# bderembl/msom

Hardware: AMD Instinct MI355X
Metric: grid-point-updates/s (timesteps/s x N^2 x nl), multi-layer QG RK2 step at 4096x4096x6 per GPU (higher is better)
Workload: dtype f64; 1 GPU; C4: msqg double gyre (Verron 1992 params), 4096x4096x6 fp64, tiles 1x1 of 4096x4096, TOLERANCE 1e-3, RK2 step = 2 inversions + 2 tendencies + 2 advances; mg_nrelax=4

## Files before the change

### msom_amd/csrc/kernels.h

```cpp
#ifndef MSOM_KERNELS_H
#define MSOM_KERNELS_H

#include <stdio.h>
#include <stdlib.h>

#include <type_traits>
#include <utility>

#include "msom_internal.h"
#include "modes_inl.h"

template <int LO, int HI, class F>
static inline bool with_int(int v, F &&f) {
  if constexpr (LO > HI) return false;
  else {
    if (v == LO) { f(std::integral_constant<int, LO>{}); return true; }
    return with_int<LO + 1, HI>(v, std::forward<F>(f));
  }
}
template <class F>
static inline void with_bool(bool b, F &&f) {
  if (b) f(std::true_type{});
  else f(std::false_type{});
}
[[noreturn]] static inline void no_kernel(const char *launcher, int nl) {
  fprintf(stderr, "msom: %s: no kernel for nl = %d\n", launcher, nl);
  abort();
}

struct LayerCoef {
  double idh0[MSOM_MAXNL], idh1[MSOM_MAXNL];
};

struct RelaxCoef {
  double D, sqD;
  double idh0[MSOM_MAXNL], idh1[MSOM_MAXNL];
  double t2[MSOM_MAXNL];
  double w[MSOM_MAXNL];
  double it1[MSOM_MAXNL];
  double S[MSOM_MAXNL];
};

struct KernelOpts {
  int march_rows = 0;
  int march_xcd = 1;
  int march_flip = 1;
  int march_dbg = 0;
  int march_lean = 2;
  int march_dma = 2;
  int march_visit_rows = 0;
  int march_visit_pairs = 2;
  int march_visit_ring = 2;
  int march_visit_split = 0;
  int resmax_rows = 0;
  int block_variant = 0;
  int rhs_dbg = 0;
  int lpw_dbg = 0;
};
int device_cu_count();

void launch_fill_ghost(hipStream_t st, double *f, const NatGeom &g, int nl, int bc, int walls, int depth = 1);
void launch_fill_periodic(hipStream_t st, double *f, const NatGeom &g, int nl, int depth);
void launch_fill_lin_dirichlet(hipStream_t st, double *f, const NatGeom &g, int nl, const double *upg, const double *vpg, double D, double Lx,
                               double Ly, int ox = 0, int oy = 0, int sides = WALL_ALL);
void launch_slip_bc(hipStream_t st, const double *po, double *zeta, const NatGeom &g, int nl, double c, int walls);
void launch_pack(hipStream_t st, const double *src, double *dst, const NatGeom &g, int nl);
void launch_unpack(hipStream_t st, const double *src, double *dst, const NatGeom &g, int nl);
void launch_del2(hipStream_t st, const double *po, double *zeta, const NatGeom &g, int nl, double add, double fac, double D);
void launch_stretch(hipStream_t st, const double *po, double *out, const double *S, const NatGeom &g, int nl, double add, double fac,
                    const LayerCoef &lc);
void launch_advection(hipStream_t st, const double *zeta, const double *psi, const double *psipg, const double *zetapg, const double *S,
                      const double *qot, double *dq, const NatGeom &g, int nl, int have_pg, int have_zpg, int stochastic, double D,
                      double beta, double itr_stoch, const LayerCoef &lc);
void launch_umax(hipStream_t st, const double *f, double *partial, double *out, const NatGeom &g, int nl, double D);
void launch_axpy(hipStream_t st, double *dq, const double *x, const NatGeom &g, int nl, double c);
void launch_forcing(hipStream_t st, const double *zeta, const double *psi, const double *qforc, const double *topo, const double *Ro,
                    const double *wind, double *dq, const NatGeom &g, int nl, int have_qforc, int flag_topo, double cs, double cb,
                    double D, double dhb);
void launch_advance(hipStream_t st, double *qo, const double *qi, const double *dq, const double *noise, const NatGeom &g, int nl, double dt,
                    double dts);
void launch_bfn_ab3(hipStream_t st, double *q, double *f1, const double *f2, const double *f3, const double *obs, const double *gain,
                    const NatGeom &g, int nl, double dt12, double k);
int bfn_misfit_blocks(const NatGeom &g);
void launch_bfn_misfit(hipStream_t st, const double *q, const double *obs, const double *gain, double *partial, double *out2, const NatGeom &g,
                       int nl);
struct StatsAcc {
  double *s[MSOM_ST_NACC];
};
void launch_stats_acc(hipStream_t st, unsigned mask, const double *psi, const double *q, const StatsAcc &a, const NatGeom &g, int nl,
                      const double *w_dev, double w, double D2, double *W);
void launch_stats_mean(hipStream_t st, double *out, const double *s, const double *W, const NatGeom &g, int nl);
void launch_stats_derive(hipStream_t st, double *out, const double *pm, const double *sa, const double *sq, const double *W, const NatGeom &g,
                         int nl, int which, double D2);
void launch_time_filter(hipStream_t st, double *me, const double *q, const NatGeom &g, int nl, double a);
int partial_count(const NatGeom &g);
void launch_sum_final(hipStream_t st, const double *partial, double *out, int n);
void launch_ke(hipStream_t st, const double *po, double *partial, double *out, const NatGeom &g, double D);
void launch_sum_layers(hipStream_t st, const double *f, double *partial, double *out, const NatGeom &g, int nl);
void launch_sub_layer_const(hipStream_t st, double *f, const double *sums, const NatGeom &g, int nl, double inv_count);
void launch_make_S(hipStream_t st, const double *Fr, const double *Ro, double *S, const NatGeom &g, int nlm);

void launch_noise(hipStream_t st, double *n, const double *sigma, const NatGeom &g, int nl, double amp, unsigned seed, unsigned draw, int gx0,
                  int gy0, int gnx);

void launch_ptr_rhs(hipStream_t st, const double *psi, const double *c, const double *rel, double *dp, const NatGeom &g, int nl, int np,
                    const double *iPe, const double *ptr_ir, double D);

void launch_advection_de(hipStream_t st, const double *zeta, const double *psi, const double *psipg, const double *zetapg, const double *S, double *j1,
                         double *j2, double *j3, const NatGeom &g, int nl, double D, double beta, double dt, double ediag, const LayerCoef &lc);
void launch_dissip_de(hipStream_t st, const double *p4, const double *str, const double *po, double *dq, const NatGeom &g, int nl, double iRe,
                      double iRe4, double dt, double ediag, double D, int stage);
void launch_ekman_de(hipStream_t st, const double *zeta, const double *po, double *dq, const NatGeom &g, int nl, double cs, double cb, double dt,
                     double ediag);
void launch_running_mean(hipStream_t st, double *pm, const double *po, const NatGeom &g, int nl, int n);
void launch_filter_de(hipStream_t st, double *ft, const double *tmp2, double *pm, const NatGeom &g, int nl, double dtflt, double ediag);

struct RhsResid {
  double *res, *res_c;
  double *res_max;
  double *bsum_partial;
  SplitGeom sg, cg;
};
int rhs_fused_blocks(const NatGeom &g);
void launch_rhs_fused(hipStream_t st, const KernelOpts &o, const double *psi, const double *S, const double *qforc, const double *wind, double *dq,
                      double *umax_partial, double *umax_out, const NatGeom &g, int nl, int walls, int uniformS, const double *Su,
                      int have_qforc, double D, double beta, double iRe, double iRe4, double cs, double cb, double slip_c,
                      const LayerCoef &lc, int variant, const double *q_in = nullptr, double *q_out = nullptr, double dt = 0.,
                      const RhsResid *rr = nullptr, int region = 0, const double *dt_ptr = nullptr);
int rhs_pipe_blocks(const NatGeom &g);
void launch_rhs_lpw(hipStream_t st, const KernelOpts &o, const double *psi, const double *S, const double *qforc, const double *wind, double *dq,
                    const NatGeom &g, int nl, int walls, int uniformS, const double *Su, int have_qforc, double D, double beta, double iRe, double iRe4,
                    double cs, double cb, double slip_c, const LayerCoef &lc, const double *q_in, double *q_out, double dt, int stoch = 0,
                    const double *q_stage = nullptr, const double *noise = nullptr, double crelax = 0., double dts = 0., int region = 0,
                    const double *dt_ptr = nullptr, const RhsResid *rr = nullptr);
int rhs_lpw_blocks(const KernelOpts &o, const NatGeom &g, int nl);

#define MGC_MAXLEV 8
#define MGC_MAXDIM 32
#define MGC_NT 512
struct CoarseLev { double *da, *res; const double *S; SplitGeom g; RelaxCoef rc; };
struct CoarseArgs { CoarseLev lev[MGC_MAXLEV]; int n, walls, prolong_fused, lds; };
void launch_mg_coarse(hipStream_t st, const CoarseArgs *d_args, int nrelax, int nl, int uniformS, int lean = 0);
size_t mg_coarse_lean_doubles(const CoarseArgs &h, int nl);
#define MGC_POOL 19200
size_t mg_coarse_static_lds();
void launch_nat_to_split(hipStream_t st, const double *nat, const NatGeom &g, double *sp, const SplitGeom &sg, int nl);
void launch_split_to_nat(hipStream_t st, const double *sp, const SplitGeom &sg, double *nat, const NatGeom &g, int nl);
void launch_split_pack(hipStream_t st, const double *src, double *sp, const SplitGeom &sg, int nl, int bc, int walls);
void launch_split_unpack(hipStream_t st, const double *sp, const SplitGeom &sg, double *dst, int nl);
void launch_residual(hipStream_t st, const double *a, const double *b, const double *S, const NatGeom &g, double *res, const SplitGeom &sg,
                     int nl, const RelaxCoef &rc, int uniformS, double *maxres, double *sum_partial, int want_sum);
int residual2_blocks(const NatGeom &g);
void launch_residual2(hipStream_t st, const KernelOpts &o, int mode, const double *a, const double *da, double *a_out, const double *b, const double *S,
                      const NatGeom &g, double *res, const SplitGeom &sg, double *res_c, const SplitGeom &cg, int nl, const RelaxCoef &rc,
                      int uniformS, int walls, double *maxres, double *sum_partial, int want_sum, double *umax_partial, double *umax_out,
                      int umax_clean = 0,
                      double *res_c2 = nullptr, const SplitGeom *cg2 = nullptr);
void launch_restrict(hipStream_t st, const double *fine, const SplitGeom &fg, double *coarse, const SplitGeom &cg, int nl);
void launch_restrict_pyramid(hipStream_t st, const double *fine, double *const *out, const SplitGeom *g, int n, int nl);
void launch_prolong(hipStream_t st, const double *coarse, const SplitGeom &cg, double *fine, const SplitGeom &fg, int nl, int walls);
void launch_relax_color(hipStream_t st, double *da, const double *res, const double *S, const SplitGeom &sg, int nl, const RelaxCoef &rc,
                        int uniformS, int color, int walls, int fine, int region = 0);
void launch_relax_ring(hipStream_t st, double *da, const double *res, const double *S, const SplitGeom &sg, int nl, const RelaxCoef &rc,
                       int uniformS, int color, int walls);
int launch_relax_block8(hipStream_t st, const KernelOpts &o, const double *da_in, const double *coarse, const SplitGeom &cg, const double *res, double *da_out,
                        const SplitGeom &sg, int nl, const RelaxCoef &rc, int walls, int nh, int c0, const double *S = nullptr);
void launch_relax_block2(hipStream_t st, const KernelOpts &o, const double *da_in, const double *coarse, const SplitGeom &cg, const double *res, double *da_out,
                         const SplitGeom &sg, int nl, const RelaxCoef &rc, int walls, int fine);
void launch_relax_red_prolong(hipStream_t st, const KernelOpts &o, double *da, const double *coarse, const SplitGeom &cg, const double *res, const double *S,
                              const SplitGeom &sg, int nl, const RelaxCoef &rc, int uniformS, int walls);
void launch_correct(hipStream_t st, double *a, const NatGeom &g, const double *da, const SplitGeom &sg, int nl, int walls);

struct VisitRingBands { int s0[4], ns[4], c0[4], nc[4], n; };
struct MarchCorrect { const double *psi; double *psi_out; NatGeom g; };
struct MarchHalo { const double *in_s, *in_n, *res_s, *res_n; size_t ls; int rows; };
int launch_relax_march(hipStream_t st, const KernelOpts &o, const double *in, double *out, const double *res, const SplitGeom &sg, int nl, const RelaxCoef &rc, int c1,
                       int K, int walls, int chunk_rows = 0, const MarchHalo *h = nullptr, const double *coarse = nullptr, const SplitGeom *cg = nullptr,
                       const MarchCorrect *mc = nullptr, int more_follow = 0, const MarchHalo *coarse_halo = nullptr, int region = 0,
                       const int *skip = nullptr, int skip_compact = 0);
int launch_relax_visit(hipStream_t st, const KernelOpts &o, double *da, double *da_alt, const double *res, const SplitGeom &sg, int nl, const RelaxCoef &rc,
                       int walls, const double *coarse, const SplitGeom &cg, const MarchCorrect &mc);
bool relax_visit_fits(int nl, const SplitGeom &sg, int rows, int pairs);
extern "C" int msom_visit_ring(int hk, int ny, int march_rows, int visit_rows, int pairs, int corr, int *geom, int *bands);
bool march_lean_fits(int nl, const SplitGeom &sg, const NatGeom *ng);

struct ModeCoef {
  double m2l[MSOM_MAXNL * MSOM_MAXNL], ibu[MSOM_MAXNL];
};
int launch_modes_eig(hipStream_t st, const double *S, const NatGeom &g, int nl, int ncx, int ncy, double *out, size_t ols, int per_column,
                     const ModesLayers &l, int *flag);
int launch_modes_get(hipStream_t st, double *out, const double *md, const ModeCoef *mc, const NatGeom &g, int nl, const ModesLayers &l, int which,
                     int first, int cnt);
int launch_modes_rd(hipStream_t st, double *rd, const double *md, const ModeCoef *mc, const NatGeom &g, int nl, int mode);
int launch_modes_project(hipStream_t st, const double *in, double *out, const double *md, const ModeCoef *mc, const NatGeom &g, int nl,
                         const ModesLayers &l, int to_modes);
int modes_energy_blocks(const NatGeom &g);
int modes_energy_stride(const NatGeom &g);
int launch_modes_energy(hipStream_t st, const double *psi, const double *md, const ModeCoef *mc, const NatGeom &g, int nl, const ModesLayers &l,
                        double *partial, double *out, double D);

struct HelmCoef {
  double ibu[MSOM_MAXNL];
  double rd[MSOM_MAXNL];
};
struct HelmCount {
  int n[MSOM_MAXNL];
};
MSOM_HD double helm_diag(double ibu, double sqD) {
#ifdef MSOM_STRICT
  return (-(ibu * sqD) + 2.) + 2.;
#else
  return fma(-ibu, sqD, 4.);
#endif
}
HelmCoef helm_coef(const double *ibu, int nl, double sqD);
int launch_helm_relax(hipStream_t st, double *da, const double *res, const double *ibu_sp, const HelmCoef *hc, const SplitGeom &sg, int nl,
                      double sqD, int color, int sweep, const HelmCount &cnt, int walls);
int helm_residual_blocks(const NatGeom &g);
int launch_helm_residual(hipStream_t st, const double *a, const double *b, const double *ibu_sp, const HelmCoef *hc, const NatGeom &g, double *res,
                         const SplitGeom &sg, int nl, double D, double *maxres, double *sum_partial, int stride, int want_sum);

enum { SPEC_IN_AB = 0, SPEC_IN_UV = 1, SPEC_IN_G = 2 };
enum { SPEC_CROSS = 0, SPEC_SUM = 1 };
struct SpecIn {
  const double *a, *b;
  size_t off, ls;
  int pitch, l0, mode;
  double D2, rD2;
  double dhc[MSOM_MAXNL];
};
int spec_prepare_device();
void launch_spec_rows(hipStream_t st, const SpecIn &in, int nx, int ny, int layers, double2 *Z, const double2 *tw, int nt);
void launch_spec_transpose(hipStream_t st, const double2 *Z, double2 *ZT, int nx, int ny, int layers);
void launch_spec_cols(hipStream_t st, const double2 *ZT, int nx, int ny, int layers, int kind, double scale, double *V, double *out2d, const double2 *tw,
                      int nt);
void launch_spec_shells(hipStream_t st, const double *V, int nx, int ny, int layers, int smax, double *TE);
void launch_spec_final(hipStream_t st, const double *TE, int smax, int nbins, int layers, double dk2, double *res);

int nq_rhs_rows(const NatGeom &g, int rows);
void launch_nq_rhs(hipStream_t st, const double *psi, const double *qforc, double *zeta, double *dq, const NatGeom &g, int walls, double D,
                   double beta, double nu, double cek, double bc_fac, const double *q_in, double *q_out, double dt, int rows);
void launch_nq_ghost(hipStream_t st, const double *psi, double *f, const NatGeom &g, double bc_fac);
void launch_nq_adv(hipStream_t st, const double *psi, const double *zeta, double *dq, const NatGeom &g, double D, double beta);

void launch_wv_restrict(hipStream_t st, const double *f, const NatGeom &fg, double *c, const NatGeom &cg, int nl);
void launch_wv_recon(hipStream_t st, const double *s, const double *sc, const double *rc, const double *sig, double *out, const NatGeom &fg,
                     const NatGeom &cg, int nl);
void launch_wv_root(hipStream_t st, const double *s, const double *sig, double *r, const NatGeom &g, int nl);
void launch_wv_recon_m(hipStream_t st, const double *s, const double *sc, const double *rc, const double *sig, const double *mc, double *out,
                       const NatGeom &fg, const NatGeom &cg, int nl);
void launch_wv_root_m(hipStream_t st, const double *s, const double *sig, const double *mc, double *r, const NatGeom &g, int nl);
void launch_wv_vert2cell(hipStream_t st, const double *v, const NatGeom &vg, double *c, const NatGeom &cg, int nl);
void launch_wv_vertex_update(hipStream_t st, double *psi, double *psif, const double *c, const double *mask, const NatGeom &vg, const NatGeom &cg, int nl,
                             double dtflt, int nbar, int update_mean);
void launch_wv_qof(hipStream_t st, double *qof, double *q, const double *tmp, const NatGeom &g, int nl, double dtflt, int nbar, int restore);

void launch_n_bnd_from(hipStream_t st, double *f, const double *g, const NatGeom &ge, int nl, double c, int use_g_bnd, double gbc, int walls = WALL_ALL);
void launch_n_bnd_const(hipStream_t st, double *f, const NatGeom &ge, int nl, double v, int sp = 0, int walls = WALL_ALL);
void launch_n_mul_mask(hipStream_t st, double *a, double *b, const double *mk, const NatGeom &g, int nl);
void launch_n_del2(hipStream_t st, const double *in, double *out, const NatGeom &g, int nl, double add, double fac, double D);
void launch_n_stretch(hipStream_t st, const double *in, double *out, const double *S2, const NatGeom &g, int nl, double add, double fac,
                      const LayerCoef &lc);
void launch_n_stretch_sqg(hipStream_t st, const double *in, const double *bs, const double *S2S, double *out, const double *S2, const NatGeom &g, int nl,
                          double add, double fac, const LayerCoef &lc);
void launch_n_lap_bs(hipStream_t st, const double *bs, double *out, const NatGeom &g, double D);
void launch_n_sqg_rhs(hipStream_t st, const double *q, const double *S2S, const double *bs, double *qeff, const NatGeom &g, int nl, double idh00);
void launch_n_rhs_main(hipStream_t st, const double *psi, const double *zeta, const double *pg, const double *S2, const double *topo, double *dq,
                       const NatGeom &g, int nl, int have_pg, int have_topo, double D, double beta, double drag, double f0, double dhb, const LayerCoef &lc);
void launch_n_axpy(hipStream_t st, double *dq, const double *x, const NatGeom &g, int nl, double c);
void launch_n_rhs_pre(hipStream_t st, double *q, const double *psi, double *psi_out, double *zeta, const double *mk, const NatGeom &g, int nl, double D,
                      double bc, double gbc);
void launch_n_del2_bnd(hipStream_t st, const double *in, double *out, const NatGeom &g, int nl, double D, double bc, int use_bnd, double gbc);
void launch_n_rhs_all(hipStream_t st, const double *psi, const double *zeta, const double *tmp, const double *pg, const double *S2, const double *topo,
                      const double *qf, const double *qf3d, const double *mk, const double *d2bs, const double *S2S, double *dq, const NatGeom &g, int nl,
// ... 67 lines not shown
```

### msom_amd/csrc/kernels_lpw.hip

```cpp
#include "rhs_inl.h"

#pragma clang fp contract(off)

#define LPW_W 58
#define LPW_R 4
#define LPW_R_RES 2
#ifdef MSOM_STRICT
#define LPW_NV 3
#define LPW_MAXW 8
#else
#define LPW_NV 2
#define LPW_MAXW 12
#endif

struct LpwArgs {
  const double *psi, *S, *qforc, *wind, *q_in;
  const double *q_stage, *noise;
  double crelax, dts;
  double *dq, *q_out;
  double dt;
  const double *dt_ptr;
  NatGeom g;
  int nl, walls, uniformS, have_qforc, H, NS;
  int noedge_off;
  int region;
  int dbg;
  RhsResid rr;
  double D, beta, iRe, iRe4, cs, cb, slip_c;
  LayerCoef lc;
  double Su[MSOM_MAXNL];
};

template <int R, bool UNI, bool QF, bool ADV, bool STOCH, bool EDGE, bool RES, int NV>
__device__ __forceinline__ void lpw_body(const LpwArgs &a, double (&ring)[2][LPW_MAXW][R][NV][64], double &res_m, double &res_bs) {
  const int lane = threadIdx.x & 63;
  const int wv = __builtin_amdgcn_readfirstlane((int)(threadIdx.x >> 6));
  const int nl = a.nl, nx = a.g.nx, ny = a.g.ny;
  const int l = wv % nl;
  const ptrdiff_t pitch = a.g.pitch;
  const int strip = blockIdx.x * a.NS + wv / nl, nstrips = (nx + LPW_W - 1) / LPW_W;
  const int x0 = min(strip, nstrips - 1) * LPW_W, y0 = blockIdx.y * a.H, y1 = min(ny, y0 + a.H);
  const int gi = x0 - 3 + lane, gic = min(gi, nx + 2);
  const double dtv = a.dt_ptr ? *a.dt_ptr : a.dt;
  const double D = a.D, D2 = D * D, rD2 = 1. / D2, D12 = 12. * D * D, rD12 = 1. / D12, D2x = 2 * D, rD2x = 1. / D2x;
  const double rD = 1. / D;
  const bool oddx = !(lane & 1);
  const bool lower = l + 1 < nl, upper = l > 0;
  const int lW = ((a.walls & WALL_W) && x0 == 0) ? 2 : -1;
  const int eL = nx - x0 + 3;
  const int lE = ((a.walls & WALL_E) && eL <= 63) ? eL : -1;
  const bool bcx = EDGE && (lW >= 0 || lE >= 0);
  const bool south = (a.walls & WALL_S) != 0, north = (a.walls & WALL_N) != 0;
  const bool slip = a.slip_c > 0.;
  const bool out_ok = lane >= 3 && lane <= 60 && gi < nx && strip < nstrips;
  const double *pP = a.psi + nat_idx(a.g, l, 0, gic);
  const double *pQ = lower ? pP + a.g.ls : pP;
  const double idh0 = a.lc.idh0[l], idh1 = a.lc.idh1[l];
  const double su0 = (nl > 1 && upper) ? a.Su[l - 1] : 0., su1 = (nl > 1 && lower) ? a.Su[l] : 0.;
  const double windv = l == 0 ? a.wind[min(y0 + lane, ny - 1)] : 0.;
  auto wind_row = [&](int j) -> double {
    const long long b = __double_as_longlong(windv);
    const int lo = __builtin_amdgcn_readlane((int)b, j - y0), hi = __builtin_amdgcn_readlane((int)(b >> 32), j - y0);
    return __longlong_as_double(((long long)hi << 32) | (unsigned int)lo);
  };

  double P[5], PL[4], PR[4], Z[4], ZL[4], ZR[4], T[3], TL[2], TR[2], Q[3], QL[3], QR[3];
#pragma unroll
  for (int k = 0; k < 5; k++) P[k] = 0.;
#pragma unroll
  for (int k = 0; k < 4; k++) PL[k] = PR[k] = Z[k] = ZL[k] = ZR[k] = 0.;
#pragma unroll
  for (int k = 0; k < 3; k++) T[k] = Q[k] = QL[k] = QR[k] = 0.;
  TL[0] = TL[1] = TR[0] = TR[1] = 0.;

#ifdef MSOM_STRICT
  double abA[R], jdA[R], lapTA[R], zcA[R], tcA[R];
#else
  double tlA[R];
#endif
  double pnext[R], qnext[R], qreg[R], fqreg[R], qsreg[STOCH ? R : 1], nzreg[STOCH ? R : 1];
  double xdA[R], ydA[R];
#pragma unroll
  for (int r = 0; r < R; r++) xdA[r] = ydA[r] = 0.;
#pragma unroll
  for (int r = 0; r < R; r++) {
#ifdef MSOM_STRICT
    abA[r] = jdA[r] = lapTA[r] = zcA[r] = tcA[r] = 0.;
#else
    tlA[r] = 0.;
#endif
    pnext[r] = qnext[r] = qreg[r] = fqreg[r] = 0.;
  }

  auto ld = [&](const double *base, int j) -> double { return base[(ptrdiff_t)((a.dbg & 2) ? y0 : (EDGE ? min(j, ny + 2) : j)) * pitch]; };
#ifdef MSOM_STRICT
  auto lap5 = [&](double c, double w, double e, double n, double s) -> double { return DIVC(e + w + n + s - 4 * c, D2, rD2); };
#else
  auto lap5 = [&](double c, double w, double e, double n, double s) -> double { return fma(-4., c, e + w + n + s) * rD2; };
#endif
  auto xfix = [&](double raw, double so, double sw, double se) -> double {
    if (bcx) {
      if (slip) {
        if (lane == lW) raw = a.slip_c * (se - so);
        if (lane == lE) raw = a.slip_c * (sw - so);
      } else {
        const double re = lane_above(raw), rw = lane_below(raw);
        if (lane == lW) raw = -re;
        if (lane == lE) raw = -rw;
      }
    }
    return raw;
  };
  auto yghost = [&](double dm, double dmw, double dme, double sm, double sg) -> double {
    double v = slip ? a.slip_c * (sm - sg) : -dm;
    if (lane == lW) v = dme;
    if (lane == lE) v = dmw;
    return v;
  };

  auto row = [&](int j, double pnew, double qnew, bool centre, bool yedge, int b, int r) {
#pragma unroll
    for (int k = 0; k < 4; k++) P[k] = P[k + 1];
    P[4] = pnew;
#pragma unroll
    for (int k = 0; k < 3; k++) { PL[k] = PL[k + 1]; PR[k] = PR[k + 1]; Z[k] = Z[k + 1]; ZL[k] = ZL[k + 1]; ZR[k] = ZR[k + 1]; }
    T[0] = T[1]; T[1] = T[2]; TL[0] = TL[1]; TR[0] = TR[1];
#pragma unroll
    for (int k = 0; k < 2; k++) { Q[k] = Q[k + 1]; QL[k] = QL[k + 1]; QR[k] = QR[k + 1]; }
    Q[2] = qnew; QL[2] = lane_below(qnew); QR[2] = lane_above(qnew);
    PL[3] = lane_below(P[3]); PR[3] = lane_above(P[3]);
    double z = xfix(lap5(P[3], PL[3], PR[3], P[4], P[2]), P[3], PL[3], PR[3]);
    if (yedge && north && j + 2 == ny) z = yghost(Z[2], ZL[2], ZR[2], P[2], P[3]);
    Z[3] = z; ZL[3] = lane_below(z); ZR[3] = lane_above(z);
    if (yedge && south && j + 2 == 0) {
      Z[2] = yghost(Z[3], ZL[3], ZR[3], P[3], P[2]);
      ZL[2] = lane_below(Z[2]); ZR[2] = lane_above(Z[2]);
    }
    double t = xfix(lap5(Z[2], ZL[2], ZR[2], Z[3], Z[1]), Z[2], ZL[2], ZR[2]);
    if (yedge && north && j + 1 == ny) t = yghost(T[1], TL[0], TR[0], Z[1], Z[2]);
    T[2] = t; TL[1] = lane_below(t); TR[1] = lane_above(t);
    if (yedge && south && j + 1 == 0) T[1] = yghost(T[2], TL[1], TR[1], Z[2], Z[1]);
    if (!centre) return;

    double p[3][3], zz[3][3], p1[3][3];
#pragma unroll
    for (int k = 0; k < 3; k++) {
      p[k][0] = PL[k]; p[k][1] = P[k]; p[k][2] = PR[k];
      zz[k][0] = ZL[k]; zz[k][1] = Z[k]; zz[k][2] = ZR[k];
      p1[k][0] = QL[k]; p1[k][1] = Q[k]; p1[k][2] = QR[k];
    }
    const double adv = (STOCH && l == 0) ? 0. : mjac9(p, zz, D12, rD12);
    const double be = DIVC(a.beta * (p[1][0] - p[1][2]), D2x, rD2x);
    const double jd = (lower && !STOCH) ? mjac9(p, p1, D12, rD12) : 0.;
    const double zc = Z[1], tc = T[1];
    const double lapT = lap5(tc, TL[0], TR[0], T[2], T[0]);
    if (RES) {
      const double dW = P[1] - PL[1], dE = PR[1] - P[1], dS = P[1] - P[0], dN = P[2] - P[1];
#ifdef MSOM_STRICT
      xdA[r] = (dW / D - dE / D) / D;
      ydA[r] = (dS / D - dN / D) / D;
#else
      const double fa = oddx ? dW : dE, fb = oddx ? dE : dW;
      const double x = fma(rD, fb, -(rD * fa));
      xdA[r] = oddx ? -x : x;
      ydA[r] = fma(rD, dS, -(rD * dN));
#endif
      ring[b][wv][r][NV - 1][lane] = Q[1] - P[1];
    }
#ifdef MSOM_STRICT
    abA[r] = adv + be; jdA[r] = jd; lapTA[r] = lapT; zcA[r] = zc; tcA[r] = tc;
    ring[b][wv][r][0][lane] = zc;
    ring[b][wv][r][1][lane] = tc;
    ring[b][wv][r][2][lane] = jd;
#else
    double tl = fma(tc, a.iRe, fma(a.iRe4, lapT, adv + be));
    if (l == 0) tl -= fma(a.cs, zc, wind_row(j));
    if (l == nl - 1) tl = fma(-a.cb, zc, tl);
    tlA[r] = tl;
    ring[b][wv][r][0][lane] = fma(a.iRe, zc, a.iRe4 * tc);
    ring[b][wv][r][1][lane] = jd;
#endif
  };

  auto finish = [&](int j, int b, int r, double s0, double s1, double fq) -> double {
#ifdef MSOM_STRICT
    const double zc = zcA[r], tc = tcA[r];
    double zm = 0., tm = 0., zp = 0., tp = 0., ju = 0.;
    if (upper) { zm = ring[b][wv - 1][r][0][lane]; tm = ring[b][wv - 1][r][1][lane]; ju = -ring[b][wv - 1][r][2][lane]; }
    if (lower) { zp = ring[b][wv + 1][r][0][lane]; tp = ring[b][wv + 1][r][1][lane]; }
    double t = abA[r];
    if (nl > 1) {
      if (upper) t = t + s0 * ju * idh0;
      if (lower) t = t + s1 * jdA[r] * idh1;
    }
    t = 0. + t;
    double dq = t;
    auto stretch = [&](double fac, double pm, double pc, double pp) -> double {
      if (l == 0) return fac * s1 * (pp - pc) * idh1;
      if (l < nl - 1) return fac * (s0 * (pm - pc) * idh0 + s1 * (pp - pc) * idh1);
      return fac * s0 * (pm - pc) * idh0;
    };
    if (a.iRe != 0.) {
      if (nl > 1) dq = 1. * dq + stretch(a.iRe, zm, zc, zp);
      dq += tc * a.iRe;
    }
    if (a.iRe4 != 0.) {
      if (nl > 1) dq = 1. * dq + stretch(a.iRe4, tm, tc, tp);
      dq = 1. * dq + a.iRe4 * lapTA[r];
    }
    if (l == 0) dq -= a.cs * zc;
    if (l == nl - 1) dq -= a.cb * zc;
    if (l == 0) dq -= wind_row(j);
#else
    double dq = tlA[r];
    const double xc = ring[b][wv][r][0][lane];
    if (nl > 1) {
      if (upper) dq = fma(s0 * idh0, (ring[b][wv - 1][r][0][lane] - xc) - ring[b][wv - 1][r][1][lane], dq);
      if (lower) dq = fma(s1 * idh1, (ring[b][wv + 1][r][0][lane] - xc) + ring[b][wv][r][1][lane], dq);
    }
#endif
    if (QF) dq += fq;
#ifdef MSOM_STRICT
    if (STOCH) return (qreg[r] + qsreg[r] * a.crelax + nzreg[r] * a.dts) + dq * a.dt;
    return ADV ? qreg[r] + dq * dtv : dq;
#else
    if (STOCH) return fma(dq, a.dt, fma(nzreg[r], a.dts, fma(qsreg[r], a.crelax, qreg[r])));
    return ADV ? fma(dq, dtv, qreg[r]) : dq;
#endif
  };

  auto resid = [&](int b, int r, double s0, double s1, double q) -> double {
    double re = q;
#ifdef MSOM_STRICT
    if (upper) re = re + s0 * ring[b][wv - 1][r][NV - 1][lane] * idh0;
    if (lower) re = re - s1 * ring[b][wv][r][NV - 1][lane] * idh1;
    re += xdA[r];
    re += ydA[r];
#else
    if (upper) re = fma(idh0, s0 * ring[b][wv - 1][r][NV - 1][lane], re);
    if (lower) re = fma(-(ring[b][wv][r][NV - 1][lane] * s1), idh1, re);
    re = fma(rD, xdA[r], re);
    re = fma(rD, ydA[r], re);
#endif
    return re;
  };

#pragma unroll
  for (int r = 0; r < R; r++) {
    pnext[r] = ld(pP, y0 + r + 3);
    qnext[r] = ld(pQ, y0 + r + 1);
  }
  {
    double wp[6], wq[2];
#pragma unroll
    for (int k = 0; k < 6; k++) wp[k] = ld(pP, y0 - 3 + k);
    wq[0] = ld(pQ, y0 - 1); wq[1] = ld(pQ, y0);
#pragma unroll
    for (int k = 0; k < 6; k++) row(y0 - 6 + k, wp[k], k >= 4 ? wq[k - 4] : 0., false, EDGE, 0, 0);
  }

  double *const outp = ADV ? a.q_out : a.dq;
  const int nblk = (y1 - y0 + R - 1) / R;
  __builtin_amdgcn_s_waitcnt(0x0F70);
  for (int k = 0; k <= nblk; k++) {
    const int b = k & 1;
    if (k > 0) {
      const int jb = y0 + (k - 1) * R;
      double s0[R], s1[R], val[R];
#pragma unroll
      for (int r = 0; r < R; r++) {
        s0[r] = su0; s1[r] = su1;
        if (!UNI && nl > 1) {
          const size_t c = nat_idx(a.g, l, min(jb + r, ny - 1), gic);
          if (upper) s0[r] = a.S[c - a.g.ls];
          if (lower) s1[r] = a.S[c];
        }
      }
#pragma unroll
      for (int r = 0; r < R; r++) {
        val[r] = finish(jb + r, b ^ 1, r, s0[r], s1[r], fqreg[r]);
        asm volatile("" : "+v"(val[r]));
      }
#pragma unroll
      for (int r = 0; r < R; r++)
        if (out_ok && jb + r < y1 && !(a.dbg & 1)) outp[nat_idx(a.g, l, jb + r, gic)] = val[r];
      if (RES) {
        double re[R];
#pragma unroll
        for (int r = 0; r < R; r++) {
          re[r] = resid(b ^ 1, r, s0[r], s1[r], val[r]);
          if (out_ok && jb + r < y1) {
            res_m = fmax(res_m, fabs(re[r]));
            res_bs += val[r];
            if (!(a.dbg & 1)) a.rr.res[split_idx(a.rr.sg, l, jb + r, gi)] = re[r];
          }
        }
#pragma unroll
        for (int r = 0; r + 1 < R; r += 2) {
          const double o0 = lane_above(re[r]), o1 = lane_above(re[r + 1]);
          if (out_ok && !oddx && jb + r + 1 < y1 && !(a.dbg & 1)) {
            double sum = 0.;
            sum += re[r];
            sum += re[r + 1];
            sum += o0;
            sum += o1;
            a.rr.res_c[split_idx(a.rr.cg, l, (jb + r) >> 1, gi >> 1)] = sum / 4;
          }
        }
      }
    }
    if (k < nblk) {
      const int j0 = y0 + k * R;
      const bool yedge = EDGE && j0 + R + 2 > ny;
#pragma unroll
      for (int r = 0; r < R; r++) {
        const size_t c = nat_idx(a.g, l, (a.dbg & 2) ? y0 : (EDGE ? min(j0 + r, ny - 1) : j0 + r), gic);
        if (ADV) qreg[r] = a.q_in[c];
        if (QF) fqreg[r] = a.qforc[c];
        if (STOCH) { qsreg[r] = a.q_stage[c]; nzreg[r] = a.noise[c]; }
      }
#pragma unroll
      for (int r = 0; r < R; r++) {
        const int j = j0 + r;
        double pn, qn;
        asm volatile("v_mov_b64 %0, %1" : "=v"(pn) : "v"(pnext[r]));
        asm volatile("v_mov_b64 %0, %1" : "=v"(qn) : "v"(qnext[r]));
        pnext[r] = ld(pP, j + R + 3);
        qnext[r] = ld(pQ, j + R + 1);
        row(j, pn, qn, true, yedge, b, r);
      }
    }
    __syncthreads();
  }
}

template <int R, bool UNI, bool QF, bool ADV, bool STOCH = false, bool RES = false>
__global__ void __launch_bounds__(64 * LPW_MAXW) k_rhs_lpw(LpwArgs a) {
  static_assert(!RES || (ADV && !STOCH && R % 2 == 0), "the residual by-product rides in the plain tendency + advance pass");
  constexpr int NV = LPW_NV + (RES ? 1 : 0);
  __shared__ double ring[2][LPW_MAXW][R][NV][64];
  double res_m = 0., res_bs = 0.;
  const int wv = __builtin_amdgcn_readfirstlane((int)(threadIdx.x >> 6));
  const int nx = a.g.nx, ny = a.g.ny;
  const int strip = blockIdx.x * a.NS + wv / a.nl, nstrips = (nx + LPW_W - 1) / LPW_W;
  const int x0 = min(strip, nstrips - 1) * LPW_W, y0 = blockIdx.y * a.H, y1 = min(ny, y0 + a.H);
  const bool xwall = ((a.walls & WALL_W) && x0 == 0) || ((a.walls & WALL_E) && nx - x0 + 3 <= 63);
  const int nblk = (y1 - y0 + R - 1) / R;
  const bool ywall = y0 == 0 || y0 + nblk * R + R > ny;
  if (a.region) {
    const bool inner = strip < nstrips && x0 - 3 >= 0 && x0 + 60 < nx && y0 - 3 >= 0 && y0 + nblk * R + R + 2 < ny;
    if ((a.region == 1) != inner) return;
  }
  if (xwall || ywall || a.noedge_off) lpw_body<R, UNI, QF, ADV, STOCH, true, RES, NV>(a, ring, res_m, res_bs);
  else lpw_body<R, UNI, QF, ADV, STOCH, false, RES, NV>(a, ring, res_m, res_bs);
  if (RES) {
    const int lane = threadIdx.x & 63, nw = blockDim.x >> 6;
    for (int o = 32; o > 0; o >>= 1) {
      res_m = fmax(res_m, __shfl_xor(res_m, o, 64));
      res_bs += __shfl_xor(res_bs, o, 64);
    }
    double *red = &ring[0][0][0][0][0];
    if (lane == 0) { red[wv] = res_m; red[LPW_MAXW + wv] = res_bs; }
    __syncthreads();
    if (threadIdx.x == 0) {
      double mm = red[0], ss = red[LPW_MAXW];
      for (int k = 1; k < nw; k++) { mm = fmax(mm, red[k]); ss += red[LPW_MAXW + k]; }
      atomicMax((unsigned long long *)a.rr.res_max, (unsigned long long)__double_as_longlong(mm));
      a.rr.bsum_partial[blockIdx.y * gridDim.x + blockIdx.x] = ss;
    }
  }
}

static void lpw_shape(const KernelOpts &o, const NatGeom &g, int nl, bool res, int &NS, int &H) {
  const int strips = (g.nx + LPW_W - 1) / LPW_W;
  H = o.rhs_dbg >> 8;
  NS = LPW_MAXW / nl < 1 ? 1 : LPW_MAXW / nl;
  if (NS > strips) NS = strips;
  if (H <= 0) {
    const int ncu = device_cu_count();
    const int wgx = (strips + NS - 1) / NS;
    double best = -1.;
    for (int h = 64; h >= 8; h -= 8) {
      const double r = (double)wgx * ((g.ny + h - 1) / h) / ncu, cost = (r <= 3. ? ceil(r) : r + 0.5) * (h + 6);
      if (best < 0. || cost < best) { best = cost; H = h; }
    }
  }
  if (H < 8) H = 8;
  if (res) H = (H + 1) & ~1;
}
int rhs_lpw_blocks(const KernelOpts &o, const NatGeom &g, int nl) {
  int NS, H;
  lpw_shape(o, g, nl, true, NS, H);
  const int strips = (g.nx + LPW_W - 1) / LPW_W;
  return ((strips + NS - 1) / NS) * ((g.ny + H - 1) / H);
}

void launch_rhs_lpw(hipStream_t st, const KernelOpts &o, const double *psi, const double *S, const double *qforc, const double *wind, double *dq,
                    const NatGeom &g, int nl, int walls, int uniformS, const double *Su, int have_qforc, double D, double beta, double iRe, double iRe4,
                    double cs, double cb, double slip_c, const LayerCoef &lc, const double *q_in, double *q_out, double dt, int stoch,
                    const double *q_stage, const double *noise, double crelax, double dts, int region, const double *dt_ptr, const RhsResid *rr) {
  LpwArgs a;
  const bool res = rr != nullptr;
  if (res && (stoch || !q_out || region || (g.nx & 1) || (g.ny & 1) || !rr->res_c)) {
    fprintf(stderr, "msom: launch_rhs_lpw: the residual by-product needs the plain tendency + advance pass on one tile with even sides\n");
    abort();
  }
  if (res) {
    a.rr = *rr;
    (void)hipMemsetAsync(rr->res_max, 0, sizeof(double), st);
  } else {
    a.rr.res = a.rr.res_c = a.rr.res_max = a.rr.bsum_partial = nullptr;
    a.rr.sg = SplitGeom(); a.rr.cg = SplitGeom();
  }
  a.region = region;
  a.dt_ptr = dt_ptr;
  a.q_stage = q_stage; a.noise = noise; a.crelax = crelax; a.dts = dts;
  a.psi = psi; a.S = S; a.qforc = qforc; a.wind = wind; a.q_in = q_in; a.dq = dq; a.q_out = q_out; a.dt = dt;
  a.dbg = o.lpw_dbg & 3;
  a.noedge_off = (o.lpw_dbg & 4) != 0;
  a.g = g; a.nl = nl; a.walls = walls; a.uniformS = uniformS; a.have_qforc = have_qforc;
  a.D = D; a.beta = beta; a.iRe = iRe; a.iRe4 = iRe4; a.cs = cs; a.cb = cb; a.slip_c = slip_c; a.lc = lc;
  for (int l = 0; l < MSOM_MAXNL; l++) a.Su[l] = Su ? Su[l] : 0.;
  const int strips = (g.nx + LPW_W - 1) / LPW_W;
  int H;
  lpw_shape(o, g, nl, res, a.NS, H);
  a.H = H;
  const dim3 gr((strips + a.NS - 1) / a.NS, (g.ny + H - 1) / H), bl(64 * nl * a.NS);
  if (stoch && !q_out) {
    fprintf(stderr, "msom: launch_rhs_lpw: stochastic variant needs q_out\n");
    abort();
  }
  with_bool(uniformS, [&](auto U) {
    with_bool(have_qforc, [&](auto Q) {
      constexpr bool UNI = decltype(U)::value, QF = decltype(Q)::value;
      if (stoch) hipLaunchKernelGGL((k_rhs_lpw<LPW_R, UNI, QF, true, true>), gr, bl, 0, st, a);
      else if (res) hipLaunchKernelGGL((k_rhs_lpw<LPW_R_RES, UNI, QF, true, false, true>), gr, bl, 0, st, a);
      else if (q_out) hipLaunchKernelGGL((k_rhs_lpw<LPW_R, UNI, QF, true>), gr, bl, 0, st, a);
      else hipLaunchKernelGGL((k_rhs_lpw<LPW_R, UNI, QF, false>), gr, bl, 0, st, a);
    });
  });
}
```

### msom_amd/csrc/kernels_mg.hip

```cpp
#include "kernels.h"
#include "mg_inl.h"
#include "rhs_inl.h"


#define BX 64
#define BY 4

static inline dim3 grid2d(int nx, int ny) { return dim3((nx + BX - 1) / BX, (ny + BY - 1) / BY); }
static inline dim3 block2d() { return dim3(BX, BY); }

__device__ __forceinline__ double wave_max(double v) {
  for (int o = 32; o > 0; o >>= 1) v = fmax(v, __shfl_down(v, o, 64));
  return v;
}
__device__ __forceinline__ double wave_sum(double v) {
  for (int o = 32; o > 0; o >>= 1) v += __shfl_down(v, o, 64);
  return v;
}


__global__ void k_nat_to_split(const double *__restrict__ nat, NatGeom g, double *sp, SplitGeom sg, int nl) {
  const int i = blockIdx.x * BX + threadIdx.x, j = blockIdx.y * BY + threadIdx.y;
  if (i >= g.nx || j >= g.ny) return;
  for (int l = 0; l < nl; l++) sp[split_idx(sg, l, j, i)] = nat[nat_idx(g, l, j, i)];
// ... 228 lines not shown
  if (p.want_sum) bs = wave_sum(bs);
  if (VEL) {
#pragma unroll
    for (int l = 0; l < MSOM_MAXNL; l++)
      if (l < nl) {
        const double v = wave_max(um[l]);
        if (threadIdx.x == 0) smu[l][threadIdx.y] = v;
      }
  }
  if (threadIdx.x == 0) { smm[threadIdx.y] = m; sms[threadIdx.y] = bs; }
  __syncthreads();
  if (threadIdx.x == 0 && threadIdx.y == 0) {
    double mm = smm[0], ss = sms[0];
    for (int k = 1; k < BY; k++) { mm = fmax(mm, smm[k]); ss += sms[k]; }
    atomicMax((unsigned long long *)p.maxres, (unsigned long long)__double_as_longlong(mm));
    if (p.want_sum) p.sum_partial[blockIdx.y * gridDim.x + blockIdx.x] = ss;
  }
  if (VEL && threadIdx.y == 0 && threadIdx.x < nl) {
    double v = smu[threadIdx.x][0];
    for (int k = 1; k < BY; k++) v = fmax(v, smu[threadIdx.x][k]);
    p.umax_partial[(size_t)(blockIdx.y * gridDim.x + blockIdx.x) * nl + threadIdx.x] = v;
  }
}

#define CR_TR 16
#define CR_TW 128
#define CR_LP 132
template <bool UNIFORM, bool CORR = true>
__global__ void __launch_bounds__(BX *BY, UNIFORM ? 4 : 3) k_correct_residual(Res2Args p) {
  __shared__ __align__(16) double T[2][CR_TR + 2][CR_LP];
  __shared__ double smm[BY];
  __shared__ double smu[MSOM_MAXNL][BY];
  constexpr int NR = CR_TR / BY;
  const int tx = threadIdx.x, ty = threadIdx.y, tid = ty * BX + tx;
  const int x0 = blockIdx.x * CR_TW, y0 = blockIdx.y * CR_TR;
  const int nl = p.nl, nx = p.g.nx, ny = p.g.ny;
  const int i = x0 + 2 * tx;
  const double D = p.rc.D, rD = 1. / D;
  const bool inx = i < nx;
  const size_t c0 = nat_idx(p.g, 0, y0 + ty, inx ? i : 0), se0 = split_idx(p.sg, 0, y0 + ty, inx ? i : 0);
  const size_t cstep = (size_t)BY * p.g.pitch, sstep = (size_t)BY * p.sg.rp;
  constexpr int NH = 2 * (CR_TW + 2) + 2 * CR_TR;
  double a0e[NR], a0o[NR], a1e[NR], a1o[NR], a2e[NR], a2o[NR];
  auto stage = [&](int l, int b, double *xe, double *xo) {
    const double *al = p.a + (size_t)l * p.g.ls, *dl = p.da + (size_t)l * p.sg.ls;
#pragma unroll
    for (int k = 0; k < NR; k++) {
      double e = 0., o = 0.;
      if (inx && y0 + ty + BY * k < ny) {
        const double2 v = *reinterpret_cast<const double2 *>(al + c0 + k * cstep);
        e = v.x; o = v.y;
        if (CORR) { e = e + dl[se0 + k * sstep]; o = o + dl[se0 + k * sstep + p.sg.hp]; }
      }
      xe[k] = e; xo[k] = o;
      *reinterpret_cast<double2 *>(&T[b][ty + BY * k + 1][2 * tx + 2]) = make_double2(e, o);
    }
    for (int h = tid; h < NH; h += BX * BY) {
      int r, cc;
      if (h < CR_TW + 2) { r = -1; cc = h - 1; }
      else if (h < 2 * (CR_TW + 2)) { r = CR_TR; cc = h - (CR_TW + 2) - 1; }
      else if (h < 2 * (CR_TW + 2) + CR_TR) { r = h - 2 * (CR_TW + 2); cc = -1; }
      else { r = h - 2 * (CR_TW + 2) - CR_TR; cc = CR_TW; }
      const int gx = x0 + cc, gy = y0 + r;
      double v = 0.;
      if (gx <= nx && gy <= ny) {
        v = al[nat_idx(p.g, 0, gy, gx)];
        if (CORR) v = v + dl[split_idx(p.sg, 0, gy, gx)];
      }
      T[b][r + 1][cc + 2] = v;
    }
  };
  double m = 0.;
  double s1e[NR], s1o[NR], s0e[NR], s0o[NR];
#pragma unroll
  for (int k = 0; k < NR; k++) { a0e[k] = a0o[k] = a2e[k] = a2o[k] = 0.; s0e[k] = s0o[k] = s1e[k] = s1o[k] = 0.; }
  stage(0, 0, a1e, a1o);
  __syncthreads();
  for (int l = 0; l < nl; l++) {
    const int b = l & 1;
    if (l < nl - 1) stage(l + 1, b ^ 1, a2e, a2o);
    const double su0 = l > 0 ? p.rc.S[l - 1] : 0., su1 = l < nl - 1 ? p.rc.S[l] : 0.;
    const double i0 = p.rc.idh0[l], i1 = p.rc.idh1[l];
    double uu = 0.;
#pragma unroll
    for (int k = 0; k < NR; k++) {
      const int j = y0 + ty + BY * k;
      if (inx && j < ny) {
        const int r = ty + BY * k + 1, cx = 2 * tx + 2;
        const size_t cl = c0 + k * cstep + (size_t)l * p.g.ls;
        const double2 bv = *reinterpret_cast<const double2 *>(p.b + cl);
        const double be = bv.x, bo = bv.y;
        double z0e, z0o, z1e, z1o;
        if (UNIFORM) { z0e = z0o = su0; z1e = z1o = su1; }
        else {
          if (l < nl - 1) { const double2 sv = *reinterpret_cast<const double2 *>(p.S + cl); s1e[k] = sv.x; s1o[k] = sv.y; }
          z0e = s0e[k]; z0o = s0o[k]; z1e = s1e[k]; z1o = s1o[k];
        }
        const double e1 = a1e[k], o1 = a1o[k];
        const double a1w = T[b][r][cx - 1], a1ee = T[b][r][cx + 2];
        const double2 sv2 = *reinterpret_cast<const double2 *>(&T[b][r - 1][cx]), nv2 = *reinterpret_cast<const double2 *>(&T[b][r + 1][cx]);
        const double a1se = sv2.x, a1so = sv2.y, a1ne = nv2.x, a1no = nv2.y;
        double re = be, ro = bo;
        if (nl > 1) {
          if (l == 0) {
            re = be + z1e * (e1 - a2e[k]) * i1;
            ro = bo + z1o * (o1 - a2o[k]) * i1;
          } else if (l < nl - 1) {
            re = be + z0e * (e1 - a0e[k]) * i0 - z1e * (a2e[k] - e1) * i1;
            ro = bo + z0o * (o1 - a0o[k]) * i0 - z1o * (a2o[k] - o1) * i1;
          } else {
            re = be + z0e * (e1 - a0e[k]) * i0;
            ro = bo + z0o * (o1 - a0o[k]) * i0;
          }
        }
        re += DIVC(DIVC(e1 - a1w, D, rD) - DIVC(o1 - e1, D, rD), D, rD);
        re += DIVC(DIVC(e1 - a1se, D, rD) - DIVC(a1ne - e1, D, rD), D, rD);
        ro += DIVC(DIVC(o1 - e1, D, rD) - DIVC(a1ee - o1, D, rD), D, rD);
        ro += DIVC(DIVC(o1 - a1so, D, rD) - DIVC(a1no - o1, D, rD), D, rD);
        if (CORR) {
          *reinterpret_cast<double2 *>(p.a_out + cl) = make_double2(e1, o1);
          nat_write_ghosts(p.a_out, p.g, l, j, i, e1, p.walls);
          nat_write_ghosts(p.a_out, p.g, l, j, i + 1, o1, p.walls);
        }
        m = fmax(m, fmax(fabs(re), fabs(ro)));
        const double nw = T[b][r + 1][cx - 1], sw = T[b][r - 1][cx - 1], se2 = T[b][r - 1][cx + 2];
        const double ue = fabs(DIVC(0.25 * (a1ne - a1se + nw - sw), D, rD)), ve = fabs(DIVC(0.25 * (o1 - a1w + a1so - sw), D, rD));
        const double uo = fabs(DIVC(0.25 * (a1no - a1so + a1ne - a1se), D, rD)), vo = fabs(DIVC(0.25 * (a1ee - e1 + se2 - a1se), D, rD));
        uu = fmax(uu, fmax(fmax(ue, ve), fmax(uo, vo)));
        a0e[k] = e1; a0o[k] = o1;
        if (!UNIFORM) { s0e[k] = s1e[k]; s0o[k] = s1o[k]; }
        a1e[k] = a2e[k]; a1o[k] = a2o[k];
      }
    }
    uu = wave_max(uu);
    if (tx == 0) smu[l][ty] = uu;
    __syncthreads();
  }
  m = wave_max(m);
  if (tx == 0) smm[ty] = m;
  __syncthreads();
  if (tid == 0) {
    double mm = smm[0];
    for (int k = 1; k < BY; k++) mm = fmax(mm, smm[k]);
    atomicMax((unsigned long long *)p.maxres, (unsigned long long)__double_as_longlong(mm));
  }
  if (ty == 0 && tx < nl) {
    double v = smu[tx][0];
    for (int k = 1; k < BY; k++) v = fmax(v, smu[tx][k]);
    p.umax_partial[(size_t)(blockIdx.y * gridDim.x + blockIdx.x) * nl + tx] = v;
  }
}

#define RM_OW 62
template <int NL>
__global__ void __launch_bounds__(256) k_resmax_march(Res2Args p, int H) {
  __shared__ double smm[4];
  __shared__ double smu[MSOM_MAXNL][4];
  const int lane = threadIdx.x & 63, wv = threadIdx.x >> 6;
  const int strip = blockIdx.x * 4 + wv;
  const int nx = p.g.nx, ny = p.g.ny, pitch = p.g.pitch;
  const int nstrips = (nx + RM_OW - 1) / RM_OW;
  const double D = p.rc.D, rD = 1. / D;
  double m = 0., uu[NL];
#pragma unroll
  for (int l = 0; l < NL; l++) uu[l] = 0.;
  const int y0 = blockIdx.y * H, y1 = min(y0 + H, ny);
  if (strip < nstrips && y0 < ny) {
    const int x0 = strip * RM_OW, gi = min(x0 - 1 + lane, nx);
    const bool own = lane >= 1 && lane <= RM_OW && x0 - 1 + lane < nx;
    const size_t ls = p.g.ls;
    const double *pa = p.a + nat_idx(p.g, 0, 0, gi), *pb = p.b + nat_idx(p.g, 0, 0, min(gi, nx - 1) < 0 ? 0 : min(gi, nx - 1));
    double Wm[NL], Wc[NL], Wp[NL], Wn[NL], Em[NL], Mm[NL], qc[NL], qn[NL];
#pragma unroll
    for (int l = 0; l < NL; l++) {
      Wm[l] = pa[l * ls + (ptrdiff_t)(y0 - 1) * pitch];
      Wc[l] = pa[l * ls + (ptrdiff_t)y0 * pitch];
      Wp[l] = pa[l * ls + (ptrdiff_t)min(y0 + 1, ny) * pitch];
      qc[l] = pb[l * ls + (ptrdiff_t)y0 * pitch];
    }
#pragma unroll
    for (int l = 0; l < NL; l++) { Em[l] = lane_above(Wm[l]); Mm[l] = lane_below(Wm[l]); }
    for (int j = y0; j < y1; j++) {
      const ptrdiff_t rn = (ptrdiff_t)min(j + 2, ny) * pitch, rq = (ptrdiff_t)min(j + 1, ny - 1) * pitch;
#pragma unroll
      for (int l = 0; l < NL; l++) { Wn[l] = pa[l * ls + rn]; qn[l] = pb[l * ls + rq]; }
#pragma unroll
      for (int l = 0; l < NL; l++) {
        const double c = Wc[l], E = lane_above(c), W = lane_below(c), N = Wp[l], S = Wm[l], NW = lane_below(N), SE = Em[l], SW = Mm[l];
        const double be = qc[l];
        double re = be;
        if (NL > 1) {
          const double i0 = p.rc.idh0[l], i1 = p.rc.idh1[l];
          const double z0 = l > 0 ? p.rc.S[l - 1] : 0., z1 = l < NL - 1 ? p.rc.S[l] : 0.;
          if (l == 0) re = be + z1 * (c - Wc[l + 1 < NL ? l + 1 : l]) * i1;
          else if (l < NL - 1) re = be + z0 * (c - Wc[l - 1]) * i0 - z1 * (Wc[l + 1 < NL ? l + 1 : l] - c) * i1;
          else re = be + z0 * (c - Wc[l - 1]) * i0;
        }
        re += DIVC(DIVC(c - W, D, rD) - DIVC(E - c, D, rD), D, rD);
        re += DIVC(DIVC(c - S, D, rD) - DIVC(N - c, D, rD), D, rD);
        const double u = fabs(DIVC(0.25 * (N - S + NW - SW), D, rD)), v = fabs(DIVC(0.25 * (E - W + SE - SW), D, rD));
        if (own) { m = fmax(m, fabs(re)); uu[l] = fmax(uu[l], fmax(u, v)); }
        Em[l] = E; Mm[l] = W;
      }
#pragma unroll
      for (int l = 0; l < NL; l++) { Wm[l] = Wc[l]; Wc[l] = Wp[l]; Wp[l] = Wn[l]; qc[l] = qn[l]; }
    }
  }
  m = wave_max(m);
  if (lane == 0) smm[wv] = m;
#pragma unroll
  for (int l = 0; l < NL; l++) {
    const double w = wave_max(uu[l]);
    if (lane == 0) smu[l][wv] = w;
  }
  __syncthreads();
  if (threadIdx.x == 0) {
    const double mm = fmax(fmax(smm[0], smm[1]), fmax(smm[2], smm[3]));
    atomicMax((unsigned long long *)p.maxres, (unsigned long long)__double_as_longlong(mm));
  }
  if (threadIdx.x < NL)
    p.umax_partial[(size_t)(blockIdx.y * gridDim.x + blockIdx.x) * NL + threadIdx.x] =
        fmax(fmax(smu[threadIdx.x][0], smu[threadIdx.x][1]), fmax(smu[threadIdx.x][2], smu[threadIdx.x][3]));
}
template <int NL>
static dim3 resmax_march_launch(hipStream_t st, const Res2Args &p, int H) {
  const int nstrips = (p.g.nx + RM_OW - 1) / RM_OW;
  dim3 gr((nstrips + 3) / 4, (p.g.ny + H - 1) / H);
  hipLaunchKernelGGL(k_resmax_march<NL>, gr, dim3(256), 0, st, p, H);
  return gr;
}
static dim3 launch_resmax_march(hipStream_t st, const Res2Args &p, int H) {
  dim3 gr;
  if (!with_int<1, MSOM_FASTNL>(p.nl, [&](auto N) { gr = resmax_march_launch<N()>(st, p, H); })) no_kernel("launch_resmax_march", p.nl);
  return gr;
}

__global__ void k_max_final_mg(const double *partial, double *out, int nb, int nl) {
  __shared__ double sm[MSOM_MAXNL][4];
  const int per = (nb + gridDim.x - 1) / gridDim.x, b0 = blockIdx.x * per, b1 = min(nb, b0 + per);
  double v[MSOM_MAXNL];
#pragma unroll
  for (int l = 0; l < MSOM_MAXNL; l++) v[l] = 0.;
  for (int b = b0 + threadIdx.x; b < b1; b += 256) {
    const double *row = partial + (size_t)b * nl;
#pragma unroll
    for (int l = 0; l < MSOM_MAXNL; l++)
      if (l < nl) v[l] = fmax(v[l], row[l]);
  }
#pragma unroll
  for (int l = 0; l < MSOM_MAXNL; l++) {
    double w = v[l];
    for (int o = 32; o > 0; o >>= 1) w = fmax(w, __shfl_down(w, o, 64));
    if ((threadIdx.x & 63) == 0) sm[l][threadIdx.x >> 6] = w;
  }
  __syncthreads();
  if (threadIdx.x < nl) {
    const double w = fmax(fmax(sm[threadIdx.x][0], sm[threadIdx.x][1]), fmax(sm[threadIdx.x][2], sm[threadIdx.x][3]));
    atomicMax((unsigned long long *)(out + threadIdx.x), (unsigned long long)__double_as_longlong(w));
  }
}

int residual2_blocks(const NatGeom &g) {
  dim3 gr = grid2d(g.nx / 2, g.ny);
  return gr.x * gr.y;
}
void launch_residual2(hipStream_t st, const KernelOpts &o, int mode, const double *a, const double *da, double *a_out, const double *b, const double *S,
                      const NatGeom &g, double *res, const SplitGeom &sg, double *res_c, const SplitGeom &cg, int nl, const RelaxCoef &rc,
                      int uniformS, int walls, double *maxres, double *sum_partial, int want_sum, double *umax_partial, double *umax_out, int umax_clean,
                      double *res_c2, const SplitGeom *cg2) {
  Res2Args p;
  p.res_c2 = res_c2;
  if (cg2) p.cg2 = *cg2; else p.cg2 = cg;
  p.dbg = o.rhs_dbg;
  p.umax_partial = umax_partial;
  p.a = a; p.b = b; p.S = S; p.da = da; p.a_out = a_out; p.res = res; p.res_c = res_c; p.maxres = maxres; p.sum_partial = sum_partial;
  p.g = g; p.sg = sg; p.cg = cg; p.nl = nl; p.uniformS = uniformS; p.want_sum = want_sum; p.walls = walls; p.rc = rc;
  dim3 gr = grid2d(g.nx / 2, g.ny);
  switch (mode) {
    case 1:
      if (g.nx % 2 == 0 && g.nx >= CR_TW && g.ny >= CR_TR && !(p.dbg & 128)) {
        gr = dim3((g.nx + CR_TW - 1) / CR_TW, (g.ny + CR_TR - 1) / CR_TR);
        if (uniformS) hipLaunchKernelGGL((k_correct_residual<true, true>), gr, block2d(), 0, st, p);
        else hipLaunchKernelGGL((k_correct_residual<false, true>), gr, block2d(), 0, st, p);
      } else
        hipLaunchKernelGGL((k_residual2<true, false, false>), gr, block2d(), 0, st, p);
      if (!umax_clean) (void)hipMemsetAsync(umax_out, 0, nl * sizeof(double), st);
      hipLaunchKernelGGL(k_max_final_mg, dim3(64), dim3(256), 0, st, umax_partial, umax_out, (int)(gr.x * gr.y), nl);
      break;
    case 2: hipLaunchKernelGGL((k_residual2<false, true, false>), gr, block2d(), 0, st, p); break;
    case 6: hipLaunchKernelGGL((k_residual2<false, true, true>), gr, block2d(), (size_t)nl * (BY * BX * 2 + 2 * BX) * sizeof(double), st, p); break;
    case 0: hipLaunchKernelGGL((k_residual2<false, false, false>), gr, block2d(), 0, st, p); break;
    case 8:
      if (uniformS && g.nx >= 64 && g.ny >= 16 && o.resmax_rows >= 0 && nl <= MSOM_FASTNL) {
        gr = launch_resmax_march(st, p, o.resmax_rows ? o.resmax_rows : 32);
      } else if (g.nx % 2 == 0 && g.nx >= CR_TW && g.ny >= CR_TR && !(p.dbg & 128)) {
        gr = dim3((g.nx + CR_TW - 1) / CR_TW, (g.ny + CR_TR - 1) / CR_TR);
        if (uniformS) hipLaunchKernelGGL((k_correct_residual<true, false>), gr, block2d(), 0, st, p);
        else hipLaunchKernelGGL((k_correct_residual<false, false>), gr, block2d(), 0, st, p);
      } else
        hipLaunchKernelGGL((k_residual2<false, false, false, true>), gr, block2d(), 0, st, p);
      if (!umax_clean) (void)hipMemsetAsync(umax_out, 0, nl * sizeof(double), st);
      hipLaunchKernelGGL(k_max_final_mg, dim3(64), dim3(256), 0, st, umax_partial, umax_out, (int)(gr.x * gr.y), nl);
      break;
    default: break;
  }
}


__device__ __forceinline__ void restrict_pt(const double *__restrict__ fine, const SplitGeom &fg, double *coarse, const SplitGeom &cg, int nl, int I, int J) {
  for (int l = 0; l < nl; l++) {
    double sum = 0.;
    sum += fine[split_idx(fg, l, 2 * J, 2 * I)];
    sum += fine[split_idx(fg, l, 2 * J + 1, 2 * I)];
    sum += fine[split_idx(fg, l, 2 * J, 2 * I + 1)];
    sum += fine[split_idx(fg, l, 2 * J + 1, 2 * I + 1)];
    coarse[split_idx(cg, l, J, I)] = sum / 4;
  }
}
__global__ void k_restrict(const double *__restrict__ fine, SplitGeom fg, double *coarse, SplitGeom cg, int nl) {
  const int I = blockIdx.x * BX + threadIdx.x, J = blockIdx.y * BY + threadIdx.y;
  if (I >= cg.nx || J >= cg.ny) return;
  restrict_pt(fine, fg, coarse, cg, nl, I, J);
}
void launch_restrict(hipStream_t st, const double *fine, const SplitGeom &fg, double *coarse, const SplitGeom &cg, int nl) {
  hipLaunchKernelGGL(k_restrict, grid2d(cg.nx, cg.ny), block2d(), 0, st, fine, fg, coarse, cg, nl);
}

#define RPYR_MAX 5
struct RestrictPyramidArgs {
  const double *fine;
  double *out[RPYR_MAX];
  SplitGeom g[RPYR_MAX + 1];
  int n, nl;
};
__global__ void __launch_bounds__(256) k_restrict_pyramid(RestrictPyramidArgs a) {
  extern __shared__ double rp[];
  const int tid = threadIdx.x, n = a.n, nl = a.nl, T = 1 << n;
  const int X0 = blockIdx.x * T, Y0 = blockIdx.y * T;
  double *cur = rp, *nxt = rp + nl * (T / 2) * (T / 2);
  {
    const int s = T >> 1;
    for (int t = tid; t < s * s * nl; t += 256) {
      const int I = t % s, J = (t / s) % s, l = t / (s * s);
      const int fi = X0 + 2 * I, fj = Y0 + 2 * J;
      double sum = 0.;
      sum += a.fine[split_idx(a.g[0], l, fj, fi)];
      sum += a.fine[split_idx(a.g[0], l, fj + 1, fi)];
      sum += a.fine[split_idx(a.g[0], l, fj, fi + 1)];
      sum += a.fine[split_idx(a.g[0], l, fj + 1, fi + 1)];
      const double v = sum / 4;
      cur[(l * s + J) * s + I] = v;
      a.out[0][split_idx(a.g[1], l, (Y0 >> 1) + J, (X0 >> 1) + I)] = v;
    }
  }
  for (int k = 2; k <= n; k++) {
    __syncthreads();
    const int s = T >> k, sf = s << 1;
    for (int t = tid; t < s * s * nl; t += 256) {
      const int I = t % s, J = (t / s) % s, l = t / (s * s);
      const double *f = cur + l * sf * sf;
      double sum = 0.;
      sum += f[(2 * J) * sf + 2 * I];
      sum += f[(2 * J + 1) * sf + 2 * I];
      sum += f[(2 * J) * sf + 2 * I + 1];
      sum += f[(2 * J + 1) * sf + 2 * I + 1];
      const double v = sum / 4;
      nxt[(l * s + J) * s + I] = v;
      a.out[k - 1][split_idx(a.g[k], l, (Y0 >> k) + J, (X0 >> k) + I)] = v;
    }
    double *tmp = cur; cur = nxt; nxt = tmp;
  }
}
void launch_restrict_pyramid(hipStream_t st, const double *fine, double *const *out, const SplitGeom *g, int n, int nl) {
  RestrictPyramidArgs a;
  a.fine = fine; a.n = n; a.nl = nl;
  for (int k = 0; k <= n; k++) a.g[k] = g[k];
  for (int k = 0; k < n; k++) a.out[k] = out[k];
  const int T = 1 << n;
  const size_t lds = (size_t)nl * ((T / 2) * (T / 2) + (T / 4 > 0 ? (T / 4) * (T / 4) : 1)) * sizeof(double);
  hipLaunchKernelGGL(k_restrict_pyramid, dim3(g[0].nx / T, g[0].ny / T), dim3(256), lds, st, a);
}

__device__ __forceinline__ void prolong_pt(const double *__restrict__ coarse, const SplitGeom &cg, double *fine, const SplitGeom &fg, int nl, int walls, int i, int j) {
  const int I = i >> 1, J = j >> 1, cx = (i & 1) ? 1 : -1, cy = (j & 1) ? 1 : -1;
  for (int l = 0; l < nl; l++) {
    const double v = BILINEAR(coarse[split_idx(cg, l, J, I)], coarse[split_idx(cg, l, J, I + cx)], coarse[split_idx(cg, l, J + cy, I)],
                              coarse[split_idx(cg, l, J + cy, I + cx)]);
    fine[split_idx(fg, l, j, i)] = v;
    split_write_ghosts(fine, fg, l, j, i, v, walls);
  }
}
__global__ void k_prolong(const double *__restrict__ coarse, SplitGeom cg, double *fine, SplitGeom fg, int nl, int walls) {
  const int i = blockIdx.x * BX + threadIdx.x, j = blockIdx.y * BY + threadIdx.y;
  if (i >= fg.nx || j >= fg.ny) return;
  prolong_pt(coarse, cg, fine, fg, nl, walls, i, j);
}
void launch_prolong(hipStream_t st, const double *coarse, const SplitGeom &cg, double *fine, const SplitGeom &fg, int nl, int walls) {
  hipLaunchKernelGGL(k_prolong, grid2d(fg.nx, fg.ny), block2d(), 0, st, coarse, cg, fine, fg, nl, walls);
}


struct RelaxArgs {
  double *da;
  const double *res, *S;
  SplitGeom g;
  int color, walls;
  int region;
  RelaxCoef rc;
};

template <int NL, bool UNIFORM>
__device__ __forceinline__ void relax_color_pt(const RelaxArgs &p, int kx, int j);
template <int NL, bool UNIFORM, bool FINE>
__global__ void __launch_bounds__(BX *BY) k_relax_color(RelaxArgs p) {
  const int kx = blockIdx.x * BX + threadIdx.x, j = blockIdx.y * BY + threadIdx.y;
  if (kx >= p.g.hk || j >= p.g.ny) return;
  if (p.region == 1) {
    const int i = 2 * kx + ((j + p.color) & 1);
    if (i == 0 || i == p.g.nx - 1 || j == 0 || j == p.g.ny - 1) return;
  }
  relax_color_pt<NL, UNIFORM>(p, kx, j);
}
template <int NL, bool UNIFORM>
__global__ void __launch_bounds__(256) k_relax_ring(RelaxArgs p) {
  const int t = blockIdx.x * 256 + threadIdx.x, hk = p.g.hk, ny = p.g.ny;
  int kx, j;
  if (t < hk) { kx = t; j = 0; }
  else if (t < 2 * hk) { kx = t - hk; j = ny - 1; }
  else if (t < 2 * hk + ny - 2) { j = 1 + t - 2 * hk; kx = ((j + p.color) & 1) ? hk - 1 : 0; }
  else return;
  if (ny == 1 && t >= hk) return;
  relax_color_pt<NL, UNIFORM>(p, kx, j);
}
template <int NL, bool UNIFORM>
__device__ __forceinline__ void relax_color_pt(const RelaxArgs &p, int kx, int j) {
  const int px = (j + p.color) & 1;
  const int i = 2 * kx + px;
  const int hp = p.g.hp, rp = p.g.rp;
  const size_t ls = p.g.ls;
  const size_t own = (size_t)(j + 1) * rp + px * hp + MSOM_SP + kx;
  const size_t oth = (size_t)(j + 1) * rp + (1 - px) * hp + MSOM_SP + kx;
  const size_t iw = oth - 1 + px, ie = oth + px, is = own - rp, in = own + rp;
  const double sqD = p.rc.sqD;
  double rhs[NL], x[NL];
  if (NL == 1) {
    double n = -sqD * p.res[own], d = 0.;
    n += p.da[ie] + p.da[iw]; d += 2.;
// ... 1069 lines not shown
```

### msom_amd/csrc/msom_api.hip

```cpp
#include "msom_host.h"

#define RHS_RESID_MIN 23
#define MARCH_HALO 4

static void free_agglomeration(msom *m);

extern "C" const char *msom_version(void) {
#ifdef MSOM_STRICT
  return "msomhip 0.1 (strict: -ffp-contract=off, reference expression order, bit-exact vs oracle)";
#else
  return "msomhip 0.1 (fast: FMA contraction, reciprocal multiplies)";
#endif
}


NatGeom make_nat(int nx, int ny) {
  NatGeom g;
  g.nx = nx; g.ny = ny;
  g.pitch = ((nx + 15) / 16) * 16 + 2 * MSOM_XP;
  g.rows = ny + 2 * MSOM_YP;
  g.ls = (size_t)g.pitch * g.rows;
  return g;
}
static SplitGeom make_split(int nx, int ny) {
  SplitGeom s;
  s.nx = nx; s.ny = ny;
  s.hk = nx / 2;
  s.hp = ((s.hk + 15) / 16) * 16 + 2 * MSOM_SP;
  s.rp = 2 * s.hp;
  s.rows = ny + 2;
  s.ls = (size_t)s.rp * s.rows;
  return s;
}

int sync_stream(msom *m) {
  HIPCHK(hipStreamSynchronize(m->st));
  return m->sticky;
}

static bool prof_on(const msom *m, const ProfSlot &ps) {
  if (m->profile == 2) return &ps == &m->prof_march_corr || &ps == &m->prof_march_visit || (&ps >= &m->prof_march[0] && &ps <= &m->prof_march[4]);
  return m->profile != 0;
}
void prof_begin(msom *m, ProfSlot &ps) {
  if (!prof_on(m, ps)) return;
  if (ps.used + 2 > ps.ev.size()) {
    hipEvent_t a, b;
    hipEventCreate(&a); hipEventCreate(&b);
    ps.ev.push_back(a); ps.ev.push_back(b);
  }
  hipEventRecord(ps.ev[ps.used], m->st);
}
void prof_end(msom *m, ProfSlot &ps) {
  if (!prof_on(m, ps)) return;
  hipEventRecord(ps.ev[ps.used + 1], m->st);
  ps.used += 2;
}
void prof_collect(msom *m, ProfSlot &ps) {
  hipStreamSynchronize(m->st);
  for (size_t k = 0; k + 1 < ps.used; k += 2) {
    float ms = 0;
    if (hipEventElapsedTime(&ms, ps.ev[k], ps.ev[k + 1]) == hipSuccess) { ps.total_ms += ms; ps.launches++; }
  }
  ps.used = 0;
}

static double wall_seconds() {
  struct timespec ts;
  clock_gettime(CLOCK_MONOTONIC, &ts);
  return ts.tv_sec + 1e-9 * ts.tv_nsec;
}
static int is_pow2(int n) { return n > 0 && (n & (n - 1)) == 0; }



static const int OPP[8] = {DIR_E, DIR_W, DIR_N, DIR_S, DIR_NE, DIR_NW, DIR_SE, DIR_SW};
#define AXIS(dir) (dir)

void comm_begin(msom *m) {
  if (m->comm_hold) return;
  hipEventRecord(m->ev_c2x, m->st);
  hipStreamWaitEvent(m->st2, m->ev_c2x, 0);
}
void comm_end(msom *m) {
  if (m->comm_hold) return;
  hipEventRecord(m->ev_x2c, m->st2);
  hipStreamWaitEvent(m->st, m->ev_x2c, 0);
}

int reduce_scal(msom *m, int slot, int n, int op) {
  if (m->nranks > 1) {
    comm_begin(m);
    const int r = comm_allreduce(m->comm, m->d_scal + slot, m->h_scal + slot, n, op);
    comm_end(m);
    return r;
  }
  if (m->dbg_nosync) return MSOM_OK;
  HIPCHK(hipMemcpyAsync(m->h_scal + slot, m->d_scal + slot, n * sizeof(double), hipMemcpyDeviceToHost, m->st));
  HIPCHK(hipStreamSynchronize(m->st));
  return MSOM_OK;
}

static bool fits_comm(msom *m, size_t count) {
  if (count <= comm_bufcount(m->comm)) return true;
  msom_set_error("halo message of %zu doubles exceeds the communication buffers (%zu)", count, comm_bufcount(m->comm));
  return false;
}

static int exch_nat(msom *m, double *f, int nl, int bc, int depth) { return exch_nat_g(m, f, m->g, nl, bc, depth); }
int exch_nat_g(msom *m, double *f, const NatGeom &g, int nl, int bc, int depth) {
  const int d = depth;
  if (m->nranks > 1 && !fits_comm(m, (size_t)d * ((g.nx > g.ny ? g.nx : g.ny) + 2 * d) * nl)) return MSOM_ERR_ARG;
  hipStream_t cs = m->nranks > 1 ? m->st2 : m->st;
  if (m->nranks > 1) comm_begin(m);
  if (m->nranks > 1) {
    Xfer x[2];
    int n = 0;
    for (int dir : {DIR_W, DIR_E}) {
      if (m->nb[dir] < 0) continue;
      launch_nat_pack_strip(cs, f, g, nl, dir == DIR_W ? 0 : g.nx - d, 0, d, g.ny, comm_sendbuf(m->comm, dir));
      x[n++] = {m->nb[dir], AXIS(dir), comm_sendbuf(m->comm, dir), comm_recvbuf(m->comm, dir), (size_t)d * g.ny * nl};
    }
    int r = comm_exchange(m->comm, x, n);
    if (r) { comm_end(m); return r; }
    for (int dir : {DIR_W, DIR_E}) {
      if (m->nb[dir] < 0) continue;
      launch_nat_unpack_strip(cs, f, g, nl, dir == DIR_W ? -d : g.nx, 0, d, g.ny, comm_recvbuf(m->comm, dir));
    }
  }
  launch_fill_ghost(cs, f, g, nl, bc, m->walls, d);
  if (m->nranks > 1) {
    Xfer x[2];
    int n = 0;
    const int w = g.nx + 2 * d;
    for (int dir : {DIR_S, DIR_N}) {
      if (m->nb[dir] < 0) continue;
      launch_nat_pack_strip(cs, f, g, nl, -d, dir == DIR_S ? 0 : g.ny - d, w, d, comm_sendbuf(m->comm, dir));
      x[n++] = {m->nb[dir], AXIS(dir), comm_sendbuf(m->comm, dir), comm_recvbuf(m->comm, dir), (size_t)d * w * nl};
    }
    int r = comm_exchange(m->comm, x, n);
    if (r) { comm_end(m); return r; }
    for (int dir : {DIR_S, DIR_N}) {
      if (m->nb[dir] < 0) continue;
      launch_nat_unpack_strip(cs, f, g, nl, -d, dir == DIR_S ? -d : g.ny, w, d, comm_recvbuf(m->comm, dir));
    }
  }
  if (m->nranks > 1) comm_end(m);
  return MSOM_OK;
}

static int exch_split_raw(msom *m, double *f, const SplitGeom &sg, int nl, int corners) {
  hipStream_t cs = m->st2;
  if (!fits_comm(m, (size_t)nl * ((sg.nx > sg.ny ? sg.nx : sg.ny) + 2))) return MSOM_ERR_ARG;
  Xfer x[4];
  int n = 0;
// ... 226 lines not shown
      else if (jx >= 0 && jx < px && jy >= 0 && jy < py) m->nb[d] = jy * px + jx;
    }
  }
  if (alloc_all(m) != MSOM_OK ||
      (m->nranks > 1 && comm_create(&m->comm, rank, m->nranks, id128, m->st2,
                                    (size_t)MARCH_HALO * ((m->nx > m->ny ? m->nx : m->ny) + 16) * m->nl * (p.nptr > 1 ? p.nptr : 1)) != MSOM_OK) ||
      (nq ? nq_alloc(m) : set_vars(m)) != MSOM_OK) {
    msom_destroy(m);
    return nullptr;
  }
  return m;
}

extern "C" msom_t *msom_create_str(const char *text) {
  if (!text) { msom_set_error("null params text"); return nullptr; }
  Params p;
  msom_params_defaults(&p);
  msom_params_parse_text(&p, text);
  msom *m = create_common(p, 1, 1, 0, nullptr);
  if (m) m->params_text = text;
  return m;
}
extern "C" msom_t *msom_create(const char *path) {
  const char *pp = path ? path : "params.in";
  FILE *fp = fopen(pp, "rt");
  if (!fp) {
    msom_set_error("file %s not found", pp);
    return nullptr;
  }
  std::string text;
  char buf[4096];
  size_t n;
  while ((n = fread(buf, 1, sizeof buf, fp)) > 0) text.append(buf, n);
  fclose(fp);
  return msom_create_str(text.c_str());
}

static void clear_graphs(msom *m);
extern "C" int msom_destroy(msom_t *m) {
  if (!m) return MSOM_ERR_ARG;
  if (m->st) hipStreamSynchronize(m->st);
  clear_graphs(m);
  for (int k = 0; k < MSOM_NFIELDS; k++)
    if (m->f[k]) hipFree(m->f[k]);
  for (int k = 0; k < m->nlev; k++) {
    if (m->da[k]) hipFree(m->da[k]);
    if (m->da_alt[k]) hipFree(m->da_alt[k]);
    for (auto *v : {&m->mh_da_s, &m->mh_da_n, &m->mh_res_s, &m->mh_res_n})
      if (k < v->size() && (*v)[k]) hipFree((*v)[k]);
    if (m->res[k]) hipFree(m->res[k]);
    if (m->S[k]) hipFree(m->S[k]);
  }
  free_agglomeration(m);
  for (size_t k = 0; k < m->wv_sig.size(); k++) {
    if (k == 0) { if (m->wv_gsend) hipFree(m->wv_gsend); if (m->wv_grecv) hipFree(m->wv_grecv); }
    if (k > 0 && m->wv_s[k]) hipFree(m->wv_s[k]);
    if (k > 0 && m->wv_r[k]) hipFree(m->wv_r[k]);
    if (m->wv_sig[k]) hipFree(m->wv_sig[k]);
  }
  if (m->psi_alt) hipFree(m->psi_alt);
  if (m->q_alt) hipFree(m->q_alt);
  if (m->ev_spec) hipEventDestroy(m->ev_spec);
  if (m->h_pub) hipHostFree(m->h_pub);
  if (m->staging) hipFree(m->staging);
  if (m->partial) hipFree(m->partial);
  if (m->partial_rr) hipFree(m->partial_rr);
  if (m->bfn_partial) hipFree(m->bfn_partial);
  stats_drop(m);
  modes_drop(m);
  spec_drop(m);
  if (m->modes_dev) hipFree(m->modes_dev);
  if (m->modes_flag) hipFree(m->modes_flag);
  if (m->modes_partial) hipFree(m->modes_partial);
  for (double *p : {m->helm_pm, m->helm_qm, m->helm_scal, m->helm_partial})
    if (p) hipFree(p);
  if (m->d_cargs) hipFree(m->d_cargs);
  if (m->partial_umax) hipFree(m->partial_umax);
  if (m->d_scal) hipFree(m->d_scal);
  if (m->h_scal) hipHostFree(m->h_scal);
  if (m->d_wind) hipFree(m->d_wind);
  for (const auto &s : prof_slots(m))
    for (auto e : s.second->ev) hipEventDestroy(e);
  if (m->comm) comm_destroy(m->comm);
  if (m->ev_c2x) hipEventDestroy(m->ev_c2x);
  if (m->ev_x2c) hipEventDestroy(m->ev_x2c);
  if (m->st2) hipStreamDestroy(m->st2);
  if (m->st) hipStreamDestroy(m->st);
  delete m;
  return MSOM_OK;
}

static void free_agglomeration(msom *m);

static void clear_graphs(msom *m);
static int *kernel_opt(KernelOpts &o, const char *key) {
#define KOPT(f) {#f, &KernelOpts::f}
  static const struct { const char *key; int KernelOpts::*f; } keys[] = {
      KOPT(march_rows), KOPT(march_xcd), KOPT(march_flip), KOPT(march_dbg), KOPT(march_lean), KOPT(march_dma),
      KOPT(march_visit_rows), KOPT(march_visit_pairs), KOPT(march_visit_ring), KOPT(march_visit_split), KOPT(resmax_rows), KOPT(block_variant), KOPT(rhs_dbg), KOPT(lpw_dbg)};
#undef KOPT
  for (const auto &k : keys)
    if (!strcmp(key, k.key)) return &(o.*k.f);
  return nullptr;
}
extern "C" int msom_set_option(msom_t *m, const char *key, double v) {
  if (m) m->res_ready = -1;
  if (!m || !key) return MSOM_ERR_ARG;
  if (m->model) return nq_set_option(m, key, v);
  clear_graphs(m);
  if (!strcmp(key, "graph")) { m->use_graph = (int)v; return MSOM_OK; }
  if (!strcmp(key, "TOLERANCE")) m->p.tolerance = v;
  else if (!strcmp(key, "NITERMAX")) m->p.nitermax = (int)v;
  else if (!strcmp(key, "NITERMIN")) m->p.nitermin = (int)v;
  else if (!strcmp(key, "DT")) m->p.DT = v;
  else if (!strcmp(key, "flag_topo")) m->flag_topo = (int)v;
  else if (!strcmp(key, "quiet")) m->quiet = (int)v;
  else if (!strcmp(key, "uniform_S")) {
    m->uniform_opt = (int)v;
    if (m->const_set) return build_coefs(m);
  }
  else if (!strcmp(key, "profile")) m->profile = (int)v;
  else if (!strcmp(key, "fused")) m->fused = (int)v;
  else if (!strcmp(key, "mg_fused")) m->mg_fused = (int)v;
  else if (!strcmp(key, "march")) m->march = (int)v;
  else if (!strcmp(key, "march_min")) m->march_min = (int)v;
  else if (!strcmp(key, "march_min_tiled")) m->march_min_tiled = (int)v;
  else if (!strcmp(key, "march_partial")) m->march_partial = (int)v;
  else if (!strcmp(key, "march_prolong")) m->march_prolong = (int)v;
  else if (!strcmp(key, "march_correct")) m->march_correct = (int)v;
  else if (!strcmp(key, "march_visit")) m->march_visit = (int)v;
  else if (!strcmp(key, "march_visit_min")) m->march_visit_min = (int)v;
  else if (!strcmp(key, "dbg_nosync")) m->dbg_nosync = (int)v;
  else if (!strcmp(key, "async_solve")) m->async_solve = (int)v;
  else if (!strcmp(key, "step_sync")) m->step_sync = (int)v;
  else if (!strcmp(key, "march_k")) m->march_k = (int)v < 2 ? 2 : ((int)v > 4 ? 4 : (int)v);
  else if (!strcmp(key, "block_small")) m->block_small = (int)v;
  else if (!strcmp(key, "block8")) m->block8 = (int)v;
  else if (!strcmp(key, "restrict2")) m->restrict2 = (int)v;
  else if (!strcmp(key, "restrict_pyr")) m->restrict_pyr = (int)v;
  else if (!strcmp(key, "block8_max")) m->block8_max = (int)v;
  else if (!strcmp(key, "block_sweeps")) { m->block_sweeps = (int)v; if (m->const_set) return build_coefs(m); }
  else if (!strcmp(key, "mg_global_sum")) m->mg_global_sum = (int)v;
  else if (!strcmp(key, "agglomerate")) { m->agglomerate = (int)v; if (m->const_set) return build_coefs(m); }
  else if (!strcmp(key, "agg_size")) { m->agg_size = (int)v; if (m->const_set) return build_coefs(m); }
  else if (!strcmp(key, "prolong_fused")) { m->prolong_fused = (int)v; if (m->const_set) return build_coefs(m); }
  else if (!strcmp(key, "mg_coarse")) { m->mgc_opt = (int)v; if (m->const_set) return build_coefs(m); }
  else if (!strcmp(key, "mgc_pfused")) { m->mgc_pfused = (int)v; if (m->const_set) return build_coefs(m); }
  else if (!strcmp(key, "mg_coarse_dim")) { m->mgc_dim = (int)v; if (m->const_set) return build_coefs(m); }
  else if (int *o = kernel_opt(m->opt, key)) *o = (int)v;
  else if (!strcmp(key, "rhs_variant")) m->rhs_variant = (int)v;
  else if (!strcmp(key, "adv_fused")) m->adv_fused = (int)v;
  else if (!strcmp(key, "overlap")) m->overlap = (int)v;
  else if (!strcmp(key, "rhs_resid")) { m->rhs_resid = (int)v; m->res_ready = -1; }
  else if (!strcmp(key, "seed")) { m->seed = (unsigned)v; srand(m->seed); }
  else if (!strcmp(key, "noise_mode")) m->noise_mode = (int)v;
  else if (!strcmp(key, "stoch_fused")) m->stoch_fused = (int)v;
  else if (!strcmp(key, "stats")) {
    if ((int)v && !m->stats_mask) { msom_set_error("option stats = 1 before msom_stats_begin"); return MSOM_ERR_STATE; }
    m->stats_on = (int)v != 0;
  }
  else if (!strcmp(key, "stats_every")) {
    if (!(v >= 1)) { msom_set_error("option stats_every = %g", v); return MSOM_ERR_ARG; }
    m->stats_every = (int)v;
  }
  else if (!strcmp(key, "ckpt_steps")) {
    if (!(v >= 0)) { msom_set_error("option ckpt_steps = %g", v); return MSOM_ERR_ARG; }
    m->ckpt_steps = (int)v;
  }
  else if (!strcmp(key, "resume")) m->resume = (int)v != 0;
  else if (!strcmp(key, "tau_f")) {
    if (!(v > 0) || !std::isfinite(v)) { msom_set_error("option tau_f = %g", v); return MSOM_ERR_ARG; }
    m->tau_f = v;
  }
  else if (!strcmp(key, "modes_compact")) {
    if ((int)v != -1 && (int)v != 0) { msom_set_error("option modes_compact = %g (-1 or 0)", v); return MSOM_ERR_ARG; }
    m->modes_compact_opt = (int)v;
  }
  else if (!strcmp(key, "mode_pv_invert")) {
    if ((int)v != 0 && (int)v != 1) { msom_set_error("option mode_pv_invert = %g (0 or 1)", v); return MSOM_ERR_ARG; }
    if ((int)v && m->nranks > 1) {
      msom_set_error("option mode_pv_invert: the modal inversion runs on a single tile, this handle is one of %d", m->nranks);
      return MSOM_ERR_CONFIG;
    }
    m->mode_pv_invert = (int)v;
    m->res_ready = -1;
  }
  else if (!strcmp(key, "stochastic")) {
    m->stochastic = (int)v;
    if (m->stochastic && !m->f[MSOM_NOISE]) {
      for (int k : {MSOM_NOISE, MSOM_SIGMA}) {
        size_t bytes = m->g.ls * m->nl * sizeof(double);
        HIPCHK(hipMalloc(&m->f[k], bytes));
        HIPCHK(hipMemsetAsync(m->f[k], 0, bytes, m->st));
      }
    }
  } else {
    msom_set_error("unknown option %s", key);
    return MSOM_ERR_ARG;
  }
  return MSOM_OK;
}

static int march_levels(const msom *m);
static int march_kmax(const msom *m);
static bool march_lean_fine(const msom *m);
static bool fine_visit_fused(const msom *m);
static int level_path(const msom *m, int k);
static bool restrict2_ok(const msom *m);
static bool rhs_resid_emits(const msom *m);
extern "C" double msom_get_param(msom_t *m, const char *key) {
  if (!m || !key) return NAN;
  if (!strcmp(key, "model")) return m->model;
  if (m->model) return nq_get_param(m, key);
  const Params &p = m->p;
  if (!strcmp(key, "N") || !strcmp(key, "nx")) return m->gnx;
  if (!strcmp(key, "ny")) return m->gny;
  if (!strcmp(key, "nl")) return m->nl;
  if (!strcmp(key, "nptr")) return p.nptr;
  if (!strcmp(key, "L0")) return p.L0;
  if (!strcmp(key, "DT")) return p.DT;
  if (!strcmp(key, "iRe")) return p.iRe;
  if (!strcmp(key, "iRe4")) return p.iRe4;
  if (!strcmp(key, "CFL")) return p.CFL;
  if (!strcmp(key, "Rom")) return p.Rom;
  if (!strcmp(key, "tend")) return p.tend;
  if (!strcmp(key, "dtout")) return p.dtout;
  if (!strcmp(key, "beta")) return p.beta;
  if (!strcmp(key, "tau0")) return p.tau0;
  if (!strcmp(key, "Ekb")) return p.Ekb;
  if (!strcmp(key, "Eks")) return p.Eks;
  if (!strcmp(key, "sbc")) return p.sbc;
  if (!strcmp(key, "TOLERANCE")) return p.tolerance;
  if (!strcmp(key, "nlevels")) return m->nlev;
  if (!strcmp(key, "uniform_S")) return m->uniformS;
  if (!strcmp(key, "agg_level")) return m->agg_level;
  if (!strcmp(key, "overlap")) return m->overlap;
  if (!strcmp(key, "stats_mask")) return m->stats_mask;
  if (!strcmp(key, "stats_dev_samples")) return (double)m->stats_ndev;
  if (!strcmp(key, "stats_bytes")) {
    int n = m->stats_qme ? 1 : 0;
    for (int k = 0; k < MSOM_ST_NACC; k++) n += m->stats.s[k] ? 1 : 0;
    return (double)n * m->nl * m->nx * m->ny * sizeof(double);
  }
  if (!strcmp(key, "mode_pv_invert")) return m->mode_pv_invert;
  if (!strcmp(key, "modes_ready")) return m->const_set && m->modes_ready;
  if (!strcmp(key, "modes_compact")) return m->const_set && m->modes_ready ? m->modes_compact : (m->modes_compact_opt != 0 && m->fr_uniform);
  if (!strcmp(key, "spec_bytes")) return (double)m->spc_bytes;
  if (!strcmp(key, "spec_batch")) return m->spc_batch;
  if (!strcmp(key, "modes_bytes"))
    return m->modes_md ? (double)(m->nl * m->nl + m->nl) * m->nx * m->ny * sizeof(double) : 0.;
  if (!strcmp(key, "resmax_marching")) return m->uniformS && m->nl <= MSOM_FASTNL && m->g.nx >= 64 && m->g.ny >= 16 && m->opt.resmax_rows >= 0;
  if (!strcmp(key, "march_visit_ring")) return !fine_visit_fused(m) ? -1 : (m->opt.march_visit_ring >= 2 ? 2 : (m->opt.march_visit_ring == 1 ? 1 : 0));
  if (const int *o = kernel_opt(m->opt, key)) return *o;
  if (!strcmp(key, "rhs_resid")) return rhs_resid_emits(m);
  if (!strncmp(key, "split_ls_", 9)) { const int k = atoi(key + 9); return k >= 0 && k < m->nlev ? (double)m->sg[k].ls : NAN; }
  if (!strncmp(key, "split_rp_", 9)) { const int k = atoi(key + 9); return k >= 0 && k < m->nlev ? (double)m->sg[k].rp : NAN; }
  if (!strcmp(key, "split_pad")) return MSOM_SP;
  if (!strcmp(key, "restrict2")) return restrict2_ok(m);
  if (!strcmp(key, "mg_coarse_lean")) return m->mgc_first >= 0 && m->mgc_lean;
  if (!strcmp(key, "march_levels")) return march_levels(m);
  if (!strcmp(key, "march_min")) return m->march_min;
  if (!strcmp(key, "march_kmax")) return march_kmax(m);
  if (!strcmp(key, "march_lean_fine")) return march_lean_fine(m);
  if (!strcmp(key, "march_visit")) return fine_visit_fused(m);
  if (!strncmp(key, "relax_path_", 11)) { const int k = atoi(key + 11); return k >= 0 && k < m->nlev ? level_path(m, k) : NAN; }
  if (!strcmp(key, "split_ls")) return m->nlev > 0 ? (double)m->sg[0].ls : NAN;
  auto idx = [](const char *s, int n) { const int k = atoi(s); return k >= 0 && k < n ? k : -1; };
  if (!strncmp(key, "idh0_", 5)) { const int k = idx(key + 5, MSOM_MAXNL); return k < 0 ? NAN : m->lc.idh0[k]; }
  if (!strncmp(key, "idh1_", 5)) { const int k = idx(key + 5, MSOM_MAXNL); return k < 0 ? NAN : m->lc.idh1[k]; }
  if (!strncmp(key, "Fr_", 3)) { const int k = idx(key + 3, MSOM_MAXARR); return k < 0 ? NAN : p.Frm[k]; }
  if (!strncmp(key, "dh_", 3)) { const int k = idx(key + 3, MSOM_MAXARR); return k < 0 ? NAN : m->dhf[k]; }
  return NAN;
}


int check_field(msom *m, int field) {
  if (!m || field < 0 || field >= MSOM_NFIELDS || !m->f[field]) {
    msom_set_error("bad field id %d", field);
    return MSOM_ERR_ARG;
  }
  return MSOM_OK;
}

int fill_bc(msom *m, int field) {
  if (m->nranks > 1 && field != MSOM_Q && field != MSOM_DQ && field != MSOM_QPRED && field != MSOM_NOISE && field != MSOM_SIGMA &&
      !(field >= MSOM_BFN_F1 && field <= MSOM_BFN_GAIN)) {
    int r = exch_nat(m, m->f[field], m->flayers[field], m->fbc[field], 1);
    if (!r && m->fbc[field] == BC_DIRICHLET_LIN) {
      const int sides = (m->ix == 0 ? WALL_W : 0) | (m->ix == m->px - 1 ? WALL_E : 0) | (m->iy == 0 ? WALL_S : 0) | (m->iy == m->py - 1 ? WALL_N : 0);
      launch_fill_lin_dirichlet(m->st, m->f[field], m->g, m->flayers[field], m->p.upg, m->p.vpg, m->p.L0 / m->gnx, m->p.L0,
                                m->p.L0 * m->gny / m->gnx, m->ix * m->nx, m->iy * m->ny, sides);
    }
    return r;
  }
  if (m->fbc[field] == BC_PERIODIC) launch_fill_periodic(m->st, m->f[field], m->g, m->flayers[field], 1);
  else if (m->fbc[field] == BC_DIRICHLET_LIN)
    launch_fill_lin_dirichlet(m->st, m->f[field], m->g, m->flayers[field], m->p.upg, m->p.vpg, m->p.L0 / m->gnx, m->p.L0,
                              m->p.L0 * m->gny / m->gnx);
  else launch_fill_ghost(m->st, m->f[field], m->g, m->flayers[field], m->fbc[field], m->walls);
  return MSOM_OK;
}

int upload(msom *m, int field, const double *a) {
  m->res_ready = -1;
  const size_t n = (size_t)m->flayers[field] * m->nx * m->ny;
  HIPCHK(hipMemcpyAsync(m->staging, a, n * sizeof(double), hipMemcpyDefault, m->st));
  launch_pack(m->st, m->staging, m->f[field], m->g, m->flayers[field]);
  fill_bc(m, field);
  return MSOM_OK;
}
int download(msom *m, int field, double *a) {
  const size_t n = (size_t)m->flayers[field] * m->nx * m->ny;
  launch_unpack(m->st, m->f[field], m->staging, m->g, m->flayers[field]);
  HIPCHK(hipMemcpyAsync(a, m->staging, n * sizeof(double), hipMemcpyDefault, m->st));
  return sync_stream(m);
}

extern "C" int msom_field_layers(msom_t *m, int field) {
  if (m && m->model && !(field >= 0 && field < MSOM_NFIELDS && m->f[field])) return 0;
  if (check_field(m, field)) return MSOM_ERR_ARG;
  return m->flayers[field];
}

int ensure_field(msom *m, int field) {
  if (m->f[field]) return MSOM_OK;
  const size_t bytes = m->g.ls * m->flayers[field] * sizeof(double);
  HIPCHK(hipMalloc(&m->f[field], bytes));
  HIPCHK(hipMemsetAsync(m->f[field], 0, bytes, m->st));
  return MSOM_OK;
}
extern "C" int msom_set_field(msom_t *m, int field, const double *a) {
  if (m && !m->model && (field == MSOM_QOF || (field >= MSOM_DE_BF && field < MSOM_NFIELDS)) && ensure_field(m, field)) return MSOM_ERR_HIP;
  if (check_field(m, field) || !a) return MSOM_ERR_ARG;
  int r = upload(m, field, a);
  if (r) return r;
  if (m->model && (r = nq_after_upload(m, field))) return r;
  if (field == MSOM_RD) m->wv_ready = 0;
  if (field == MSOM_FR || field == MSOM_RO || field == MSOM_S) { m->fr_uniform = 0; m->const_set = 0; }
  if (field == MSOM_PSIPG) { m->have_pg = 1; m->const_set = 0; }
  if (field == MSOM_ZETAPG) m->have_zpg = 1;
  if (field == MSOM_QFORC) m->have_qforc = 1;
  if (field == MSOM_TOPO) m->flag_topo = 1;
  if (field == MSOM_BFN_OBS) m->bfn_obs_set = 1;
  if (field == MSOM_BFN_GAIN) m->bfn_gain_set = 1;
  return sync_stream(m);
}
extern "C" int msom_get_field(msom_t *m, int field, double *a) {
  if (m && !m->model && (field == MSOM_QOF || (field >= MSOM_DE_BF && field < MSOM_NFIELDS)) && ensure_field(m, field)) return MSOM_ERR_HIP;
  if (check_field(m, field) || !a) return MSOM_ERR_ARG;
  return download(m, field, a);
}

extern "C" int msom_remove_mean(msom_t *m, int field) {
  MSQG_ONLY(m);
  if (check_field(m, field)) return MSOM_ERR_ARG;
  const int nl = m->flayers[field];
  m->res_ready = -1;
#ifdef MSOM_STRICT
  std::vector<double> mean(nl);
  if (m->nranks == 1) {
    std::vector<double> h((size_t)nl * m->nx * m->ny);
    int r = download(m, field, h.data());
    if (r) return r;
    const double D2 = (m->p.L0 / m->gnx) * (m->p.L0 / m->gnx);
    for (int l = 0; l < nl; l++) {
      double sum = 0, vol = 0;
      for (int i = 0; i < m->nx; i++)
        for (int j = 0; j < m->ny; j++) { sum += h[((size_t)l * m->ny + j) * m->nx + i] * D2; vol += D2; }
      mean[l] = sum / vol;
    }
    HIPCHK(hipMemcpyAsync(m->d_scal + SC_LSUM, mean.data(), nl * sizeof(double), hipMemcpyHostToDevice, m->st));
    launch_sub_layer_const(m->st, m->f[field], m->d_scal + SC_LSUM, m->g, nl, 1.);
    fill_bc(m, field);
    return sync_stream(m);
  }
#endif
  launch_sum_layers(m->st, m->f[field], m->partial, m->d_scal + SC_LSUM, m->g, nl);
  if (m->nranks > 1) {
    int r = reduce_scal(m, SC_LSUM, nl, RED_SUM);
    if (r) return r;
  }
  launch_sub_layer_const(m->st, m->f[field], m->d_scal + SC_LSUM, m->g, nl, 1. / ((double)m->gnx * m->gny));
  fill_bc(m, field);
  return sync_stream(m);
}


static void make_relax_coef(msom *m, int k) {
  RelaxCoef &rc = m->rc[k];
  memset(&rc, 0, sizeof rc);
  const int nl = m->nl;
  rc.D = m->p.L0 / (double)(m->gnx >> k);
  rc.sqD = rc.D * rc.D;
  for (int l = 0; l < nl; l++) { rc.idh0[l] = m->lc.idh0[l]; rc.idh1[l] = m->lc.idh1[l]; }
  if (nl < 2) { rc.it1[0] = 0.25; return; }
  double t0[MSOM_MAXNL], t1[MSOM_MAXNL], t2[MSOM_MAXNL];
  for (int l = 0; l < nl - 1; l++) {
    const double r = m->s_zero ? 0. : m->p.Frm[l] / m->p.Rom;
    rc.S[l] = r * r;
  }
  for (int l = 0; l < nl; l++) {
    t0[l] = l > 0 ? -rc.sqD * rc.S[l - 1] * rc.idh0[l] : 0.;
    t2[l] = l < nl - 1 ? -rc.sqD * rc.S[l] * rc.idh1[l] : 0.;
    t1[l] = -t0[l] - t2[l] + 4.;
  }
  for (int l = 1; l < nl; l++) t1[l] -= t0[l] * t2[l - 1] / t1[l - 1];
  for (int l = 0; l < nl; l++) {
// ... 127 lines not shown
  const int auto_uniform = 0;
#else
  const int auto_uniform = 1;
#endif
  m->uniformS = (m->uniform_opt < 0 ? auto_uniform : m->uniform_opt) && m->fr_uniform && nl > 1;
  for (int k = 0; k < m->nlev; k++) make_relax_coef(m, k);
  {
    int r = setup_agglomeration(m);
    if (r) return r;
    if ((r = setup_mg_coarse(m))) return r;
  }
  {
    std::vector<double> w(m->ny);
    for (int j = 0; j < m->ny; j++) {
      const double y = (m->iy * m->ny + j + 0.5) * D;
      w[j] = p.tau0 / (p.Rom * m->dhf[0]) * sin(2 * M_PI * y / p.L0) * sin(M_PI * y / p.L0);
    }
    HIPCHK(hipMemcpyAsync(m->d_wind, w.data(), m->ny * sizeof(double), hipMemcpyHostToDevice, m->st));
    HIPCHK(hipStreamSynchronize(m->st));
  }
  return MSOM_OK;
}

extern "C" int msom_set_const(msom_t *m) {
  if (m) m->res_ready = -1;
  if (!m) return MSOM_ERR_ARG;
  if (m->model) return nq_set_const(m);
  m->s_zero = 0;
  int rr = build_coefs(m);
  if (rr) return rr;
  m->wv_ready = 0;
  const Params &p = m->p;
  const int nl = m->nl;
  const double D = p.L0 / m->gnx;
  launch_del2(m->st, m->f[MSOM_PSI], m->f[MSOM_Q], m->g, nl, 0., 1., D);
  launch_stretch(m->st, m->f[MSOM_PSI], m->f[MSOM_Q], m->f[MSOM_S], m->g, nl, 1., 1., m->lc);
  fill_bc(m, MSOM_Q);
  if (p.flsrv == 1) {
    launch_del2(m->st, m->f[MSOM_PSIPG], m->f[MSOM_ZETAPG], m->g, nl, 0., 1., D);
    fill_bc(m, MSOM_ZETAPG);
    m->have_zpg = 1;
  }
  for (int l = 0; l < MSOM_MAXNL; l++) m->umax_pg[l] = 0.;
  if (m->have_pg) {
    launch_umax(m->st, m->f[MSOM_PSIPG], m->partial_umax, m->d_scal + SC_UMAX, m->g, nl, D);
    int r = reduce_scal(m, SC_UMAX, nl, RED_MAX);
    if (r) return r;
    for (int l = 0; l < nl; l++) m->umax_pg[l] = m->h_scal[SC_UMAX + l];
  }
  m->const_set = 1;
  m->bfn_begun = 0;
  stats_drop(m);
  modes_drop(m);
  spec_drop(m);
  m->helm_solved = 0;
  if (m->helm_pm) HIPCHK(hipMemsetAsync(m->helm_pm, 0, m->g.ls * nl * sizeof(double), m->st));
  if (m->mode_pv_invert) {
    if ((rr = msom_modes_compute(m))) return rr;
    if (nl > 1 && (rr = msom_modes_set_rd(m, 1))) return rr;
  }
  return sync_stream(m);
}


Lev tile_lev(const msom *m, int k) {
  return Lev{const_cast<double **>(&m->da[k]), const_cast<double **>(&m->da_alt[k]), m->res[k], m->S[k], &m->sg[k], &m->rc[k], m->walls, m->nranks > 1, k == 0, k};
}
static Lev glob_lev(const msom *m, int k) {
  const int q = k - m->agg_level;
  return Lev{const_cast<double **>(&m->gda[q]), const_cast<double **>(&m->gda_alt[q]), m->gres[q], nullptr, &m->gsg[q], &m->rc[k], m->bc == BC_PERIODIC ? WALL_PER : WALL_ALL, false, false, -1};
}

enum { RP_COLOUR = 0, RP_BLOCK2 = 1, RP_BLOCK8 = 2, RP_MARCH = 3, RP_COARSE = 4, RP_GATHERED = 8 };
static bool layered_fusions(const msom *m) { return !m->mode_pv_invert; }
static bool rhs_resid_on(const msom *m) {
  return m->rhs_resid > 0 || (m->rhs_resid < 0 && m->rhs_variant == 6 && (size_t)m->g.nx * m->g.ny * m->nl >= ((size_t)1 << RHS_RESID_MIN));
}
static bool rhs_resid_variant(const msom *m) {
#ifdef MSOM_STRICT
  return m->rhs_variant == 1 || m->rhs_variant == 6;
#else
  return m->rhs_variant == 6;
#endif
}
static bool rhs_resid_emits(const msom *m) {
  return rhs_resid_on(m) && m->fused && m->adv_fused && m->nl <= MSOM_FASTNL && !m->have_pg && !m->have_zpg && !m->flag_topo && !m->stochastic &&
         layered_fusions(m) && rhs_resid_variant(m) && m->mg_fused && m->nlev > 1 && m->bc != BC_PERIODIC && m->nranks == 1 &&
         !(m->g.nx & 1) && !(m->g.ny & 1);
}
static int sweep_path(const msom *m, const Lev &L) {
  const SplitGeom &g = *L.sg;
  if (!layered_fusions(m)) return RP_COLOUR;
  if (m->march && !m->block_sweeps && (m->uniformS || m->nl == 1) && m->nl <= MSOM_FASTNL && g.nx >= 512 && g.ny >= 64 &&
      (L.tiled || L.walls == WALL_ALL || (L.walls == WALL_PER && L.k >= 0)) &&
      (m->march >= 2 || (size_t)g.nx * g.ny * m->nl >= ((size_t)1 << (L.tiled ? m->march_min_tiled : m->march_min))))
    return RP_MARCH;
  if (m->block8 && !m->block_sweeps && (m->uniformS || m->nl == 1 || L.S) && m->nl <= MSOM_FASTNL && !L.tiled && g.nx >= 64 && g.ny >= 16 &&
      g.nx <= m->block8_max && (L.walls == WALL_ALL || (L.walls == WALL_PER && L.k >= 0 && g.ny >= 64)))
    return RP_BLOCK8;
  if ((m->block_sweeps || (m->block_small && g.nx <= m->block_small)) && m->uniformS && m->nl <= MSOM_FASTNL && !L.tiled &&
      !(m->walls & WALL_PER) && g.nx >= 64 && g.ny >= 16)
    return RP_BLOCK2;
  return RP_COLOUR;
}
static int level_path(const msom *m, int k) {
  if (m->mgc_first >= 0 && k >= m->mgc_first) return RP_COARSE;
  if (m->agg_level >= 0 && k >= m->agg_level) return RP_GATHERED + sweep_path(m, glob_lev(m, k));
  return sweep_path(m, tile_lev(m, k));
}
static int march_levels(const msom *m) {
  int n = 0;
  for (int k = 0; k < m->nlev; k++) n += level_path(m, k) == RP_MARCH;
  return n;
}
static bool march_lean_fine(const msom *m) {
  return m->nlev > 0 && m->opt.march_lean && level_path(m, 0) == RP_MARCH && march_lean_fits(m->nl, m->sg[0], &m->g);
}
static bool fuse_prolong(const msom *m, const Lev &L, int nrelax) {
  const int path = sweep_path(m, L);
  if (path == RP_BLOCK2 && nrelax >= 2) return true;
  if (path == RP_BLOCK8 && nrelax >= 1) return true;
  return m->prolong_fused && m->nl <= MSOM_FASTNL && nrelax >= 1 && L.sg->nx >= 4 && L.sg->ny >= 4;
}
static bool corr_wanted(const msom *m) { return m->mg_fused && m->nlev > 1 && m->march_correct; }

static int march_kmax(const msom *m) { return m->nl >= 7 && m->march_k > 3 ? 3 : m->march_k; }

enum { MA_DONE, MA_VISIT, MA_PL, MA_REDPROL, MA_PASS, MA_HALF };
struct MarchAct { int kind, K; bool corr, partial; };
static MarchAct march_next(const msom *m, const Lev &L, const Lev *coarse, int n, bool corr_req) {
  const int kmax = march_kmax(m), nl = m->nl;
  const bool deep = L.tiled || (L.walls & WALL_PER);
  auto pass = [&](int kind, int kmin, bool corr_ok) {
    int K = n < kmax ? n : kmax;
    if (n - K == 1 && K > kmin) K--;
    return MarchAct{kind, K, corr_ok && n == K, m->march_partial && n - K >= 1};
  };
  if (coarse && n > 0) {
    const bool pl_tiled = coarse->k >= 0 && nl <= 6 && m->march_prolong >= 1 && coarse->sg->nx >= 2 * MARCH_HALO && coarse->sg->ny >= 2 * MARCH_HALO;
    if (n < 3 || kmax < 3 || !m->march_prolong || (deep && !pl_tiled)) return MarchAct{MA_REDPROL, 1, false, false};
    if (n == 8 && kmax == 4 && L.fine && corr_req && m->march_visit && m->opt.march_dma && m->uniformS && nl >= 2 && m->march_partial &&
        (m->march_visit >= 2 || (size_t)L.sg->nx * L.sg->ny * nl >= ((size_t)1 << m->march_visit_min)) && !L.tiled && L.walls == WALL_ALL &&
        march_lean_fine(m) && relax_visit_fits(nl, *L.sg, m->opt.march_visit_rows, m->opt.march_visit_pairs))
      return MarchAct{MA_VISIT, 8, true, false};
    return pass(MA_PL, 3, false);
  }
  if (n >= 2) return pass(MA_PASS, 2, corr_req && L.fine);
  return MarchAct{n == 1 ? MA_HALF : MA_DONE, n, false, false};
}
static bool fine_visit_fused(const msom *m) {
  if (m->nlev < 2 || level_path(m, 0) != RP_MARCH) return false;
  const Lev L = tile_lev(m, 0), C = tile_lev(m, 1);
  return march_next(m, L, fuse_prolong(m, L, 4) ? &C : nullptr, 8, corr_wanted(m)).kind == MA_VISIT;
}

static bool march_halo(msom *m, int k, bool wrap, bool res, MarchHalo *h) {
  const auto arrays = {&m->mh_da_s, &m->mh_da_n, &m->mh_res_s, &m->mh_res_n};
  if (m->mh_da_s.size() < (size_t)m->nlev)
    for (auto *v : arrays) v->assign(m->nlev, nullptr);
  const size_t ls = make_split(m->sg[k].nx, MARCH_HALO).ls, bytes = ls * m->nl * sizeof(double);
  if (!m->mh_da_s[k])
    for (auto *v : arrays) {
      if (hipMalloc(&(*v)[k], bytes) != hipSuccess) { m->sticky = MSOM_ERR_HIP; return false; }
      hipMemsetAsync((*v)[k], 0, bytes, m->st);
    }
  const bool s = wrap || m->nb[DIR_S] >= 0, n = wrap || m->nb[DIR_N] >= 0;
  *h = MarchHalo{s ? m->mh_da_s[k] : nullptr, n ? m->mh_da_n[k] : nullptr, s && res ? m->mh_res_s[k] : nullptr, n && res ? m->mh_res_n[k] : nullptr, ls, MARCH_HALO};
  return true;
}
template <class Launch, class Halos>
static void march_pass(msom *m, bool overlap, ProfSlot *ps, Launch launch, Halos halos) {
  if (ps) prof_begin(m, *ps);
  if (overlap) {
    comm_begin(m); m->comm_hold = 1;
    launch(1);
    halos();
    m->comm_hold = 0; comm_end(m);
    launch(2);
  } else {
    halos();
    launch(0);
  }
  if (ps) prof_end(m, *ps);
}

void relax_sweeps(msom *m, Lev &L, const Lev *coarse, int nrelax, int corners_last) {
  const bool prof = m->profile && L.fine;
  const int nl = m->nl;
  const int path = sweep_path(m, L);
  int it = 0;
  if (path == RP_MARCH) {
    const bool wrap = !L.tiled && (L.walls & WALL_PER), deep = L.tiled || wrap;
    const int kwalls = wrap ? 0 : L.walls;
    auto fill_halo = [&](int k, bool res) {
      double *f = res ? m->res[k] : m->da[k], *fs = res ? m->mh_res_s[k] : m->mh_da_s[k], *fn = res ? m->mh_res_n[k] : m->mh_da_n[k];
      const SplitGeom hgeo = make_split(m->sg[k].nx, MARCH_HALO);
      if (L.tiled) STICKY(m, exch_split_deep(m, f, m->sg[k], fs, fn, hgeo, nl));
      else { launch_split_wrap(m->st, f, m->sg[k], fs, fn, hgeo, nl, MARCH_HALO, 0); launch_split_wrap(m->st, f, m->sg[k], fs, fn, hgeo, nl, MARCH_HALO, 1); }
    };
    MarchHalo mh{nullptr, nullptr, nullptr, nullptr, 0, MARCH_HALO}, ch = mh;
    if (deep && !march_halo(m, L.k, wrap, true, &mh)) return;
    const bool ovl = L.tiled && m->overlap;
    bool res_halo = deep;
    const MarchCorrect mc{m->f[MSOM_PSI], m->psi_alt, m->g};
    const Lev *src = coarse;
    int n = 2 * nrelax, c = 0;
    for (;;) {
      const MarchAct a = march_next(m, L, src, n, m->corr_req);
      if (a.kind == MA_HALF || a.kind == MA_DONE) break;
      if (a.kind == MA_VISIT) {
        if (prof) prof_begin(m, m->prof_march_visit);
        if (launch_relax_visit(m->st, m->opt, *L.da, *L.da_alt, L.res, *L.sg, nl, *L.rc, kwalls, *src->da, *src->sg, mc))
          m->sticky = MSOM_ERR_ARG;
        if (prof) prof_end(m, m->prof_march_visit);
        m->corr_done = 1;
        return;
      } else if (a.kind == MA_REDPROL) {
        if (prof) prof_begin(m, m->prof_redprol);
        launch_relax_red_prolong(m->st, m->opt, *L.da, *src->da, *src->sg, L.res, L.S, *L.sg, nl, *L.rc, m->uniformS, L.walls);
        if (prof) prof_end(m, m->prof_redprol);
      } else {
        const Lev *pl = a.kind == MA_PL ? src : nullptr;
        if (pl && deep && !march_halo(m, pl->k, wrap, false, &ch)) return;
        march_pass(m, ovl, !prof ? nullptr : (pl ? &m->prof_march_pl : (a.corr ? &m->prof_march_corr : &m->prof_march[a.K])),
                   [&](int region) {
                     if (launch_relax_march(m->st, m->opt, pl ? nullptr : *L.da, *L.da_alt, L.res, *L.sg, nl, *L.rc, c, a.K, kwalls, m->opt.march_rows, deep ? &mh : nullptr,
                                            pl ? *pl->da : nullptr, pl ? pl->sg : nullptr, a.corr ? &mc : nullptr, a.partial, pl && deep ? &ch : nullptr, region))
                       m->sticky = MSOM_ERR_ARG;
                   },
                   [&]() {
                     if (res_halo) fill_halo(L.k, true);
                     res_halo = false;
                     if (deep) fill_halo(pl ? pl->k : L.k, false);
                   });
        if (a.corr) { m->corr_done = 1; return; }
        std::swap(*L.da, *L.da_alt);
      }
      src = nullptr; n -= a.K; c = (c + a.K) & 1;
    }
    if (wrap) launch_split_wrap(m->st, *L.da, *L.sg, nullptr, nullptr, make_split(L.sg->nx, MARCH_HALO), nl, MARCH_HALO, 2);
    if (n == 1) {
      if (L.tiled) STICKY(m, exch_split(m, *L.da, *L.sg, nl, 0));
      launch_relax_color(m->st, *L.da, L.res, L.S, *L.sg, nl, *L.rc, m->uniformS, c, L.walls, L.fine);
    }
    if (L.tiled) STICKY(m, exch_split(m, *L.da, *L.sg, nl, corners_last));
    return;
  }
  if (path == RP_BLOCK8) {
    int n = 2 * nrelax, c = 0;
    const Lev *src = coarse;
    while (n > 0) {
      const int K = n < 8 ? n : 8;
      if (K == 1) { launch_relax_color(m->st, *L.da, L.res, L.S, *L.sg, nl, *L.rc, m->uniformS, c, L.walls, L.fine); break; }
      if (launch_relax_block8(m->st, m->opt, *L.da, src ? *src->da : nullptr, src ? *src->sg : *L.sg, L.res, *L.da_alt, *L.sg, nl, *L.rc, L.walls, K, c, m->uniformS ? nullptr : L.S)) m->sticky = MSOM_ERR_ARG;
      std::swap(*L.da, *L.da_alt);
      src = nullptr; n -= K; c = (c + K) & 1;
      if (L.walls & WALL_PER) launch_split_wrap(m->st, *L.da, *L.sg, nullptr, nullptr, make_split(L.sg->nx, MARCH_HALO), nl, MARCH_HALO, 2);
    }
    return;
  }
  if (path == RP_BLOCK2) {
    for (; it + 2 <= nrelax; it += 2) {
      const bool pl = coarse && it == 0;
      if (prof && !pl) prof_begin(m, m->prof_block);
      launch_relax_block2(m->st, m->opt, *L.da, pl ? *coarse->da : nullptr, pl ? *coarse->sg : *L.sg, L.res, *L.da_alt, *L.sg, nl, *L.rc, L.walls, L.fine);
      if (prof && !pl) prof_end(m, m->prof_block);
      std::swap(*L.da, *L.da_alt);
    }
  }
  for (; it < nrelax; it++) {
    const bool pl = coarse && it == 0;
    if (prof && !pl) prof_begin(m, m->prof_sweep);
    for (int c = 0; c < 2; c++) {
      const int corners = corners_last && it == nrelax - 1 && c == 1;
      if (L.tiled && m->overlap && !(pl && c == 0) && !corners && L.sg->nx >= 32 && L.sg->ny >= 8) {
        launch_relax_ring(m->st, *L.da, L.res, L.S, *L.sg, nl, *L.rc, m->uniformS, c, L.walls);
        comm_begin(m);
        STICKY(m, exch_split_raw(m, *L.da, *L.sg, nl, 0));
        launch_relax_color(m->st, *L.da, L.res, L.S, *L.sg, nl, *L.rc, m->uniformS, c, L.walls, L.fine, 1);
        comm_end(m);
        continue;
      }
      if (pl && c == 0) {
        if (prof) prof_begin(m, m->prof_redprol);
        launch_relax_red_prolong(m->st, m->opt, *L.da, *coarse->da, *coarse->sg, L.res, L.S, *L.sg, nl, *L.rc, m->uniformS, L.walls);
        if (prof) prof_end(m, m->prof_redprol);
      } else
        launch_relax_color(m->st, *L.da, L.res, L.S, *L.sg, nl, *L.rc, m->uniformS, c, L.walls, L.fine);
      if (L.tiled) STICKY(m, exch_split(m, *L.da, *L.sg, nl, corners));
    }
    if (prof && !pl) prof_end(m, m->prof_sweep);
  }
}

static void level_solve(msom *m, Lev &L, const Lev *coarse, int nrelax, int corners_last) {
  const int nl = m->nl;
  bool fused = false;
  if (!coarse) hipMemsetAsync(*L.da, 0, L.sg->ls * nl * sizeof(double), m->st);
  else if (fuse_prolong(m, L, nrelax)) fused = true;
  else {
    launch_prolong(m->st, *coarse->da, *coarse->sg, *L.da, *L.sg, nl, L.walls);
    if (L.tiled) STICKY(m, exch_split(m, *L.da, *L.sg, nl, 0));
  }
  relax_sweeps(m, L, fused ? coarse : nullptr, nrelax, corners_last);
}

// ... 25 lines not shown
  }
  if (glob) {
    const SplitGeom &tg = m->sg[kc];
    const size_t cnt = (size_t)nl * tg.nx * tg.ny;
    launch_split_unpack(m->st, m->res[kc], tg, m->agg_send, nl);
    comm_begin(m);
    STICKY(m, comm_allgather(m->comm, m->agg_send, m->agg_recv, cnt));
    comm_end(m);
    launch_assemble_global(m->st, m->agg_recv, m->gres[0], m->gsg[0], nl, tg.nx, tg.ny, m->px);
    const int gtop = kg >= 0 ? kg : m->nlev - 1;
    for (int k = kc + 1; k <= gtop; k++) launch_restrict(m->st, m->gres[k - 1 - kc], m->gsg[k - 1 - kc], m->gres[k - kc], m->gsg[k - kc], nl);
    if (kg >= 0) {
      launch_mg_coarse(m->st, m->d_cargs, nrelax, nl, m->uniformS, m->mgc_lean);
      if (hipGetLastError() != hipSuccess && !m->sticky) m->sticky = MSOM_ERR_HIP;
    }
    for (int k = (kg >= 0 ? kg : m->nlev) - 1; k >= kc; k--) {
      Lev L = glob_lev(m, k);
      if (k == m->nlev - 1) level_solve(m, L, nullptr, nrelax, 0);
      else { Lev C = glob_lev(m, k + 1); level_solve(m, L, &C, nrelax, 0); }
    }
    launch_extract_tile(m->st, m->gda[0], m->gsg[0], m->da[kc], tg, nl, m->ix * tg.nx, m->iy * tg.ny);
  } else if (kg >= 0) {
    launch_mg_coarse(m->st, m->d_cargs, nrelax, nl, m->uniformS, m->mgc_lean);
    if (hipGetLastError() != hipSuccess && !m->sticky) m->sticky = MSOM_ERR_HIP;
  }
  for (int k = (glob ? kc : (kg >= 0 ? kg : m->nlev)) - 1; k >= 0; k--) {
    Lev L = tile_lev(m, k);
    if (k == m->nlev - 1) level_solve(m, L, nullptr, nrelax, k > 0);
    else { Lev C = tile_lev(m, k + 1); level_solve(m, L, &C, nrelax, k > 0); }
  }
}

static void clear_graphs(msom *m) {
  for (auto &kv : m->cyc_graph) (void)hipGraphExecDestroy(kv.second);
  m->cyc_graph.clear();
}
static void mg_cycle(msom *m, int nrelax, int first_restrict) {
  bool ok = m->use_graph && m->nranks == 1 && !m->profile;
  for (int k = 0; ok && k < m->nlev; k++) {
    Lev L = tile_lev(m, k);
    if (sweep_path(m, L) != RP_COLOUR) ok = false;
  }
  if (!ok) { mg_cycle_levels(m, nrelax, first_restrict); return; }
  const long key = (long)nrelax * 8 + first_restrict;
  auto it = m->cyc_graph.find(key);
  if (it == m->cyc_graph.end()) {
    hipGraph_t g = nullptr;
    hipGraphExec_t ex = nullptr;
    if (hipStreamBeginCapture(m->st, hipStreamCaptureModeThreadLocal) != hipSuccess) { m->use_graph = 0; mg_cycle_levels(m, nrelax, first_restrict); return; }
    mg_cycle_levels(m, nrelax, first_restrict);
    if (hipStreamEndCapture(m->st, &g) != hipSuccess || !g || hipGraphInstantiate(&ex, g, nullptr, nullptr, 0) != hipSuccess) {
      if (g) (void)hipGraphDestroy(g);
      (void)hipGetLastError();
      m->use_graph = 0;
      mg_cycle_levels(m, nrelax, first_restrict);
      return;
    }
    (void)hipGraphDestroy(g);
    it = m->cyc_graph.emplace(key, ex).first;
  }
  if (hipGraphLaunch(it->second, m->st) != hipSuccess && !m->sticky) m->sticky = MSOM_ERR_HIP;
}

void residual(msom *m, const double *a, const double *b, int slot, int want_sum) {
  if (m->profile) prof_begin(m, m->prof_resid);
  launch_residual(m->st, a, b, m->f[MSOM_S], m->g, m->res[0], m->sg[0], m->nl, m->rc[0], m->uniformS, m->d_scal + slot, m->partial, want_sum);
  if (m->profile) prof_end(m, m->prof_resid);
}
static bool restrict2_ok(const msom *m) { return m->restrict2 && m->mg_fused && m->nlev > 2 && m->g.ny % 4 == 0 && m->sg[0].hk % 2 == 0; }
void residual2(msom *m, int mode, const double *b, int slot, int want_sum) {
  ProfSlot &which = (mode & 8) ? m->prof_resmax : (mode & 1) ? m->prof_rescorr : m->prof_respre;
  if (m->profile) { prof_begin(m, m->prof_resid); prof_begin(m, which); }
  const bool r2 = (mode & 4) && restrict2_ok(m);
  launch_residual2(m->st, m->opt, mode, m->f[MSOM_PSI], m->da[0], m->psi_alt, b, m->f[MSOM_S], m->g, m->res[0], m->sg[0],
                   m->nlev > 1 ? m->res[1] : nullptr, m->sg[m->nlev > 1 ? 1 : 0], m->nl, m->rc[0], m->uniformS, m->walls, m->d_scal + slot,
                   m->partial, want_sum, m->partial_umax, m->d_scal + SC_UMAX, m->umax_clean, r2 ? m->res[2] : nullptr, r2 ? &m->sg[2] : nullptr);
  if (mode & (1 | 8)) m->umax_clean = 0;
  if (m->profile) { prof_end(m, m->prof_resid); prof_end(m, which); }
}

static int read_residuals(msom *m) {
  if (m->nranks == 1) {
    if (m->dbg_nosync) return MSOM_OK;
    if (m->spec_launched) {
      volatile long *seq = reinterpret_cast<volatile long *>(m->h_pub + SC_COUNT);
      const double t0 = wall_seconds();
      while (*seq != m->pub_seq) {
        if (wall_seconds() - t0 > 5.) {
          HIPCHK(hipStreamSynchronize(m->st));
          if (*seq != m->pub_seq) { msom_set_error("the device did not publish the solver's scalars"); return MSOM_ERR_HIP; }
        }
      }
      __atomic_thread_fence(__ATOMIC_ACQUIRE);
      memcpy(m->h_scal, m->h_pub, SC_COUNT * sizeof(double));
      return MSOM_OK;
    }
    HIPCHK(hipMemcpyAsync(m->h_scal, m->d_scal, SC_COUNT * sizeof(double), hipMemcpyDeviceToHost, m->st));
    HIPCHK(hipStreamSynchronize(m->st));
    return MSOM_OK;
  }
  int r = reduce_scal(m, SC_RES0, 2 + m->nl, RED_MAX);
  if (r) return r;
  if (m->nranks > 1 && !m->mg_global_sum) {
    HIPCHK(hipMemcpyAsync(m->h_scal + SC_BSUM, m->d_scal + SC_BSUM, sizeof(double), hipMemcpyDeviceToHost, m->st));
    HIPCHK(hipStreamSynchronize(m->st));
    return MSOM_OK;
  }
  return reduce_scal(m, SC_BSUM, 1, RED_SUM);
}

static int mg_solve(msom *m, const double *b, msom_mgstats *s) {
  const Params &p = m->p;
  const bool fused = m->mg_fused && m->nlev > 1;
  s->i = 0; s->nrelax = 4;
  HIPCHK(hipMemsetAsync(m->d_scal, 0, (SC_UMAX + MSOM_MAXNL) * sizeof(double), m->st));
  m->umax_clean = 1;
  m->umax_ready = 0;
  const bool have_res = fused && m->res_ready >= 0 && b == m->f[m->res_ready];
  m->res_ready = -1;
  if (have_res) {
    HIPCHK(hipMemcpyAsync(m->d_scal + SC_RES0, m->d_scal + SC_RESF, sizeof(double), hipMemcpyDeviceToDevice, m->st));
    launch_sum_final(m->st, m->partial_rr, m->d_scal + SC_BSUM, m->rr_nparts);
  } else if (fused) {
    residual2(m, 2 | 4, b, SC_RES0, 1);
    launch_sum_final(m->st, m->partial, m->d_scal + SC_BSUM, residual2_blocks(m->g));
  } else {
    residual(m, m->f[MSOM_PSI], b, SC_RES0, 1);
    launch_sum_final(m->st, m->partial, m->d_scal + SC_BSUM, partial_count(m->g));
  }
  if (m->psi_ghosts_stale) {
    m->psi_ghosts_stale = 0;
    fill_bc(m, MSOM_PSI);
  }
  bool have_first = false;
  double resb = 0;
  if (p.nitermin < 1) {
    int rr = read_residuals(m);
    if (rr) return rr;
    resb = s->resb = s->resa = m->h_scal[SC_RES0];
    s->sum = m->h_scal[SC_BSUM];
    have_first = true;
  }
  for (s->i = 0; s->i < p.nitermax && (s->i < p.nitermin || s->resa > p.tolerance); s->i++) {
    m->corr_req = corr_wanted(m);
    m->corr_done = 0;
    mg_cycle(m, s->nrelax, fused ? ((restrict2_ok(m) && !(have_res && s->i == 0)) ? 3 : 2) : 1);
    m->corr_req = 0;
    if (s->i > 0) HIPCHK(hipMemsetAsync(m->d_scal + SC_RES1, 0, sizeof(double), m->st));
    if (m->corr_done) {
      std::swap(m->f[MSOM_PSI], m->psi_alt);
      if (m->nranks > 1) STICKY(m, exch_nat(m, m->f[MSOM_PSI], m->nl, m->bc, 1));
      else if (m->bc == BC_PERIODIC) launch_fill_periodic(m->st, m->f[MSOM_PSI], m->g, m->nl, 1);
      else launch_fill_ghost(m->st, m->f[MSOM_PSI], m->g, m->nl, m->bc, m->walls);
      residual2(m, 8, b, SC_RES1, 0);
      m->umax_ready = 1;
    } else if (fused) {
      residual2(m, 1, b, SC_RES1, 0);
      std::swap(m->f[MSOM_PSI], m->psi_alt);
      m->umax_ready = 1;
      if (m->nranks > 1) STICKY(m, exch_nat(m, m->f[MSOM_PSI], m->nl, m->bc, 1));
    } else {
      launch_correct(m->st, m->f[MSOM_PSI], m->g, m->da[0], m->sg[0], m->nl, m->walls);
      if (m->nranks > 1) STICKY(m, exch_nat(m, m->f[MSOM_PSI], m->nl, m->bc, 1));
      residual(m, m->f[MSOM_PSI], b, SC_RES1, 0);
    }
    if (s->i == 0 && m->spec_hook && m->umax_ready && m->nranks == 1) {
      m->spec_hook([&]() {});
      m->spec_launched = 1;
    }
    int rr = read_residuals(m);
    if (rr) { m->spec_launched = 0; return rr; }
    if (m->spec_launched) {
      const double ra = m->h_scal[SC_RES1];
      m->spec_valid = !(s->i + 1 < p.nitermax && (s->i + 1 < p.nitermin || ra > p.tolerance));
      m->spec_launched = 0;
    }
    if (!have_first) {
      resb = s->resb = m->h_scal[SC_RES0];
      s->sum = m->h_scal[SC_BSUM];
      have_first = true;
    }
    s->resa = m->h_scal[SC_RES1];
    if (s->resa > p.tolerance) {
      if (resb / s->resa < 1.2 && s->nrelax < 100) s->nrelax++;
      else if (resb / s->resa > 10 && s->nrelax > 2) s->nrelax--;
    }
    resb = s->resa;
    if (fused && s->i + 1 < p.nitermax && (s->i + 1 < p.nitermin || s->resa > p.tolerance)) residual2(m, 2 | 4, b, SC_SCRATCH, 0);
  }
  if (!have_first) {
    int rr = read_residuals(m);
    if (rr) return rr;
    s->resb = s->resa = m->h_scal[SC_RES0];
    s->sum = m->h_scal[SC_BSUM];
  }
  if (s->resa > p.tolerance && !m->quiet)
    fprintf(stderr, "WARNING: convergence not reached after %d iterations\n  res: %g sum: %g nrelax: %d\n", s->i, s->resa, s->sum, s->nrelax);
  return MSOM_OK;
}

int invertq(msom *m, const double *q) {
  if (m->mode_pv_invert) return helm_solve(m, q);
  return mg_solve(m, q, &m->mg);
}


double limiter(msom *m, double umax, double dtmax) {
  const double D = m->p.L0 / m->gnx;
  dtmax /= m->p.CFL;
  if (umax != 0.) {
    const double dt = D / umax;
    if (dt < dtmax) dtmax = dt;
  }
  dtmax *= m->p.CFL;
  if (dtmax > m->previous) dtmax = (m->previous + 0.1 * dtmax) / 1.1;
  m->previous = dtmax;
  return dtmax;
}

void comp_del2(msom *m, int in, int out, double add, double fac) {
  const double D = m->p.L0 / m->gnx;
  launch_del2(m->st, m->f[in], m->f[out], m->g, m->nl, add, fac, D);
  fill_bc(m, out);
  if (m->p.sbc > 0) launch_slip_bc(m->st, m->f[in], m->f[out], m->g, m->nl, m->p.sbc / ((0.5 * m->p.sbc + 1) * D * D), m->walls);
}
void comp_stretch(msom *m, int in, int out, double add, double fac) {
  launch_stretch(m->st, m->f[in], m->f[out], m->f[MSOM_S], m->g, m->nl, add, fac, m->lc);
  fill_bc(m, out);
}

static int stoch_prepare(msom *m, double dt, double *dts);
int rhs_terms(msom *m, int qfield, int dqfield, int with_qforcing, double iRe, double iRe4, double Eks, double Ekb, int adv_out,
                     int adv_in, double adv_dt, int *advanced) {
  if (advanced) *advanced = 0;
  const Params &p = m->p;
  const double D = p.L0 / m->gnx;
  const int nl = m->nl;
#ifdef MSOM_STRICT
  const bool stoch_fused = false;
#else
  const bool stoch_fused = m->stochastic && m->stoch_fused && m->adv_fused && adv_out >= 0 && m->rhs_variant == 6;
#endif
  if (m->fused && m->nl <= MSOM_FASTNL && !m->have_pg && !m->have_zpg && !m->flag_topo && (!m->stochastic || stoch_fused) &&
      (m->nranks == 1 || (m->nx >= 4 && m->ny >= 4))) {
    if (m->bc == BC_PERIODIC && m->nranks == 1) launch_fill_periodic(m->st, m->f[MSOM_PSI], m->g, nl, 3);
    if (!m->adv_fused) adv_out = -1;
    const int variant = m->rhs_variant;
    const bool use_rr = adv_out >= 0 && rhs_resid_emits(m);
    RhsResid rr;
    if (use_rr) {
      rr.res = m->res[0]; rr.res_c = m->res[1]; rr.res_max = m->d_scal + SC_RESF; rr.bsum_partial = m->partial_rr;
      rr.sg = m->sg[0]; rr.cg = m->sg[1];
    }
    auto with_psi_halo = [&](bool splittable, auto launch) {
      if (m->nranks > 1 && m->overlap && splittable) {
        comm_begin(m); m->comm_hold = 1;
        launch(1);
        STICKY(m, exch_nat(m, m->f[MSOM_PSI], nl, m->bc, 3));
        m->comm_hold = 0; comm_end(m);
        launch(2);
      } else {
        if (m->nranks > 1) STICKY(m, exch_nat(m, m->f[MSOM_PSI], nl, m->bc, 3));
        launch(0);
      }
    };
    if (stoch_fused) {
      double dts;
      int r = stoch_prepare(m, adv_dt, &dts);
      if (r) return r;
      m->res_ready = -1;
      prof_begin(m, m->prof_rhs);
      with_psi_halo(true, [&](int region) {
        launch_rhs_lpw(m->st, m->opt, m->f[MSOM_PSI], m->f[MSOM_S], m->f[MSOM_QFORC], m->d_wind, nullptr, m->g, nl, m->walls & WALL_ALL, m->uniformS,
                       m->rc[0].S, with_qforcing && m->have_qforc, D, p.beta, iRe, iRe4, Eks / (p.Rom * 2 * m->dhf[0]),
                       Ekb / (p.Rom * 2 * m->dhf[nl - 1]), p.sbc > 0 ? p.sbc / ((0.5 * p.sbc + 1) * D * D) : 0., m->lc, m->f[adv_in],
                       m->f[adv_out], adv_dt, 1, m->f[qfield], m->f[MSOM_NOISE], -adv_dt * p.itr_stoch, dts, region);
      });
      prof_end(m, m->prof_rhs);
      if (advanced) *advanced = 1;
      return MSOM_OK;
    }
    prof_begin(m, m->prof_rhs);
    with_psi_halo(variant == 6, [&](int region) {
      launch_rhs_fused(m->st, m->opt, m->f[MSOM_PSI], m->f[MSOM_S], m->f[MSOM_QFORC], m->d_wind, m->f[dqfield], nullptr,
                       nullptr, m->g, nl, m->walls & WALL_ALL, m->uniformS, m->rc[0].S, with_qforcing && m->have_qforc, D, p.beta, iRe,
                       iRe4, Eks / (p.Rom * 2 * m->dhf[0]), Ekb / (p.Rom * 2 * m->dhf[nl - 1]),
                       p.sbc > 0 ? p.sbc / ((0.5 * p.sbc + 1) * D * D) : 0., m->lc, variant, adv_out >= 0 ? m->f[adv_in] : nullptr,
                       adv_out >= 0 ? (m->adv_out_override ? m->adv_out_override : m->f[adv_out]) : nullptr, adv_dt, use_rr ? &rr : nullptr, region,
                       variant == 6 ? m->dt_dev : nullptr);
    });
    prof_end(m, m->prof_rhs);
    if (use_rr) {
      m->res_ready = adv_out;
      m->rr_nparts = variant == 6 ? rhs_lpw_blocks(m->opt, m->g, nl) : rhs_pipe_blocks(m->g);
    }
    if (advanced && adv_out >= 0) *advanced = 1;
    return MSOM_OK;
  }
  HIPCHK(hipMemsetAsync(m->f[dqfield], 0, m->g.ls * nl * sizeof(double), m->st));
  comp_del2(m, MSOM_PSI, MSOM_ZETA, 0., 1.0);
  launch_advection(m->st, m->f[MSOM_ZETA], m->f[MSOM_PSI], m->f[MSOM_PSIPG], m->f[MSOM_ZETAPG], m->f[MSOM_S], m->f[qfield], m->f[dqfield],
                   m->g, nl, m->have_pg, m->have_zpg, m->stochastic, D, p.beta, p.itr_stoch, m->lc);
  if (iRe != 0) comp_stretch(m, MSOM_ZETA, dqfield, 1., iRe);
  if (iRe != 0 || iRe4 != 0) comp_del2(m, MSOM_ZETA, MSOM_TMP, 0., 1.);
  if (iRe != 0) launch_axpy(m->st, m->f[dqfield], m->f[MSOM_TMP], m->g, nl, iRe);
  if (iRe4 != 0) {
    comp_stretch(m, MSOM_TMP, dqfield, 1., iRe4);
    comp_del2(m, MSOM_TMP, dqfield, 1., iRe4);
  }
  launch_forcing(m->st, m->f[MSOM_ZETA], m->f[MSOM_PSI], m->f[MSOM_QFORC], m->f[MSOM_TOPO], m->f[MSOM_RO], m->d_wind, m->f[dqfield], m->g,
                 nl, with_qforcing && m->have_qforc, m->flag_topo, Eks / (p.Rom * 2 * m->dhf[0]), Ekb / (p.Rom * 2 * m->dhf[nl - 1]), D,
                 m->dhf[nl - 1]);
  return MSOM_OK;
}

static int tracer_update(msom *m, int cfield);

struct StepDtArgs { double umax_pg[MSOM_MAXNL]; double D, CFL, previous, dtmax, t, tnext; int nl, with_dt; long seq; };
__global__ void __launch_bounds__(64) k_step_dt(double *scal, StepDtArgs a, double *pub) {
#pragma clang fp contract(off)
  if (threadIdx.x == 0 && a.with_dt) {
  const double *umax = scal + SC_UMAX;
  double *out = scal + SC_SPEC;
  double dtmax = a.dtmax, previous = a.previous;
  for (int k = 0; k < 2 * a.nl; k++) {
    const double u = (k & 1) ? a.umax_pg[k >> 1] : umax[k >> 1];
    dtmax /= a.CFL;
    if (u != 0.) {
      const double dt = a.D / u;
      if (dt < dtmax) dtmax = dt;
    }
    dtmax *= a.CFL;
    if (dtmax > previous) dtmax = (previous + 0.1 * dtmax) / 1.1;
    previous = dtmax;
  }
  double dt = dtmax, tnext = a.tnext;
  if (tnext != HUGE_VAL && tnext > a.t) {
    const unsigned int n = (unsigned int)((tnext - a.t) / dt);
    if (n == 0) dt = tnext - a.t;
    else {
      const double dt1 = (tnext - a.t) / n;
      if (dt1 > dt * (1. + 1e-9)) dt = (tnext - a.t) / (n + 1);
      else if (dt1 < dt) dt = dt1;
      tnext = a.t + dt;
    }
  } else
    tnext = a.t + dt;
  out[0] = dtmax; out[1] = dt; out[2] = tnext; out[3] = dt / 2.;
  }
  __syncthreads();
  if (pub) {
    pub[threadIdx.x] = scal[threadIdx.x];
    __threadfence_system();
    __syncthreads();
    if (threadIdx.x == 0) __atomic_store_n(reinterpret_cast<long *>(pub + SC_COUNT), a.seq, __ATOMIC_RELEASE);
  }
}
static_assert(SC_COUNT == 64, "k_step_dt publishes one slot per thread");

static double solve_and_dt(msom *m, int qfield, double dtmax) {
  const int nl = m->nl;
  m->spec_valid = 0;
  if (invertq(m, m->f[qfield])) return -1;
  if (m->spec_valid && m->dt_dev) {
    m->previous = m->h_scal[SC_SPEC];
    return m->h_scal[SC_SPEC];
  }
  if (!m->umax_ready) {
    launch_umax(m->st, m->f[MSOM_PSI], m->partial_umax, m->d_scal + SC_UMAX, m->g, nl, m->p.L0 / m->gnx);
    if (reduce_scal(m, SC_UMAX, nl, RED_MAX)) return -1;
  }
  if (m->sticky) return -1;
  for (int l = 0; l < nl; l++) {
    dtmax = limiter(m, m->h_scal[SC_UMAX + l], dtmax);
    dtmax = limiter(m, m->umax_pg[l], dtmax);
  }
  return dtmax;
}

static double update_qg(msom *m, int qfield, int dqfield, double dtmax) {
  const Params &p = m->p;
  dtmax = solve_and_dt(m, qfield, dtmax);
  if (dtmax < 0) return -1;
  if (rhs_terms(m, qfield, dqfield, 1, p.iRe, p.iRe4, p.Eks, p.Ekb)) return -1;
  if (p.nptr > 0 && tracer_update(m, qfield == MSOM_QPRED ? MSOM_PTR_PRED : MSOM_PTR)) return -1;
  return dtmax;
}

static int generate_noise_host(msom *m) {
  const int nl = m->nl, nx = m->nx, ny = m->ny;
  std::vector<double> sig((size_t)nl * nx * ny), n((size_t)nl * nx * ny);
  int r = download(m, MSOM_SIGMA, sig.data());
  if (r) return r;
  for (int i = 0; i < nx; i++)
    for (int j = 0; j < ny; j++)
      for (int l = 0; l < nl; l++) {
        const double a = sqrt(-2. * log(((double)(rand()) + 1.) / ((double)(RAND_MAX) + 2.)));
        const double nn = a * cos(2 * M_PI * rand() / (double)RAND_MAX);
        const size_t k = ((size_t)l * ny + j) * nx + i;
        n[k] = m->p.amp_stoch * sig[k] * nn;
      }
  return upload(m, MSOM_NOISE, n.data());
}

static int stoch_prepare(msom *m, double dt, double *dts) {
// ... 101 lines not shown
  if (!m->const_set || !m->helm_solved) { msom_set_error("msom_modes_mgstats: no modal solve since msom_set_const"); return MSOM_ERR_STATE; }
  if (mode < 0 || mode >= m->nl) { msom_set_error("msom_modes_mgstats: mode %d outside 0 .. %d", mode, m->nl - 1); return MSOM_ERR_ARG; }
  *st = m->helm.s[mode];
  return MSOM_OK;
}


int check_shape(msom *m, int a, int b, int c) {
  if (a != m->nl || b != m->ny || c != m->nx) {
    msom_set_error("array shape (%d,%d,%d) != (nl,N,N) = (%d,%d,%d)", a, b, c, m->nl, m->ny, m->nx);
    return MSOM_ERR_ARG;
  }
  return MSOM_OK;
}

extern "C" int pystep_bfn(msom_t *m, double *varin_py, int len1, int len2, int len3, double *tend_py, int len4, int len5, int len6,
                          double direction, int vartype) {
  if (m) m->res_ready = -1;
  MSQG_ONLY(m);
  NEED_CONST(m);
  if (check_shape(m, len1, len2, len3) || check_shape(m, len4, len5, len6)) return MSOM_ERR_ARG;
  Params &p = m->p;
  int r;
  if (direction > 0) {
    p.iRe = p.Re == 0 ? 0. : 1 / p.Re;
    p.iRe4 = p.Re4 == 0 ? 0. : -1 / p.Re4;
    p.Eks = fabs(p.Eks); p.Ekb = fabs(p.Ekb);
  } else {
    p.iRe = p.Re == 0 ? 0. : -1 / p.Re;
    p.iRe4 = p.Re4 == 0 ? 0. : 1 / p.Re4;
    p.Eks = -fabs(p.Eks); p.Ekb = -fabs(p.Ekb);
  }
  if (vartype != 1) HIPCHK(hipMemsetAsync(m->f[MSOM_DQ], 0, m->g.ls * m->nl * sizeof(double), m->st));
  if (vartype == 1) {
    if ((r = upload(m, MSOM_Q, varin_py))) return r;
    if (solve_and_dt(m, MSOM_Q, p.DT) < 0) return MSOM_ERR_HIP;
    if ((r = rhs_terms(m, MSOM_Q, MSOM_DQ, 0, p.iRe, p.iRe4, p.Eks, p.Ekb))) return r;
  } else if (!m->quiet)
    fprintf(stdout, "temporary disabled psi tendency\n");
  return download(m, MSOM_DQ, tend_py);
}
extern "C" int pyq2p(msom_t *m, double *po_py, int len7, int len8, int len9, double *qo_py, int len10, int len11, int len12) {
  MSQG_ONLY(m);
  NEED_CONST(m);
  if (check_shape(m, len7, len8, len9) || check_shape(m, len10, len11, len12)) return MSOM_ERR_ARG;
  int r;
  m->res_ready = -1;
  HIPCHK(hipMemsetAsync(m->f[MSOM_PSI], 0, m->g.ls * m->nl * sizeof(double), m->st));
  if ((r = upload(m, MSOM_Q, qo_py))) return r;
  if ((r = invertq(m, m->f[MSOM_Q]))) return r;
  return download(m, MSOM_PSI, po_py);
}
extern "C" int pyp2q(msom_t *m, double *po_py, int len13, int len14, int len15, double *qo_py, int len16, int len17, int len18) {
  if (m) m->res_ready = -1;
  MSQG_ONLY(m);
  NEED_CONST(m);
  if (check_shape(m, len13, len14, len15) || check_shape(m, len16, len17, len18)) return MSOM_ERR_ARG;
  return msom_comp_q(m, po_py, qo_py);
}


extern "C" int msom_bfn_begin(msom_t *m) {
  if (m) m->res_ready = -1;
  MSQG_ONLY(m);
  NEED_CONST(m);
  int r;
  for (int k = MSOM_BFN_F1; k <= MSOM_BFN_F3; k++) {
    if ((r = ensure_field(m, k))) return r;
    HIPCHK(hipMemsetAsync(m->f[k], 0, m->g.ls * m->nl * sizeof(double), m->st));
  }
  m->bfn_begun = 1;
  return sync_stream(m);
}

extern "C" int msom_bfn_steps(msom_t *m, int nsteps, double dt, double direction, double k) {
  MSQG_ONLY(m);
  if (!m) return MSOM_ERR_ARG;
  if (nsteps < 0) { msom_set_error("msom_bfn_steps: nsteps = %d", nsteps); return MSOM_ERR_ARG; }
  if (!m->const_set || !m->bfn_begun) { msom_set_error("msom_bfn_steps before msom_bfn_begin"); return MSOM_ERR_STATE; }
  if (k != 0 && !m->bfn_obs_set) { msom_set_error("msom_bfn_steps: k != 0 and MSOM_BFN_OBS was never set"); return MSOM_ERR_STATE; }
  if (nsteps == 0) return MSOM_OK;
  Params &p = m->p;
  int r;
  if (direction > 0) {
    p.iRe = p.Re == 0 ? 0. : 1 / p.Re;
    p.iRe4 = p.Re4 == 0 ? 0. : -1 / p.Re4;
    p.Eks = fabs(p.Eks); p.Ekb = fabs(p.Ekb);
  } else {
    p.iRe = p.Re == 0 ? 0. : -1 / p.Re;
    p.iRe4 = p.Re4 == 0 ? 0. : 1 / p.Re4;
    p.Eks = -fabs(p.Eks); p.Ekb = -fabs(p.Ekb);
  }
  const double dt12 = dt / 12;
  const double *obs = k != 0 ? m->f[MSOM_BFN_OBS] : nullptr, *gain = (k != 0 && m->bfn_gain_set) ? m->f[MSOM_BFN_GAIN] : nullptr;
  for (int n = 0; n < nsteps; n++) {
    if (solve_and_dt(m, MSOM_Q, p.DT) < 0) return m->sticky ? m->sticky : MSOM_ERR_HIP;
    if ((r = rhs_terms(m, MSOM_Q, MSOM_BFN_F1, 0, p.iRe, p.iRe4, p.Eks, p.Ekb))) return r;
    launch_bfn_ab3(m->st, m->f[MSOM_Q], m->f[MSOM_BFN_F1], m->f[MSOM_BFN_F2], m->f[MSOM_BFN_F3], obs, gain, m->g, m->nl, dt12, k);
    fill_bc(m, MSOM_Q);
    m->res_ready = -1;
    m->umax_ready = 0;
    m->spec_valid = 0;
    double *f1 = m->f[MSOM_BFN_F1];
    m->f[MSOM_BFN_F1] = m->f[MSOM_BFN_F3];
    m->f[MSOM_BFN_F3] = m->f[MSOM_BFN_F2];
    m->f[MSOM_BFN_F2] = f1;
  }
  return sync_stream(m);
}

extern "C" int msom_bfn_misfit(msom_t *m, double *misfit) {
  MSQG_ONLY(m);
  if (!m || !misfit) return MSOM_ERR_ARG;
  if (!m->bfn_obs_set) { msom_set_error("msom_bfn_misfit: MSOM_BFN_OBS was never set"); return MSOM_ERR_STATE; }
  if (!m->bfn_partial) HIPCHK(hipMalloc(&m->bfn_partial, 2 * ((size_t)bfn_misfit_blocks(m->g) + 64) * sizeof(double)));
  launch_bfn_misfit(m->st, m->f[MSOM_Q], m->f[MSOM_BFN_OBS], m->bfn_gain_set ? m->f[MSOM_BFN_GAIN] : nullptr, m->bfn_partial,
                    m->d_scal + SC_LSUM, m->g, m->nl);
  int r = reduce_scal(m, SC_LSUM, 2, RED_SUM);
  if (r) return r;
  *misfit = sqrt(m->h_scal[SC_LSUM] / m->h_scal[SC_LSUM + 1]);
  return MSOM_OK;
}


double dtnext(msom *m, double dt, double *tnext_out) {
  double tnext = m->tnext, t = m->t;
  if (tnext != HUGE_VAL && tnext > t) {
    unsigned int n = (unsigned int)((tnext - t) / dt);
    if (n == 0) dt = tnext - t;
    else {
      double dt1 = (tnext - t) / n;
      if (dt1 > dt * (1. + 1e-9)) dt = (tnext - t) / (n + 1);
      else if (dt1 < dt) dt = dt1;
      tnext = t + dt;
    }
  } else
    tnext = t + dt;
  *tnext_out = tnext;
  return dt;
}

static int tracer_update(msom *m, int cfield) {
  const int nt = m->nl * m->p.nptr;
  HIPCHK(hipMemsetAsync(m->f[MSOM_DPTR], 0, m->g.ls * nt * sizeof(double), m->st));
  launch_ptr_rhs(m->st, m->f[MSOM_PSI], m->f[cfield], m->f[MSOM_PTR_RELAX], m->f[MSOM_DPTR], m->g, m->nl, m->p.nptr, m->p.iPe, m->p.ptr_ir,
                 m->p.L0 / m->gnx);
  return MSOM_OK;
}
static int tracer_advance(msom *m, int out, int in, double dt) {
  launch_advance(m->st, m->f[out], m->f[in], m->f[MSOM_DPTR], nullptr, m->g, m->nl * m->p.nptr, dt, 0.);
  return fill_bc(m, out);
}

static bool spec_ok(msom *m) {
  return layered_fusions(m) && m->async_solve && m->nranks == 1 && m->fused && m->adv_fused && m->rhs_variant == 6 && m->mg_fused && m->nlev > 1 &&
         m->nl <= MSOM_FASTNL && !m->have_pg && !m->have_zpg && !m->flag_topo && !m->stochastic && m->p.nptr == 0 && m->p.nitermin >= 1 && !m->dbg_nosync;
}

extern "C" int msom_step(msom_t *m, double *dt_used) {
  if (m && m->model) return nq_step(m, dt_used);
  NEED_CONST(m);
  if (m->stats_on && !m->stats_mask) { msom_set_error("msom_step: option stats = 1 and no msom_stats_begin since msom_set_const"); return MSOM_ERR_STATE; }
  const Params &p = m->p;
  double tnext;
  int r, advanced = 0;
  const bool spec = spec_ok(m);
  int spec_rc = 0;
  if (spec) {
    m->dt_dev = m->d_scal + SC_SPEC + 3;
    m->spec_hook = [&](const std::function<void()> &host_read) {
      StepDtArgs a;
      for (int l = 0; l < MSOM_MAXNL; l++) a.umax_pg[l] = m->umax_pg[l];
      a.D = p.L0 / m->gnx; a.CFL = p.CFL; a.previous = m->previous; a.dtmax = p.DT; a.t = m->t; a.tnext = m->tnext; a.nl = m->nl;
      a.with_dt = 1; a.seq = ++m->pub_seq;
      hipLaunchKernelGGL(k_step_dt, dim3(1), dim3(64), 0, m->st, m->d_scal, a, m->d_pub);
      host_read();
      int adv = 0;
      spec_rc = rhs_terms(m, MSOM_Q, MSOM_DQ, 1, p.iRe, p.iRe4, p.Eks, p.Ekb, MSOM_QPRED, MSOM_Q, 0., &adv);
      if (!adv && !spec_rc) spec_rc = MSOM_ERR_STATE;
    };
  }
  const double d = solve_and_dt(m, MSOM_Q, p.DT);
  m->spec_hook = nullptr;
  const bool hit1 = spec && m->spec_valid && !spec_rc;
  m->dt_dev = nullptr;
  if (!hit1) m->res_ready = -1;
  if (d < 0) return m->sticky ? m->sticky : MSOM_ERR_HIP;
  if (hit1) {
    m->dt = m->h_scal[SC_SPEC + 1];
    tnext = m->h_scal[SC_SPEC + 2];
  } else {
    m->dt = dtnext(m, d, &tnext);
    if ((r = rhs_terms(m, MSOM_Q, MSOM_DQ, 1, p.iRe, p.iRe4, p.Eks, p.Ekb, MSOM_QPRED, MSOM_Q, m->dt / 2., &advanced))) return r;
    if (!advanced && (r = advance_qg(m, MSOM_QPRED, MSOM_Q, MSOM_DQ, m->dt / 2.))) return r;
  }
  if (m->stats_on && m->stats_count++ % m->stats_every == 0) {
    stats_sample(m, hit1 ? m->d_scal + SC_SPEC + 1 : nullptr, m->dt);
    m->stats_ndev += hit1;
  }
  const bool tracers = m->p.nptr > 0;
  if (tracers && ((r = tracer_update(m, MSOM_PTR)) || (r = tracer_advance(m, MSOM_PTR_PRED, MSOM_PTR, m->dt / 2.)))) return r;
  spec_rc = 0;
  if (spec) {
    if (!m->q_alt) {
      HIPCHK(hipMalloc(&m->q_alt, m->g.ls * m->nl * sizeof(double)));
      HIPCHK(hipMemcpyAsync(m->q_alt, m->f[MSOM_Q], m->g.ls * m->nl * sizeof(double), hipMemcpyDeviceToDevice, m->st));
    }
    m->spec_hook = [&](const std::function<void()> &host_read) {
      StepDtArgs a;
      memset(&a, 0, sizeof a);
      a.with_dt = 0; a.seq = ++m->pub_seq;
      hipLaunchKernelGGL(k_step_dt, dim3(1), dim3(64), 0, m->st, m->d_scal, a, m->d_pub);
      host_read();
      int adv = 0;
      m->adv_out_override = m->q_alt;
      spec_rc = rhs_terms(m, MSOM_QPRED, MSOM_DQ, 1, p.iRe, p.iRe4, p.Eks, p.Ekb, MSOM_Q, MSOM_Q, m->dt, &adv);
      m->adv_out_override = nullptr;
      if (!adv && !spec_rc) spec_rc = MSOM_ERR_STATE;
    };
  }
  const double d2 = solve_and_dt(m, MSOM_QPRED, m->dt);
  m->spec_hook = nullptr;
  if (d2 < 0) return m->sticky ? m->sticky : MSOM_ERR_HIP;
  const bool rr2 = m->res_ready == MSOM_Q;
  m->res_ready = -1;
  if (spec && m->spec_valid && !spec_rc) {
    std::swap(m->f[MSOM_Q], m->q_alt);
    if (rr2) m->res_ready = MSOM_Q;
  } else {
    if ((r = rhs_terms(m, MSOM_QPRED, MSOM_DQ, 1, p.iRe, p.iRe4, p.Eks, p.Ekb, MSOM_Q, MSOM_Q, m->dt, &advanced))) return r;
    if (!advanced && (r = advance_qg(m, MSOM_Q, MSOM_Q, MSOM_DQ, m->dt))) return r;
  }
  if (tracers && ((r = tracer_update(m, MSOM_PTR_PRED)) || (r = tracer_advance(m, MSOM_PTR, MSOM_PTR, m->dt)))) return r;
  const bool lazy = m->step_sync == 0 || (m->step_sync < 0 && (size_t)m->g.nx * m->g.ny * m->nl < ((size_t)1 << 23));
  if (!spec || !lazy) { if ((r = sync_stream(m))) return r; }
  else if (m->sticky) return m->sticky;
  m->t = tnext;
  m->iter++;
  if (dt_used) *dt_used = m->dt;
  return MSOM_OK;
}
extern "C" int msom_sync(msom_t *m) {
  if (!m) return MSOM_ERR_ARG;
  return sync_stream(m);
}
extern "C" int msom_set_tnext(msom_t *m, double tnext) {
  if (!m) return MSOM_ERR_ARG;
  m->tnext = tnext;
  return MSOM_OK;
}
extern "C" double msom_time(msom_t *m) { return m ? m->t : NAN; }
extern "C" int msom_iter(msom_t *m) { return m ? m->iter : -1; }

extern "C" double msom_ke(msom_t *m) {
  if (!m) return NAN;
  launch_ke(m->st, m->f[MSOM_PSI], m->partial, m->d_scal + SC_KE, m->g, m->p.L0 / m->gnx);
  if (reduce_scal(m, SC_KE, 1, RED_SUM)) return NAN;
  return -m->h_scal[SC_KE];
}


extern "C" int msom_set_device(int device) {
  HIPCHK(hipSetDevice(device));
  return MSOM_OK;
}

extern "C" int msom_comm_unique_id(void *id128) {
  if (!id128) return MSOM_ERR_ARG;
  return comm_unique_id(id128);
}
extern "C" msom_t *msom_create_tiled(const char *params_text, int px, int py, int rank, const void *id128) {
  if (!params_text || px < 1 || py < 1 || rank < 0 || rank >= px * py || (px * py > 1 && !id128)) {
    msom_set_error("msom_create_tiled: bad arguments");
    return nullptr;
  }
  Params p;
  msom_params_defaults(&p);
  msom_params_parse_text(&p, params_text);
  msom *m = create_common(p, px, py, rank, id128);
  if (m) m->params_text = params_text;
  return m;
}
extern "C" int msom_tile_info(msom_t *m, int *px, int *py, int *ix, int *iy, int *nx_local, int *ny_local) {
  MSQG_ONLY(m);
  if (!m) return MSOM_ERR_ARG;
  if (px) *px = m->px;
  if (py) *py = m->py;
  if (ix) *ix = m->ix;
  if (iy) *iy = m->iy;
  if (nx_local) *nx_local = m->nx;
  if (ny_local) *ny_local = m->ny;
  return MSOM_OK;
}
```

### msom_amd/csrc/msom_host.h

```cpp
#ifndef MSOM_HOST_H
#define MSOM_HOST_H

#include <math.h>
#include <stdio.h>
#include <stdlib.h>
#include <string.h>
#include <sys/stat.h>
#include <sys/types.h>
#include <time.h>

#include <algorithm>
#include <cmath>
#include <string>
#include <utility>
#include <functional>
#include <map>
#include <vector>

#include "comm.h"
#include "kernels.h"
#include "spec_inl.h"
#include "helm_inl.h"

#define HIPCHK(x)                                                                          \
  do {                                                                                     \
    hipError_t e__ = (x);                                                                  \
    if (e__ != hipSuccess) {                                                               \
      msom_set_error("HIP error %s at %s:%d (%s)", hipGetErrorString(e__), __FILE__, __LINE__, #x); \
      return MSOM_ERR_HIP;                                                                 \
    }                                                                                      \
  } while (0)
#define STICKY(m, call)                                  \
  do {                                                   \
    int r__ = (call);                                    \
    if (r__ && !(m)->sticky) (m)->sticky = r__;          \
  } while (0)

enum { SC_BSUM = 2, SC_KE = 3, SC_SCRATCH = 4, SC_RES0 = 6, SC_RES1 = 7, SC_UMAX = 8 , SC_RESF = 8 + MSOM_MAXNL , SC_LSUM = 32 , SC_SPEC = 48 , SC_COUNT = 64 };
static_assert(SC_RESF < SC_LSUM && SC_LSUM + MSOM_MAXNL <= SC_SPEC && SC_SPEC + 4 <= SC_COUNT, "scalar slots overlap");

struct ProfSlot {
  std::vector<hipEvent_t> ev;
  size_t used = 0;
  double total_ms = 0;
  long launches = 0;
};

struct msom {
  Params p;
  std::string params_text;
  int px = 1, py = 1, ix = 0, iy = 0, rank = 0, nranks = 1;
  int gnx = 0, gny = 0;
  int nx = 0, ny = 0;
  int walls = WALL_ALL;
  Comm *comm = nullptr;
  int sticky = MSOM_OK;
  int comm_hold = 0;
  int dbg_nosync = 0;
  KernelOpts opt;
  int async_solve = 1;
  int step_sync = -1;
  std::function<void(const std::function<void()> &)> spec_hook;
  int spec_launched = 0, spec_valid = 0;
  hipEvent_t ev_spec = nullptr;
  double *h_pub = nullptr, *d_pub = nullptr;
  long pub_seq = 0;
  double *q_alt = nullptr;
  double *adv_out_override = nullptr;
  const double *dt_dev = nullptr;
  int nb[8];
  int nl = 1, nlm = 1;
  int bc = BC_DIRICHLET0;
  double dhf[MSOM_MAXARR], dhc[MSOM_MAXARR];
  LayerCoef lc;
  NatGeom g;
  double *f[MSOM_NFIELDS];
  int flayers[MSOM_NFIELDS];
  int fbc[MSOM_NFIELDS];
  int nlev = 0;
  std::vector<SplitGeom> sg;
  std::vector<double *> da, da_alt, res, S;
  std::vector<double *> mh_da_s, mh_da_n, mh_res_s, mh_res_n;
  std::vector<RelaxCoef> rc;
  size_t max_split = 0;
  int agg_level = -1, agglomerate = 1, agg_size = 256;
  int mg_global_sum = 0;
  std::vector<SplitGeom> gsg;
  std::vector<double *> gda, gda_alt, gres;
  double *agg_send = nullptr, *agg_recv = nullptr;
  double *staging = nullptr;
  double *partial = nullptr;
  double *partial_rr = nullptr;
  double *partial_umax = nullptr;
  double *d_scal = nullptr, *h_scal = nullptr;
  double *d_wind = nullptr;
  double umax_pg[MSOM_MAXNL];
  int umax_ready = 0;
  hipStream_t st = nullptr;
  hipStream_t st2 = nullptr;
  hipEvent_t ev_c2x = nullptr, ev_x2c = nullptr;
  int overlap = 1;
  int const_set = 0, flag_topo = 0, have_pg = 0, have_zpg = 0, have_qforc = 0;
  int fr_uniform = 1, uniformS = 0, uniform_opt = -1 ;
  int stochastic = 0, corrector_step = 0, noise_mode = 0, stoch_fused = 1;
  int prolong_fused = 1;
  int block_sweeps = 0;
  int restrict_pyr = 1;
  int restrict2 = 1;
  int block8 = 1;
  int block8_max = 1024;
  int block_small = 0;
  int march = 1;
  int march_k = 4;
  int use_graph = 0;
  std::map<long, hipGraphExec_t> cyc_graph;
  int march_partial = 1;
  int march_min_tiled = 22;
  int march_min = 23;
  int march_correct = 1;
  int corr_req = 0, corr_done = 0;
  int march_visit = 1;
  int march_visit_min = 25;
  int march_prolong = 1;
  int mg_fused = 1;
  double *psi_alt = nullptr;
  int rhs_variant = 6;
  int fused = 1;
  unsigned seed = 1, noise_draw = 0;
  int quiet = 0;
  int wv_nlev = 0, wv_ready = 0;
  int wv_kt = 0, wv_gx = 0, wv_gy = 0;
  std::vector<std::vector<double>> wv_top_sig;
  double *wv_gsend = nullptr, *wv_grecv = nullptr;
  int nme_ft = 0;
  CoarseArgs *d_cargs = nullptr;
  int mgc_dim = MGC_MAXDIM;
  int mgc_pfused = 1;
  int umax_clean = 0;
  int mgc_first = -1, mgc_opt = 4;
  int mgc_lean = 0;
  int psi_ghosts_stale = 0;
  int res_ready = -1;
  int adv_fused = 1;
  int rhs_resid = -1;
  int rr_nparts = 0;
  int bfn_begun = 0;
  int bfn_obs_set = 0, bfn_gain_set = 0;
  double *bfn_partial = nullptr;
  unsigned stats_mask = 0;
  StatsAcc stats = {};
  double *stats_W = nullptr;
  double *stats_qme = nullptr;
  int stats_on = 0, stats_every = 1;
  long stats_count = 0;
  long stats_ndev = 0;
  double tau_f = 20;
  int modes_ready = 0;
  int modes_compact = 0;
  int modes_compact_opt = -1;
  ModeCoef modes_mc = {};
  double *modes_md = nullptr;
  double *modes_dev = nullptr;
  int *modes_flag = nullptr;
  double *modes_partial = nullptr;
  int mode_pv_invert = 0;
  std::vector<double *> helm_ibu;
  double *helm_pm = nullptr, *helm_qm = nullptr;
  double *helm_scal = nullptr;
  double *helm_partial = nullptr;
  HelmSolve helm = {};
  int helm_solved = 0;
  ProfSlot prof_helm_relax, prof_helm_resid, prof_helm_coarse;
  int spc_batch = 0;
  int spc_smax = 0;
  double2 *spc_z = nullptr, *spc_zt = nullptr;
  double2 *spc_tw = nullptr;
  double *spc_v = nullptr;
  double *spc_te = nullptr, *spc_res = nullptr;
  double *spc_hin = nullptr;
  double *spc_o2d = nullptr;
  size_t spc_bytes = 0;
  std::vector<long> spc_count;
  int s_zero = 0;
  std::vector<NatGeom> wv_g;
  std::vector<double *> wv_s, wv_r, wv_sig;
  int model = 0;
  NewqgParams nq = {};
  int nq_fused = 1;
  int nq_adv_fused = 1;
  int nq_rows = 0;
  int ckpt_steps = 0, resume = 0;
  long state_flip = -1;
  int run_loaded = 0, run_outdir = 0;
  double run_tout = 0, run_tflt = 0;
  double t = 0, dt = 1., tnext = HUGE_VAL, previous = 0;
  int iter = 0;
  msom_mgstats mg = {0, 0, 0, 0, 0};
  int profile = 0;
  ProfSlot prof_sweep, prof_resid, prof_block, prof_march[5];
  ProfSlot prof_march_pl;
  ProfSlot prof_march_visit;
  ProfSlot prof_march_corr, prof_resmax;
  ProfSlot prof_rhs, prof_redprol, prof_rescorr, prof_respre;
};

enum { HS_RES0 = 0, HS_RES1 = MSOM_MAXNL, HS_BSUM = 2 * MSOM_MAXNL, HS_COUNT = 3 * MSOM_MAXNL };

struct Lev {
  double **da, **da_alt;
  double *res;
  const double *S;
  const SplitGeom *sg;
  const RelaxCoef *rc;
  int walls;
  bool tiled;
  bool fine;
  int k;
};

#define MSQG_ONLY(m)                                  \
  do {                                                \
    if ((m) && (m)->model) return nq_refuse(__func__); \
  } while (0)
#define NEED_CONST(m)                                                    \
  do {                                                                   \
    if (!(m)) return MSOM_ERR_ARG;                                       \
    if (!(m)->const_set) {                                               \
      int r__ = msom_set_const(m);                                       \
      if (r__) return r__;                                               \
    }                                                                    \
  } while (0)
#define NEED_MODES(m, fn)                                                                   \
  do {                                                                                      \
    if (!(m)->const_set || !(m)->modes_ready) {                                             \
      msom_set_error(fn ": no successful msom_modes_compute since msom_set_const");         \
      return MSOM_ERR_STATE;                                                                \
    }                                                                                       \
  } while (0)

#pragma GCC visibility push(hidden)
int sync_stream(msom *m);
void prof_begin(msom *m, ProfSlot &ps);
void prof_end(msom *m, ProfSlot &ps);
void prof_collect(msom *m, ProfSlot &ps);
NatGeom make_nat(int nx, int ny);
void comm_begin(msom *m);
void comm_end(msom *m);
int reduce_scal(msom *m, int slot, int n, int op);
int exch_nat_g(msom *m, double *f, const NatGeom &g, int nl, int bc, int depth);
int exch_split(msom *m, double *f, const SplitGeom &sg, int nl, int corners);
msom *create_common(const Params &p0, int px, int py, int rank, const void *id128, const NewqgParams *nq = nullptr);
int check_field(msom *m, int field);
int ensure_field(msom *m, int field);
int fill_bc(msom *m, int field);
int upload(msom *m, int field, const double *a);
int download(msom *m, int field, double *a);
int build_coefs(msom *m);
Lev tile_lev(const msom *m, int k);
void relax_sweeps(msom *m, Lev &L, const Lev *coarse, int nrelax, int corners_last);
void residual(msom *m, const double *a, const double *b, int slot, int want_sum);
void residual2(msom *m, int mode, const double *b, int slot, int want_sum);
int invertq(msom *m, const double *q);
double limiter(msom *m, double umax, double dtmax);
void comp_del2(msom *m, int in, int out, double add, double fac);
void comp_stretch(msom *m, int in, int out, double add, double fac);
int rhs_terms(msom *m, int qfield, int dqfield, int with_qforcing, double iRe, double iRe4, double Eks, double Ekb, int adv_out = -1,
              int adv_in = -1, double adv_dt = 0., int *advanced = nullptr);
int check_shape(msom *m, int a, int b, int c);
double dtnext(msom *m, double dt, double *tnext_out);
void helm_drop_pyramid(msom *m);
int helm_partial_stride(const msom *m);
int helm_ensure(msom *m);
int helm_relax_level(msom *m, int k, int nhalf, const HelmCount &cnt, ProfSlot *ps);
int helm_residual(msom *m, const double *a, const double *b, int slot, int want_sum);
int helm_read(msom *m, double *h);
void helm_fill(msom *m, double *f);
int helm_run(msom *m, double *a, const double *b);
int helm_solve(msom *m, const double *q);
void stats_drop(msom *m);
void stats_sample(msom *m, const double *w_dev, double w);
void modes_drop(msom *m);
ModesLayers modes_layers(const msom *m);
const ModeCoef *modes_mc(const msom *m);
int modes_energy_launch(msom *m);
void spec_drop(msom *m);
int spec_guard(msom *m, const char *fn);
int spec_ensure(msom *m);
SpecIn spec_in_nat(const msom *m, int mode, const double *a, const double *b);
void spec_batch_2d(msom *m, const SpecIn &in, int cnt, int kind, double *o2d);
void spec_batch_1d(msom *m, int cnt);
int nq_refuse(const char *fn);
bool nq_has_field(int field);
int nq_alloc(msom *m);
int nq_set_option(msom *m, const char *key, double v);
double nq_get_param(msom *m, const char *key);
int nq_after_upload(msom *m, int field);
int nq_set_const(msom *m);
double nq_update(msom *m, const double *q, double *dqdt, double dtmax);
// ... 12 lines not shown
```

Measured before the change: 18.42 billion grid-point-updates/s.

## Fold closing residual and umax check into speculative tendency pass

Adds a 'closing' by-product to the fused tendency+advance kernel. During the speculative launch it computes the final-iteration residual max, and in mode 2 the per-layer velocity max, from values already held in shared memory. This removes the separate residual march over psi and q, which was a full extra read sweep. In mode 1 the march still runs but only computes umax from psi. The step_dt publication is reordered to follow the speculative rhs pass. The cost is extra shared memory, extra reductions and more register pressure in the LPW kernel.

```diff
diff --git a/msom_amd/csrc/kernels.h b/msom_amd/csrc/kernels.h
--- a/msom_amd/csrc/kernels.h
+++ b/msom_amd/csrc/kernels.h
@@ -120,6 +120,10 @@
   double *res_max;
   double *bsum_partial;
   SplitGeom sg, cg;
+  int cls = 0;
+  const double *cls_b = nullptr;
+  double *cls_max = nullptr;
+  double *cls_umax = nullptr;
 };
 int rhs_fused_blocks(const NatGeom &g);
 void launch_rhs_fused(hipStream_t st, const KernelOpts &o, const double *psi, const double *S, const double *qforc, const double *wind, double *dq,
diff --git a/msom_amd/csrc/kernels_lpw.hip b/msom_amd/csrc/kernels_lpw.hip
--- a/msom_amd/csrc/kernels_lpw.hip
+++ b/msom_amd/csrc/kernels_lpw.hip
@@ -8,9 +8,11 @@
 #ifdef MSOM_STRICT
 #define LPW_NV 3
 #define LPW_MAXW 8
+#define LPW_CLS_PARK(CLS) 0
 #else
 #define LPW_NV 2
 #define LPW_MAXW 12
+#define LPW_CLS_PARK(CLS) ((CLS) == 2 ? 3 : (CLS) == 1 ? 1 : 0)
 #endif
 
 struct LpwArgs {
@@ -31,8 +33,11 @@
   double Su[MSOM_MAXNL];
 };
 
-template <int R, bool UNI, bool QF, bool ADV, bool STOCH, bool EDGE, bool RES, int NV>
-__device__ __forceinline__ void lpw_body(const LpwArgs &a, double (&ring)[2][LPW_MAXW][R][NV][64], double &res_m, double &res_bs) {
+template <int R, bool UNI, bool QF, bool ADV, bool STOCH, bool EDGE, bool RES, int CLS, int NV>
+__device__ __forceinline__ void lpw_body(const LpwArgs &a, double (&ring)[2][LPW_MAXW][R][NV][64], double &res_m, double &res_bs, double &cls_m,
+                                         double &cls_u) {
+  constexpr int DS = RES ? LPW_NV : 0, XS = LPW_CLS_PARK(CLS) ? LPW_NV + 1 : 0;
+  constexpr bool PARK3 = LPW_CLS_PARK(CLS) == 3;
   const int lane = threadIdx.x & 63;
   const int wv = __builtin_amdgcn_readfirstlane((int)(threadIdx.x >> 6));
   const int nl = a.nl, nx = a.g.nx, ny = a.g.ny;
@@ -80,8 +85,11 @@
 #endif
   double pnext[R], qnext[R], qreg[R], fqreg[R], qsreg[STOCH ? R : 1], nzreg[STOCH ? R : 1];
   double xdA[R], ydA[R];
+  double breg[CLS == 2 ? R : 1];
 #pragma unroll
   for (int r = 0; r < R; r++) xdA[r] = ydA[r] = 0.;
+#pragma unroll
+  for (int r = 0; r < (CLS == 2 ? R : 1); r++) breg[r] = 0.;
 #pragma unroll
   for (int r = 0; r < R; r++) {
 #ifdef MSOM_STRICT
@@ -162,10 +170,16 @@
 #else
       const double fa = oddx ? dW : dE, fb = oddx ? dE : dW;
       const double x = fma(rD, fb, -(rD * fa));
-      xdA[r] = oddx ? -x : x;
-      ydA[r] = fma(rD, dS, -(rD * dN));
-#endif
-      ring[b][wv][r][NV - 1][lane] = Q[1] - P[1];
+      const double xd = oddx ? -x : x, yd = fma(rD, dS, -(rD * dN));
+      if (PARK3) { ring[b][wv][r][XS + 1][lane] = xd; ring[b][wv][r][XS + 2][lane] = yd; }
+      else { xdA[r] = xd; ydA[r] = yd; }
+      if (CLS) ring[b][wv][r][XS][lane] = fma(rD, dW, -(rD * dE));
+#endif
+      if (CLS == 2) {
+        const double u = fabs(DIVC(0.25 * (P[2] - P[0] + PL[2] - PL[0]), D, rD)), v = fabs(DIVC(0.25 * (PR[1] - PL[1] + PR[0] - PL[0]), D, rD));
+        if (out_ok && j < y1) cls_u = fmax(cls_u, fmax(u, v));
+      }
+      ring[b][wv][r][DS][lane] = Q[1] - P[1];
     }
 #ifdef MSOM_STRICT
     abA[r] = adv + be; jdA[r] = jd; lapTA[r] = lapT; zcA[r] = zc; tcA[r] = tc;
@@ -232,15 +246,30 @@
   auto resid = [&](int b, int r, double s0, double s1, double q) -> double {
     double re = q;
 #ifdef MSOM_STRICT
-    if (upper) re = re + s0 * ring[b][wv - 1][r][NV - 1][lane] * idh0;
-    if (lower) re = re - s1 * ring[b][wv][r][NV - 1][lane] * idh1;
+    if (upper) re = re + s0 * ring[b][wv - 1][r][DS][lane] * idh0;
+    if (lower) re = re - s1 * ring[b][wv][r][DS][lane] * idh1;
     re += xdA[r];
     re += ydA[r];
 #else
-    if (upper) re = fma(idh0, s0 * ring[b][wv - 1][r][NV - 1][lane], re);
-    if (lower) re = fma(-(ring[b][wv][r][NV - 1][lane] * s1), idh1, re);
-    re = fma(rD, xdA[r], re);
-    re = fma(rD, ydA[r], re);
+    if (upper) re = fma(idh0, s0 * ring[b][wv - 1][r][DS][lane], re);
+    if (lower) re = fma(-(ring[b][wv][r][DS][lane] * s1), idh1, re);
+    re = fma(rD, PARK3 ? ring[b][wv][r][XS + 1][lane] : xdA[r], re);
+    re = fma(rD, PARK3 ? ring[b][wv][r][XS + 2][lane] : ydA[r], re);
+#endif
+    return re;
+  };
+  auto resid_close = [&](int b, int r, double s0, double s1, double q) -> double {
+    double re = q;
+#ifdef MSOM_STRICT
+    if (upper) re = re + s0 * ring[b][wv - 1][r][DS][lane] * idh0;
+    if (lower) re = re - s1 * ring[b][wv][r][DS][lane] * idh1;
+    re += xdA[r];
+    re += ydA[r];
+#else
+    if (upper) re = fma(idh0, s0 * ring[b][wv - 1][r][DS][lane], re);
+    if (lower) re = fma(-(ring[b][wv][r][DS][lane] * s1), idh1, re);
+    re = fma(rD, ring[b][wv][r][XS][lane], re);
+    re = fma(rD, PARK3 ? ring[b][wv][r][XS + 2][lane] : ydA[r], re);
 #endif
     return re;
   };
@@ -284,6 +313,13 @@
 #pragma unroll
       for (int r = 0; r < R; r++)
         if (out_ok && jb + r < y1 && !(a.dbg & 1)) outp[nat_idx(a.g, l, jb + r, gic)] = val[r];
+      if (CLS) {
+#pragma unroll
+        for (int r = 0; r < R; r++) {
+          const double cr = resid_close(b ^ 1, r, s0[r], s1[r], CLS == 2 ? breg[r] : qreg[r]);
+          if (out_ok && jb + r < y1) cls_m = fmax(cls_m, fabs(cr));
+        }
+      }
       if (RES) {
         double re[R];
 #pragma unroll
@@ -316,6 +352,7 @@
       for (int r = 0; r < R; r++) {
         const size_t c = nat_idx(a.g, l, (a.dbg & 2) ? y0 : (EDGE ? min(j0 + r, ny - 1) : j0 + r), gic);
         if (ADV) qreg[r] = a.q_in[c];
+        if (CLS == 2) breg[r] = a.rr.cls_b[c];
         if (QF) fqreg[r] = a.qforc[c];
         if (STOCH) { qsreg[r] = a.q_stage[c]; nzreg[r] = a.noise[c]; }
       }
@@ -334,12 +371,13 @@
   }
 }
 
-template <int R, bool UNI, bool QF, bool ADV, bool STOCH = false, bool RES = false>
+template <int R, bool UNI, bool QF, bool ADV, bool STOCH = false, bool RES = false, int CLS = 0>
 __global__ void __launch_bounds__(64 * LPW_MAXW) k_rhs_lpw(LpwArgs a) {
   static_assert(!RES || (ADV && !STOCH && R % 2 == 0), "the residual by-product rides in the plain tendency + advance pass");
-  constexpr int NV = LPW_NV + (RES ? 1 : 0);
+  static_assert(!CLS || (RES && UNI), "the closing by-product rides beside the residual by-product, uniform S");
+  constexpr int NV = LPW_NV + (RES ? 1 : 0) + LPW_CLS_PARK(CLS);
   __shared__ double ring[2][LPW_MAXW][R][NV][64];
-  double res_m = 0., res_bs = 0.;
+  double res_m = 0., res_bs = 0., cls_m = 0., cls_u = 0.;
   const int wv = __builtin_amdgcn_readfirstlane((int)(threadIdx.x >> 6));
   const int nx = a.g.nx, ny = a.g.ny;
   const int strip = blockIdx.x * a.NS + wv / a.nl, nstrips = (nx + LPW_W - 1) / LPW_W;
@@ -351,22 +389,38 @@
     const bool inner = strip < nstrips && x0 - 3 >= 0 && x0 + 60 < nx && y0 - 3 >= 0 && y0 + nblk * R + R + 2 < ny;
     if ((a.region == 1) != inner) return;
   }
-  if (xwall || ywall || a.noedge_off) lpw_body<R, UNI, QF, ADV, STOCH, true, RES, NV>(a, ring, res_m, res_bs);
-  else lpw_body<R, UNI, QF, ADV, STOCH, false, RES, NV>(a, ring, res_m, res_bs);
+  if (xwall || ywall || a.noedge_off) lpw_body<R, UNI, QF, ADV, STOCH, true, RES, CLS, NV>(a, ring, res_m, res_bs, cls_m, cls_u);
+  else lpw_body<R, UNI, QF, ADV, STOCH, false, RES, CLS, NV>(a, ring, res_m, res_bs, cls_m, cls_u);
   if (RES) {
     const int lane = threadIdx.x & 63, nw = blockDim.x >> 6;
     for (int o = 32; o > 0; o >>= 1) {
       res_m = fmax(res_m, __shfl_xor(res_m, o, 64));
       res_bs += __shfl_xor(res_bs, o, 64);
+      if (CLS) cls_m = fmax(cls_m, __shfl_xor(cls_m, o, 64));
+      if (CLS == 2) cls_u = fmax(cls_u, __shfl_xor(cls_u, o, 64));
     }
     double *red = &ring[0][0][0][0][0];
-    if (lane == 0) { red[wv] = res_m; red[LPW_MAXW + wv] = res_bs; }
+    if (lane == 0) {
+      red[wv] = res_m; red[LPW_MAXW + wv] = res_bs;
+      if (CLS) red[2 * LPW_MAXW + wv] = cls_m;
+      if (CLS == 2) red[3 * LPW_MAXW + wv] = cls_u;
+    }
     __syncthreads();
     if (threadIdx.x == 0) {
       double mm = red[0], ss = red[LPW_MAXW];
       for (int k = 1; k < nw; k++) { mm = fmax(mm, red[k]); ss += red[LPW_MAXW + k]; }
       atomicMax((unsigned long long *)a.rr.res_max, (unsigned long long)__double_as_longlong(mm));
       a.rr.bsum_partial[blockIdx.y * gridDim.x + blockIdx.x] = ss;
+      if (CLS) {
+        double cm = red[2 * LPW_MAXW];
+        for (int k = 1; k < nw; k++) cm = fmax(cm, red[2 * LPW_MAXW + k]);
+        atomicMax((unsigned long long *)a.rr.cls_max, (unsigned long long)__double_as_longlong(cm));
+      }
+    }
+    if (CLS == 2 && (int)threadIdx.x < a.nl) {
+      double um = red[3 * LPW_MAXW + threadIdx.x];
+      for (int k = threadIdx.x + a.nl; k < nw; k += a.nl) um = fmax(um, red[3 * LPW_MAXW + k]);
+      atomicMax((unsigned long long *)(a.rr.cls_umax + threadIdx.x), (unsigned long long)__double_as_longlong(um));
     }
   }
 }
@@ -403,6 +457,10 @@
   const bool res = rr != nullptr;
   if (res && (stoch || !q_out || region || (g.nx & 1) || (g.ny & 1) || !rr->res_c)) {
     fprintf(stderr, "msom: launch_rhs_lpw: the residual by-product needs the plain tendency + advance pass on one tile with even sides\n");
+    abort();
+  }
+  if (res && rr->cls && (!uniformS || rr->cls < 0 || rr->cls > 2 || !rr->cls_max || (rr->cls == 2 && (!rr->cls_b || !rr->cls_umax)))) {
+    fprintf(stderr, "msom: launch_rhs_lpw: the closing by-product needs uniform S, its accumulators and (second stage) the solve's right-hand side\n");
     abort();
   }
   if (res) {
@@ -434,6 +492,8 @@
     with_bool(have_qforc, [&](auto Q) {
       constexpr bool UNI = decltype(U)::value, QF = decltype(Q)::value;
       if (stoch) hipLaunchKernelGGL((k_rhs_lpw<LPW_R, UNI, QF, true, true>), gr, bl, 0, st, a);
+      else if (res && UNI && a.rr.cls == 1) hipLaunchKernelGGL((k_rhs_lpw<LPW_R_RES, UNI, QF, true, false, true, UNI ? 1 : 0>), gr, bl, 0, st, a);
+      else if (res && UNI && a.rr.cls == 2) hipLaunchKernelGGL((k_rhs_lpw<LPW_R_RES, UNI, QF, true, false, true, UNI ? 2 : 0>), gr, bl, 0, st, a);
       else if (res) hipLaunchKernelGGL((k_rhs_lpw<LPW_R_RES, UNI, QF, true, false, true>), gr, bl, 0, st, a);
       else if (q_out) hipLaunchKernelGGL((k_rhs_lpw<LPW_R, UNI, QF, true>), gr, bl, 0, st, a);
       else hipLaunchKernelGGL((k_rhs_lpw<LPW_R, UNI, QF, false>), gr, bl, 0, st, a);
diff --git a/msom_amd/csrc/kernels_mg.hip b/msom_amd/csrc/kernels_mg.hip
--- a/msom_amd/csrc/kernels_mg.hip
+++ b/msom_amd/csrc/kernels_mg.hip
@@ -404,7 +404,7 @@
 }
 
 #define RM_OW 62
-template <int NL>
+template <int NL, bool PSI_ONLY = false>
 __global__ void __launch_bounds__(256) k_resmax_march(Res2Args p, int H) {
   __shared__ double smm[4];
   __shared__ double smu[MSOM_MAXNL][4];
@@ -428,30 +428,32 @@
       Wm[l] = pa[l * ls + (ptrdiff_t)(y0 - 1) * pitch];
       Wc[l] = pa[l * ls + (ptrdiff_t)y0 * pitch];
       Wp[l] = pa[l * ls + (ptrdiff_t)min(y0 + 1, ny) * pitch];
-      qc[l] = pb[l * ls + (ptrdiff_t)y0 * pitch];
+      qc[l] = PSI_ONLY ? 0. : pb[l * ls + (ptrdiff_t)y0 * pitch];
     }
 #pragma unroll
     for (int l = 0; l < NL; l++) { Em[l] = lane_above(Wm[l]); Mm[l] = lane_below(Wm[l]); }
     for (int j = y0; j < y1; j++) {
       const ptrdiff_t rn = (ptrdiff_t)min(j + 2, ny) * pitch, rq = (ptrdiff_t)min(j + 1, ny - 1) * pitch;
 #pragma unroll
-      for (int l = 0; l < NL; l++) { Wn[l] = pa[l * ls + rn]; qn[l] = pb[l * ls + rq]; }
+      for (int l = 0; l < NL; l++) { Wn[l] = pa[l * ls + rn]; qn[l] = PSI_ONLY ? 0. : pb[l * ls + rq]; }
 #pragma unroll
       for (int l = 0; l < NL; l++) {
         const double c = Wc[l], E = lane_above(c), W = lane_below(c), N = Wp[l], S = Wm[l], NW = lane_below(N), SE = Em[l], SW = Mm[l];
         const double be = qc[l];
         double re = be;
-        if (NL > 1) {
+        if (NL > 1 && !PSI_ONLY) {
           const double i0 = p.rc.idh0[l], i1 = p.rc.idh1[l];
           const double z0 = l > 0 ? p.rc.S[l - 1] : 0., z1 = l < NL - 1 ? p.rc.S[l] : 0.;
           if (l == 0) re = be + z1 * (c - Wc[l + 1 < NL ? l + 1 : l]) * i1;
           else if (l < NL - 1) re = be + z0 * (c - Wc[l - 1]) * i0 - z1 * (Wc[l + 1 < NL ? l + 1 : l] - c) * i1;
           else re = be + z0 * (c - Wc[l - 1]) * i0;
         }
-        re += DIVC(DIVC(c - W, D, rD) - DIVC(E - c, D, rD), D, rD);
-        re += DIVC(DIVC(c - S, D, rD) - DIVC(N - c, D, rD), D, rD);
+        if (!PSI_ONLY) {
+          re += DIVC(DIVC(c - W, D, rD) - DIVC(E - c, D, rD), D, rD);
+          re += DIVC(DIVC(c - S, D, rD) - DIVC(N - c, D, rD), D, rD);
+        }
         const double u = fabs(DIVC(0.25 * (N - S + NW - SW), D, rD)), v = fabs(DIVC(0.25 * (E - W + SE - SW), D, rD));
-        if (own) { m = fmax(m, fabs(re)); uu[l] = fmax(uu[l], fmax(u, v)); }
+        if (own) { if (!PSI_ONLY) m = fmax(m, fabs(re)); uu[l] = fmax(uu[l], fmax(u, v)); }
         Em[l] = E; Mm[l] = W;
       }
 #pragma unroll
@@ -466,7 +468,7 @@
     if (lane == 0) smu[l][wv] = w;
   }
   __syncthreads();
-  if (threadIdx.x == 0) {
+  if (threadIdx.x == 0 && !PSI_ONLY) {
     const double mm = fmax(fmax(smm[0], smm[1]), fmax(smm[2], smm[3]));
     atomicMax((unsigned long long *)p.maxres, (unsigned long long)__double_as_longlong(mm));
   }
@@ -475,15 +477,16 @@
         fmax(fmax(smu[threadIdx.x][0], smu[threadIdx.x][1]), fmax(smu[threadIdx.x][2], smu[threadIdx.x][3]));
 }
 template <int NL>
-static dim3 resmax_march_launch(hipStream_t st, const Res2Args &p, int H) {
+static dim3 resmax_march_launch(hipStream_t st, const Res2Args &p, int H, bool psi_only) {
   const int nstrips = (p.g.nx + RM_OW - 1) / RM_OW;
   dim3 gr((nstrips + 3) / 4, (p.g.ny + H - 1) / H);
-  hipLaunchKernelGGL(k_resmax_march<NL>, gr, dim3(256), 0, st, p, H);
+  if (psi_only) hipLaunchKernelGGL((k_resmax_march<NL, true>), gr, dim3(256), 0, st, p, H);
+  else hipLaunchKernelGGL((k_resmax_march<NL, false>), gr, dim3(256), 0, st, p, H);
   return gr;
 }
-static dim3 launch_resmax_march(hipStream_t st, const Res2Args &p, int H) {
+static dim3 launch_resmax_march(hipStream_t st, const Res2Args &p, int H, bool psi_only) {
   dim3 gr;
-  if (!with_int<1, MSOM_FASTNL>(p.nl, [&](auto N) { gr = resmax_march_launch<N()>(st, p, H); })) no_kernel("launch_resmax_march", p.nl);
+  if (!with_int<1, MSOM_FASTNL>(p.nl, [&](auto N) { gr = resmax_march_launch<N()>(st, p, H, psi_only); })) no_kernel("launch_resmax_march", p.nl);
   return gr;
 }
 
@@ -542,9 +545,15 @@
     case 2: hipLaunchKernelGGL((k_residual2<false, true, false>), gr, block2d(), 0, st, p); break;
     case 6: hipLaunchKernelGGL((k_residual2<false, true, true>), gr, block2d(), (size_t)nl * (BY * BX * 2 + 2 * BX) * sizeof(double), st, p); break;
     case 0: hipLaunchKernelGGL((k_residual2<false, false, false>), gr, block2d(), 0, st, p); break;
+    case 8 | 16:
+      if (!(uniformS && g.nx >= 64 && g.ny >= 16 && o.resmax_rows >= 0 && nl <= MSOM_FASTNL)) no_kernel("launch_residual2 (psi only)", nl);
+      gr = launch_resmax_march(st, p, o.resmax_rows ? o.resmax_rows : 32, true);
+      if (!umax_clean) (void)hipMemsetAsync(umax_out, 0, nl * sizeof(double), st);
+      hipLaunchKernelGGL(k_max_final_mg, dim3(64), dim3(256), 0, st, umax_partial, umax_out, (int)(gr.x * gr.y), nl);
+      break;
     case 8:
       if (uniformS && g.nx >= 64 && g.ny >= 16 && o.resmax_rows >= 0 && nl <= MSOM_FASTNL) {
-        gr = launch_resmax_march(st, p, o.resmax_rows ? o.resmax_rows : 32);
+        gr = launch_resmax_march(st, p, o.resmax_rows ? o.resmax_rows : 32, false);
       } else if (g.nx % 2 == 0 && g.nx >= CR_TW && g.ny >= CR_TR && !(p.dbg & 128)) {
         gr = dim3((g.nx + CR_TW - 1) / CR_TW, (g.ny + CR_TR - 1) / CR_TR);
         if (uniformS) hipLaunchKernelGGL((k_correct_residual<true, false>), gr, block2d(), 0, st, p);
diff --git a/msom_amd/csrc/msom_api.hip b/msom_amd/csrc/msom_api.hip
--- a/msom_amd/csrc/msom_api.hip
+++ b/msom_amd/csrc/msom_api.hip
@@ -1,6 +1,8 @@
 #include "msom_host.h"
 
 #define RHS_RESID_MIN 23
+#define RHS_CLOSE_MIN 23
+#define RHS_CLOSE_DEFAULT 2
 #define MARCH_HALO 4
 
 static void free_agglomeration(msom *m);
@@ -533,6 +535,10 @@
   else if (!strcmp(key, "adv_fused")) m->adv_fused = (int)v;
   else if (!strcmp(key, "overlap")) m->overlap = (int)v;
   else if (!strcmp(key, "rhs_resid")) { m->rhs_resid = (int)v; m->res_ready = -1; }
+  else if (!strcmp(key, "rhs_close")) {
+    if ((int)v < -1 || (int)v > 2) { msom_set_error("option rhs_close = %g (-1, 0, 1 or 2)", v); return MSOM_ERR_ARG; }
+    m->rhs_close = (int)v; m->res_ready = -1;
+  }
   else if (!strcmp(key, "seed")) { m->seed = (unsigned)v; srand(m->seed); }
   else if (!strcmp(key, "noise_mode")) m->noise_mode = (int)v;
   else if (!strcmp(key, "stoch_fused")) m->stoch_fused = (int)v;
@@ -589,6 +595,7 @@
 static int level_path(const msom *m, int k);
 static bool restrict2_ok(const msom *m);
 static bool rhs_resid_emits(const msom *m);
+static int rhs_close_mode(const msom *m);
 extern "C" double msom_get_param(msom_t *m, const char *key) {
   if (!m || !key) return NAN;
   if (!strcmp(key, "model")) return m->model;
@@ -634,6 +641,7 @@
   if (!strcmp(key, "march_visit_ring")) return !fine_visit_fused(m) ? -1 : (m->opt.march_visit_ring >= 2 ? 2 : (m->opt.march_visit_ring == 1 ? 1 : 0));
   if (const int *o = kernel_opt(m->opt, key)) return *o;
   if (!strcmp(key, "rhs_resid")) return rhs_resid_emits(m);
+  if (!strcmp(key, "rhs_close")) return rhs_close_mode(m);
   if (!strncmp(key, "split_ls_", 9)) { const int k = atoi(key + 9); return k >= 0 && k < m->nlev ? (double)m->sg[k].ls : NAN; }
   if (!strncmp(key, "split_rp_", 9)) { const int k = atoi(key + 9); return k >= 0 && k < m->nlev ? (double)m->sg[k].rp : NAN; }
   if (!strcmp(key, "split_pad")) return MSOM_SP;
@@ -1067,6 +1075,27 @@
   if (m->nlev < 2 || level_path(m, 0) != RP_MARCH) return false;
   const Lev L = tile_lev(m, 0), C = tile_lev(m, 1);
   return march_next(m, L, fuse_prolong(m, L, 4) ? &C : nullptr, 8, corr_wanted(m)).kind == MA_VISIT;
+}
+
+static bool fine_corr_in_smoother(const msom *m) {
+  if (m->nlev < 2 || level_path(m, 0) != RP_MARCH || !corr_wanted(m)) return false;
+  const Lev L = tile_lev(m, 0), C = tile_lev(m, 1);
+  const Lev *src = fuse_prolong(m, L, 4) ? &C : nullptr;
+  for (int n = 8;;) {
+    const MarchAct a = march_next(m, L, src, n, true);
+    if (a.kind == MA_HALF || a.kind == MA_DONE) return false;
+    if (a.kind == MA_VISIT || a.corr) return true;
+    src = nullptr; n -= a.K;
+  }
+}
+static bool spec_ok(const msom *m);
+static int rhs_close_mode(const msom *m) {
+  int v = m->rhs_close;
+  if (v < 0) v = (size_t)m->g.nx * m->g.ny * m->nl >= ((size_t)1 << RHS_CLOSE_MIN) ? (m->have_qforc ? 1 : RHS_CLOSE_DEFAULT) : 0;
+  if (v <= 0) return 0;
+  const bool resmax_marching = m->uniformS && m->nl <= MSOM_FASTNL && m->g.nx >= 64 && m->g.ny >= 16 && m->opt.resmax_rows >= 0;
+  if (!spec_ok(m) || !rhs_resid_emits(m) || !resmax_marching || !fine_corr_in_smoother(m)) return 0;
+  return v;
 }
 
 static bool march_halo(msom *m, int k, bool wrap, bool res, MarchHalo *h) {
@@ -1398,7 +1427,14 @@
       if (m->nranks > 1) STICKY(m, exch_nat(m, m->f[MSOM_PSI], m->nl, m->bc, 1));
       else if (m->bc == BC_PERIODIC) launch_fill_periodic(m->st, m->f[MSOM_PSI], m->g, m->nl, 1);
       else launch_fill_ghost(m->st, m->f[MSOM_PSI], m->g, m->nl, m->bc, m->walls);
-      residual2(m, 8, b, SC_RES1, 0);
+      const int cls = (s->i == 0 && m->spec_hook && m->nranks == 1) ? rhs_close_mode(m) : 0;
+      m->close_cls = !cls ? 0 : (m->dt_dev ? 1 : (cls >= 2 ? 2 : 0));
+      m->close_b = b;
+      if (m->close_cls == 2) {
+        if (!m->umax_clean) HIPCHK(hipMemsetAsync(m->d_scal + SC_UMAX, 0, m->nl * sizeof(double), m->st));
+        m->umax_clean = 0;
+      }
+      else residual2(m, m->close_cls ? 8 | 16 : 8, b, SC_RES1, 0);
       m->umax_ready = 1;
     } else if (fused) {
       residual2(m, 1, b, SC_RES1, 0);
@@ -1414,6 +1450,7 @@
       m->spec_hook([&]() {});
       m->spec_launched = 1;
     }
+    m->close_cls = 0;
     int rr = read_residuals(m);
     if (rr) { m->spec_launched = 0; return rr; }
     if (m->spec_launched) {
@@ -1497,6 +1534,9 @@
     if (use_rr) {
       rr.res = m->res[0]; rr.res_c = m->res[1]; rr.res_max = m->d_scal + SC_RESF; rr.bsum_partial = m->partial_rr;
       rr.sg = m->sg[0]; rr.cg = m->sg[1];
+      if (m->close_cls) {
+        rr.cls = m->close_cls; rr.cls_b = m->close_b; rr.cls_max = m->d_scal + SC_RES1; rr.cls_umax = m->d_scal + SC_UMAX;
+      }
     }
     auto with_psi_halo = [&](bool splittable, auto launch) {
       if (m->nranks > 1 && m->overlap && splittable) {
@@ -1904,7 +1944,7 @@
   return fill_bc(m, out);
 }
 
-static bool spec_ok(msom *m) {
+static bool spec_ok(const msom *m) {
   return layered_fusions(m) && m->async_solve && m->nranks == 1 && m->fused && m->adv_fused && m->rhs_variant == 6 && m->mg_fused && m->nlev > 1 &&
          m->nl <= MSOM_FASTNL && !m->have_pg && !m->have_zpg && !m->flag_topo && !m->stochastic && m->p.nptr == 0 && m->p.nitermin >= 1 && !m->dbg_nosync;
 }
@@ -1925,11 +1965,15 @@
       for (int l = 0; l < MSOM_MAXNL; l++) a.umax_pg[l] = m->umax_pg[l];
       a.D = p.L0 / m->gnx; a.CFL = p.CFL; a.previous = m->previous; a.dtmax = p.DT; a.t = m->t; a.tnext = m->tnext; a.nl = m->nl;
       a.with_dt = 1; a.seq = ++m->pub_seq;
-      hipLaunchKernelGGL(k_step_dt, dim3(1), dim3(64), 0, m->st, m->d_scal, a, m->d_pub);
+      hipLaunchKernelGGL(k_step_dt, dim3(1), dim3(64), 0, m->st, m->d_scal, a, m->close_cls ? nullptr : m->d_pub);
       host_read();
       int adv = 0;
       spec_rc = rhs_terms(m, MSOM_Q, MSOM_DQ, 1, p.iRe, p.iRe4, p.Eks, p.Ekb, MSOM_QPRED, MSOM_Q, 0., &adv);
       if (!adv && !spec_rc) spec_rc = MSOM_ERR_STATE;
+      if (m->close_cls) {
+        a.with_dt = 0;
+        hipLaunchKernelGGL(k_step_dt, dim3(1), dim3(64), 0, m->st, m->d_scal, a, m->d_pub);
+      }
     };
   }
   const double d = solve_and_dt(m, MSOM_Q, p.DT);
@@ -1962,13 +2006,14 @@
       StepDtArgs a;
       memset(&a, 0, sizeof a);
       a.with_dt = 0; a.seq = ++m->pub_seq;
-      hipLaunchKernelGGL(k_step_dt, dim3(1), dim3(64), 0, m->st, m->d_scal, a, m->d_pub);
+      if (!m->close_cls) hipLaunchKernelGGL(k_step_dt, dim3(1), dim3(64), 0, m->st, m->d_scal, a, m->d_pub);
       host_read();
       int adv = 0;
       m->adv_out_override = m->q_alt;
       spec_rc = rhs_terms(m, MSOM_QPRED, MSOM_DQ, 1, p.iRe, p.iRe4, p.Eks, p.Ekb, MSOM_Q, MSOM_Q, m->dt, &adv);
       m->adv_out_override = nullptr;
       if (!adv && !spec_rc) spec_rc = MSOM_ERR_STATE;
+      if (m->close_cls) hipLaunchKernelGGL(k_step_dt, dim3(1), dim3(64), 0, m->st, m->d_scal, a, m->d_pub);
     };
   }
   const double d2 = solve_and_dt(m, MSOM_QPRED, m->dt);
diff --git a/msom_amd/csrc/msom_host.h b/msom_amd/csrc/msom_host.h
--- a/msom_amd/csrc/msom_host.h
+++ b/msom_amd/csrc/msom_host.h
@@ -144,6 +144,9 @@
   int adv_fused = 1;
   int rhs_resid = -1;
   int rr_nparts = 0;
+  int rhs_close = -1;
+  int close_cls = 0;
+  const double *close_b = nullptr;
   int bfn_begun = 0;
   int bfn_obs_set = 0, bfn_gain_set = 0;
   double *bfn_partial = nullptr;
```

New measurement: 19.10 billion grid-point-updates/s (median of 6 runs). 1.04x the previous value.
